# gchochla/VAuLT

Hardware: AMD Instinct MI355X
Metric: train samples/sec (img+text pairs) ViLT-B32+BERTweet, bs256, 1/2/4/8 MI355X (higher is better)
Workload: dtype bf16; 1 GPU; ViLT-B32 + bertweet fine-tune step (fwd+bwd+AdamW), per-GPU batch 256, 40 text tokens + 384x384 image (185-token fused sequence; resident as the patch-embedding operand `pixel_patches`, the input pipeline's output), all weights trained; global_batch=256, seq_len=185, parallelism=dp1

## Files before the change

include/vault_hip.h:

```cpp
#ifndef VAULT_HIP_H
#define VAULT_HIP_H
#include <stdint.h>
#ifdef __cplusplus
extern "C" {
#endif

int vault_abi_version(void);
int vault_operand_format(void);

typedef struct vault_gemm_args {
  const void* A; const void* B; void* out; void* out2;
  const float* bias; const float* res; const void* aux; const float* addtab;
  float* colsum;
  int split3;
  int M, N, K, lda, ldb, ldo, m_valid;
  int a_mode, b_mode, epi, cfg, splits, accumulate;
  int rpg, gstride, goff;
  uint32_t drop_thresh, drop_seed, drop_stream; float drop_scale;
  int gn;
  int persist;
  int batch;
  long long batch_a, batch_b, batch_o;
  int aux_u8;
  int out_hm;
  int a_hm;
  void* out_q; void* out_scale;
  void* splitk_ws; long long splitk_bytes;
} vault_gemm_args;
int vault_gemm(const vault_gemm_args* args, void* stream);
int vault_gemm_plan(const vault_gemm_args* args);

typedef struct vault_wgrad_seg {
  const void* dy; const void* x; float* dw;
  int n_out, n_in, ld_dy, ld_x, ld_dw;
  int batch;
  int first, count;
  long long batch_dy, batch_x, batch_dw;
  int dy_hm;
} vault_wgrad_seg;
typedef struct vault_wgrad_grouped_args {
  int nseg;
  vault_wgrad_seg seg[3];
  int tokens, splits, accumulate;
  int persist;
} vault_wgrad_grouped_args;
int vault_wgrad_grouped(const vault_wgrad_grouped_args* args, void* stream);

int vault_quant_mxfp8(const void* src_bf16, long long rows, int K, int ld_src, void* dst_q, void* dst_scale, void* stream);
int vault_gemm_mxfp8(const vault_gemm_args* args, const void* a_scale, const void* b_scale, void* stream);
int vault_gemm_mxfp8_plan(const vault_gemm_args* args);


typedef struct vault_ln_fwd_args {
  const float* x; const float* gamma; const float* beta; const float* post_add;
  void* y_bf16; float* y_f32; float* mean; float* rstd;
  int rows, H; float eps;
  int x_rpg, x_gstride, x_goff, y_rpg, y_gstride, y_goff;
  uint32_t drop_thresh, drop_seed, drop_stream; float drop_scale;
  void* y_split3;
  void* y_q; void* y_scale;
} vault_ln_fwd_args;
int vault_layernorm_fwd(const vault_ln_fwd_args* args, void* stream);

typedef struct vault_ln_bwd_args {
  const void* dy_bf16; const float* dy_f32; const float* x; const float* mean; const float* rstd;
  const float* gamma; const float* dres;
  float* dx_f32; void* dx_bf16; float* dgamma; float* dbeta;
  int rows, H;
  int dy_rpg, dy_gstride, dy_goff, x_rpg, x_gstride, x_goff, dx_rpg, dx_gstride, dx_goff;
  uint32_t drop_thresh, drop_seed, drop_stream; float drop_scale;
  int drop_on_dy;
  float* dbias;
  const void* dres_bf16;
} vault_ln_bwd_args;
int vault_layernorm_bwd(const vault_ln_bwd_args* args, void* stream);

int vault_colsum(const void* in_bf16, int ld, int rows, int N, float* out, void* stream);
int vault_colsum_hm(const void* in_bf16, int rows, int hm_rows, int planes, float* out, int batch, long long batch_in,
                    long long batch_out, void* stream);
int vault_colsum_batched(const void* in_bf16, int ld, int rows, int N, float* out, int batch, long long batch_in,
                         long long batch_out, void* stream);


typedef struct vault_attn_args {
  const void* qkv; const float* keymask; void* ctx; float* lse;
  const void* dctx; void* dqkv;
  int B, S, H, heads;
  uint32_t drop_thresh, drop_seed, drop_stream; float drop_scale;
  void* ctx_split3;
  int qkv_hm;
  float* bias_partials;
  int bias_thirds;
  int q_rows;
} vault_attn_args;
int vault_attention_fwd(const vault_attn_args* args, void* stream);
int vault_attention_bwd(const vault_attn_args* args, void* stream);
int vault_attention_bwd_partials(const vault_attn_args* args);
int vault_colsum_partials(const float* part, int nparts, int n, float* out, int batch, long long batch_in,
                          long long batch_out, void* stream);


int vault_position_ids(const int64_t* ids, int* pos, int B, int T, int mode, int pad, void* stream);

typedef struct vault_gather_args {
  const float* src; float* out;
  const float* tab[3]; const void* idx[3]; int is64[3]; int fixed[3];
  int period, rows, H;
  const float* rowmask;
} vault_gather_args;
int vault_gather_sum(const vault_gather_args* args, void* stream);
int vault_scatter_add(const vault_gather_args* args, void* stream);

int vault_im2col(const float* pixel_values, void* out_bf16, int B, int C, int IMG, int ps, int split3, void* stream);

int vault_image_consts(const float* conv_bias, const float* pos_emb, const float* mtype1, const float* cls,
                       float* addtab, float* x, int P, int H, int B, int S, int T, void* stream);
int vault_image_rows_bwd(const float* dx, float* dpos, float* dmtype1, float* dcls, float* dconv_bias,
                         void* dyp_bf16, int P, int H, int B, int S, int T, void* stream);

int vault_im2col_sel(const float* pixel_values, void* out_bf16, const int* sel, int B, int L, int C, int HP, int WP,
                     int ps, int split3, void* stream);
int vault_image_sel_consts(const float* conv_bias, const float* pos_emb, const float* mtype1, const float* cls,
                           float* addtab, float* x, int L, int H, int B, int S, int T, void* stream);
int vault_image_pos_sel_fwd(float* x, const float* pos_emb, const int* sel, const int* hw, int B, int L, int S, int T,
                            int H, int gw, int G, void* stream);
int vault_image_sel_bwd(const float* dx, float* dpos, float* dmtype1, float* dcls, float* dconv_bias, void* dyp_bf16,
                        const int* sel, const int* hw, int B, int L, int S, int T, int H, int gw, int G, void* stream);
int vault_axpy_f32(float* dst, const float* src, float a, long long n, void* stream);
int vault_scale_f32(float* x, float a, long long n, void* stream);
int vault_rows_add_f32(const float* src, const float* vec, float* out, int rows, int H, int rpg, int gstride, int goff,
                       void* stream);
int vault_rows_gather_bwd_f32(const float* dx, float* dsrc, float* dvec, int rows, int H, int rpg, int gstride, int goff,
                              void* stream);
int vault_rows_scatter_bf16(const void* src, void* out, int rows, int H, int rpg, int gstride, int goff, void* stream);

typedef struct vault_head_args {
  const float* pre; const float* Wc; const float* bc; const int64_t* labels; const float* dlogits;
  float* pooled; float* logits; float* loss_sum; float* dWc; float* dbc; void* dpre_bf16;
  int B, H, C; float loss_scale, grad_scale;
  uint32_t drop_thresh, drop_seed, drop_stream; float drop_scale;
  const float* targets; int loss_kind;
} vault_head_args;
int vault_head_fwd(const vault_head_args* args, void* stream);
int vault_head_bwd(const vault_head_args* args, void* stream);
int vault_tanh_bwd(const float* pooled, const float* dpooled, void* dpre_bf16, long long n, void* stream);
int vault_gelu_fwd(const float* x, void* y_bf16, long long n, void* stream);
int vault_gelu_fwd_f32(const float* x, float* y_f32, long long n, void* stream);
int vault_gelu_bwd(const float* x, const float* dy, float* dx, long long n, void* stream);

int vault_adamw_step(float* p, float* g, float* m, float* v, void* p_bf16, long long n, float lr, float beta1,
                     float beta2, float eps, float weight_decay, float bias_corr_factor, float grad_scale,
                     int zero_grad, const unsigned char* zero_mask, void* stream);
#define VAULT_GRAD_NORM_PARTIALS 2048
int vault_grad_norm(const float* g, long long n, double* partials, float* out2, float max_norm, float unscale, void* stream);
int vault_adamw_step_grouped(float* p, float* g, float* m, float* v, void* p_bf16, long long n,
                             const unsigned char* group_map, const float* group_table, int n_groups, float lr_factor,
                             float beta1, float beta2, float eps, float bias_corr_factor, float grad_scale,
                             const float* coef, int zero_grad, const unsigned char* zero_mask, void* stream);
int vault_adamw_step_ema(float* p, float* g, float* m, float* v, void* p_bf16, float* ema, long long n,
                         const unsigned char* group_map, const float* group_table, int n_groups, float lr_factor,
                         float beta1, float beta2, float eps, float bias_corr_factor, float grad_scale, const float* coef,
                         float one_minus_decay, int zero_grad, const unsigned char* zero_mask, void* stream);
int vault_ema_swap(float* p, float* ema, void* p_bf16, long long n, void* stream);
int vault_adamw_step_torch(float* p, float* g, float* m, float* v, void* p_bf16, float* ema ,
                           long long n, const unsigned char* group_map, const float* group_table, int n_groups,
                           float lr_factor, float beta1, float beta2, float eps, float inv_bias_corr1,
                           float inv_sqrt_bias_corr2, float grad_scale, const float* coef, float one_minus_decay,
                           int zero_grad, const unsigned char* zero_mask, void* stream);
int vault_cast_bf16(const float* x, void* y_bf16, long long n, void* stream);
int vault_h16_census(const void* x_h16, long long n, unsigned long long* out4, void* stream);
int vault_rows_union(const long long* keys, long long n_keys, int V, int* flags_zeroed, long long* uniq, int* count,
                     void* stream);
int vault_rows_gather_f32(const float* table, const long long* idx, int n_rows, int H, float* out, void* stream);
int vault_rows_scatter_f32(const float* src, const long long* idx, int n_rows, int H, float* table, void* stream);
int vault_sum_chunks_bf16(const void* src_bf16, int n_src, long long chunk, void* out_bf16, void* stream);
int vault_widen_bf16(const void* x_bf16, float* y, long long n, void* stream);
int vault_transpose_bf16(const void* src, void* dst, int rows, int cols, int batch, long long stride_src,
                         long long stride_dst, void* stream);
int vault_split3_bf16(const float* x, void* out_bf16, long long rows, int K, int layout, void* stream);

typedef struct vault_layer_args {
  int B, S, H, FF, heads, rows, rows_pad; float eps;
  const void *wqkv, *wo, *wi, *wf, *wo_t, *wf_t;
  const float *bqkv, *bo, *bi, *bf, *ln1w, *ln1b, *ln2w, *ln2b;
  const float* x_in; const void* x_in_bf16; float* x_out; void* x_out_bf16; const float* keymask;
  void *n1, *qkv, *ctx; float* lse; float* xm; float* y1; void* n2; void* act; void* u; float* h2;
  float *m1, *r1, *m2, *r2;
  uint32_t attn_drop_thresh, hid_drop_thresh, drop_seed, drop_stream_base; float attn_drop_scale, hid_drop_scale;
  int persist;
  void* splitk_ws; long long splitk_bytes;
} vault_layer_args;
typedef struct vault_layer_bwd_args {
  const vault_layer_args* fwd;
  const void* dy_bf16; const float* dy_f32;
  float* dx_f32; void* dx_bf16;
  void *dU, *dN, *dctx, *dqkv, *dmid_bf16, *dh1_bf16; float* dmid_f32;
  float *g_wqkv, *g_bqkv, *g_wo, *g_bo, *g_wi, *g_bi, *g_wf, *g_bf, *g_ln1w, *g_ln1b, *g_ln2w, *g_ln2b, *g_bf_below;
  int do_wgrad;
} vault_layer_bwd_args;
long long vault_layer_workspace_bytes(int B, int S, int H, int FF, int heads, int train, long long* rows_pad_out);
int vault_vilt_layer_fwd(const vault_layer_args* args, void* stream);
int vault_vilt_layer_bwd(const vault_layer_bwd_args* args, void* stream);
int vault_lm_layer_fwd(const vault_layer_args* args, void* stream);
int vault_lm_layer_bwd(const vault_layer_bwd_args* args, void* stream);

typedef struct vault_lm_embed_args {
  int B, T, H, rows_pad, pos_mode, pad_id; float eps;
  const int64_t* ids; const int64_t* token_type_ids; const float* inputs_embeds;
  const float *word, *pos, *type, *lnw, *lnb;
  int* pos_ids; float* esum; float* mean; float* rstd; float* y; void* y_bf16;
  uint32_t drop_thresh, drop_seed, drop_stream; float drop_scale;
  const void* dy_bf16; const float* dy_f32; float* desum; const float* rowmask;
  float *g_word, *g_pos, *g_type, *g_lnw, *g_lnb;
} vault_lm_embed_args;
int vault_lm_embed_fwd(const vault_lm_embed_args* args, void* stream);
int vault_lm_embed_bwd(const vault_lm_embed_args* args, void* stream);

typedef struct vault_text_embed_args {
  int B, T, S, H, rows_pad; float eps;
  const float* text_src; const int64_t* ids; const int64_t* token_type_ids;
  const float *word, *pos, *type, *lnw, *lnb, *mtype0;
  float* vsum; float* mean; float* rstd; float* x;
  const float* dx; float* dvsum; float* dbeta_scratch;
  float *g_word, *g_pos, *g_type, *g_lnw, *g_lnb, *g_mtype0;
} vault_text_embed_args;
int vault_vilt_text_embed_fwd(const vault_text_embed_args* args, void* stream);
int vault_vilt_text_embed_bwd(const vault_text_embed_args* args, void* stream);

typedef struct vault_patch_embed_args {
  int B, C, IMG, ps, T, S, H;
  const float* pixel_values; const void* w_bf16; const float *conv_bias, *pos_emb, *mtype1, *cls;
  void* apatch; float* addtab; float* x; int persist;
  const float* dx; void* dyp;
  float *g_w, *g_conv_bias, *g_pos, *g_mtype1, *g_cls;
} vault_patch_embed_args;
int vault_patch_embed_fwd(const vault_patch_embed_args* args, void* stream);
int vault_patch_embed_bwd(const vault_patch_embed_args* args, void* stream);

typedef struct vault_head_loss_args {
  int B, S, H, C, seq_rows_pad; float eps;
  const float* x; const float *lnw, *lnb; const void* wp_bf16; const float* bp; const float *Wc, *bc;
  const int64_t* labels; const float* targets; int loss_kind; float loss_scale, grad_scale;
  void* h0_bf16; float* mean; float* rstd; float* pre; float* pooled; float* logits; float* loss;
  uint32_t drop_thresh, drop_seed, drop_stream; float drop_scale; int persist;
  void* dpre; void* dh0; float* dx_f32; void* dx_bf16;
  float *g_Wc, *g_bc, *g_wp, *g_bp, *g_lnw, *g_lnb, *g_bf_last;
} vault_head_loss_args;
int vault_head_loss_fwd(const vault_head_loss_args* args, void* stream);
int vault_head_loss_bwd(const vault_head_loss_args* args, void* stream);

typedef struct vault_image_desc {
  long long src_off, tmp_off;
  int h_in, w_in, h_out, w_out, ksize_h, ksize_v;
  int hb_off, hk_off, vb_off, vk_off;
} vault_image_desc;
typedef struct vault_preprocess_args {
  const uint8_t* src; uint8_t* tmp; const int* plan; const vault_image_desc* desc; const float* lut;
  float* pixel_values; int64_t* pixel_mask; float* pixel_mask_f32;
  int B, H, W, max_h_in, max_w_out;
  int max_w_in; long long src_bytes;
  void* patch_unfold_bf16; int ps;
  int ksize_max, band_rows_max;
} vault_preprocess_args;
int vault_image_preprocess(const vault_preprocess_args* args, void* stream);
int vault_image_preprocess_is_fused(const vault_preprocess_args* args);

typedef struct vault_model_dims {
  int H, FF, heads, lm_layers, vilt_layers, IMG, ps, C, n_classes;
} vault_model_dims;
long long vault_workspace_bytes(const vault_model_dims* dims, int B, int T, int train);

#ifdef __cplusplus
}
#endif
#endif
```

vault_amd/backward.py:

```python
from __future__ import annotations

import contextlib
from typing import Dict, Optional

import torch

from . import ops
from .params import _in_format, _pad


class BackwardMixin:
    def _wgrads_aside(self, launch, after_layer, items=0):
        if not (self._wgrad_side or items > 0) or after_layer is not None:
            launch()
            return
        if self._wgrad_stream is None:
            self._wgrad_stream = torch.cuda.Stream(self.device)
        side, main, ev = self._wgrad_stream, torch.cuda.current_stream(), torch.cuda.Event()
        ops.pycall(lambda: ev.record(main))
        ops.pycall(lambda: side.wait_event(ev))
        with torch.cuda.stream(side):
            self._wgrad_items = items
            try:
                launch()
            finally:
                self._wgrad_items = 0
        self._wgrad_pending = True

    def _join_wgrads(self):
        if self._wgrad_pending:
            side, main, ev = self._wgrad_stream, torch.cuda.current_stream(), torch.cuda.Event()
            ops.pycall(lambda: ev.record(side))
            ops.pycall(lambda: main.wait_event(ev))
            self._wgrad_pending = False

    def _wgrad(self, dy_bf16, x_bf16, wname, bname, Mtok_pad, Nout, Kin, m_valid, out_rows=0, unsplit=False):
        P = self.params
        gw = P.gr(wname, n_elems=Nout * Kin, shape=(Nout, Kin))
        if gw is None:
            return
        nk = Mtok_pad // 64
        wide = Nout % 256 == 0 and Kin % 256 == 0 and (Nout // 256) * (Kin // 256) >= 24
        if Mtok_pad <= 16384 and Nout % 128 == 0 and Kin % 128 == 0 and not wide:
            tiles = (Nout // 128) * (Kin // 128)
            splits = 7 if tiles <= 36 else (4 if tiles <= 108 else 3)
            cfg = 0
        elif Nout % 256 == 0 and Kin % 256 == 0:
            tiles = (Nout // 256) * (Kin // 256)
            splits = max(1, min(nk // 2, 256 // tiles, 16))
            cfg = 3
        else:
            tiles = (Nout // 128) * (Kin // 128)
            splits = max(1, min(nk, (self.WGRAD_TARGET_WGS + tiles - 1) // tiles))
            cfg = 0
        if unsplit:
            splits = 1
        if cfg == 3:
            ops.pycall(lambda: self._prof_begin("wgrad"))
        ops.gemm(dy_bf16, x_bf16, gw, Nout, Kin, Mtok_pad, Nout, Kin, Kin, 1, 1, ops.EPI_F32_ATOMIC, cfg=cfg,
                 splits=splits, accumulate=1, m_valid=out_rows)
        if cfg == 3:
            fl = 2.0 * m_valid * Nout * Kin
            ops.pycall(lambda: self._prof_end("wgrad", fl))
        if bname is not None:
            ops.colsum(dy_bf16, Nout, m_valid, Nout, P.gr(bname, n_elems=Nout, shape=(Nout,)))

    @staticmethod
    def _wgrad_splits(items, per_round, nk, fixed, fixed_unsplit=None):
        def cost(sp):
            fx = fixed_unsplit if (sp == 1 and fixed_unsplit is not None) else fixed
            return -(-items * sp // per_round) * (1.67 * -(-nk // sp) + fx)
        return min((sp for sp in range(1, 9) if nk // sp >= 2), key=cost)

    def _wgrad_batched(self, dY_all, X_all, wnames, i0, Mtok_pad, Nout, Kin, m_valid):
        P = self.params
        G = len(wnames)
        offs = [P.offsets[w][0] for w in wnames]
        stride_o = (offs[1] - offs[0]) if G > 1 else 0
        if any(offs[k + 1] - offs[k] != stride_o for k in range(G - 1)) or Nout % 128 or Kin % 128:
            raise RuntimeError("batched weight gradients need identically laid out layers and 128-multiples")
        gw = P.gr(wnames[0], n_elems=Nout * Kin, shape=(Nout, Kin))
        nk = Mtok_pad // 64
        if Nout % 256 == 0 and Kin % 256 == 0:
            cfg, tiles = 3, (Nout // 256) * (Kin // 256) * G
            splits = self._wgrad_splits(tiles, 256, nk, 40.0)
        else:
            cfg, tiles = 0, (Nout // 128) * (Kin // 128) * G
            splits = max(1, min(8, Mtok_pad // 512, int(round(512.0 / tiles))))
        st = torch.cuda.current_stream()
        if cfg == 3:
            ops.pycall(lambda: self._prof_begin("wgrad", st))
        acc = 0 if (self._grads_zero and splits == 1) else 1
        ops.gemm(dY_all[i0], X_all[i0], gw, Nout, Kin, Mtok_pad, Nout, Kin, Kin, 1, 1, ops.EPI_F32_ATOMIC, cfg=cfg,
                 splits=splits, accumulate=acc, batch=G, batch_a=dY_all.stride(0), batch_b=X_all.stride(0),
                 batch_o=stride_o)
        if acc == 0:
            self._stored_ranges += [(o, Nout * Kin) for o in offs]
        if cfg == 3:
            fl = 2.0 * m_valid * Nout * Kin * G
            ops.pycall(lambda: self._prof_end("wgrad", fl, st))
    def _wgrad_group_size(self, n_layers, after_layer, stack="lm"):
        if after_layer is None or self.dp_world <= 1:
            return n_layers
        if stack == "vilt" and self.spec.lm is not None and not self.freeze_lm:
            return n_layers
        g = self.LM_WGRAD_GROUP
        return g if g > 0 else n_layers

    def _wgrad_group(self, kinds, layers, i0, hi, Mtok_pad, m_valid, counts=None):
        P = self.params
        Gs = [hi - i0] * len(kinds) if counts is None else list(counts)
        kinds, Gs = [k for k, n in zip(kinds, Gs) if n > 0], [n for n in Gs if n > 0]
        hms = [k[5] if len(k) > 5 else 0 for k in kinds]
        kinds = [k[:5] for k in kinds]
        ok = all(no % 256 == 0 and ki % 256 == 0 for *_, no, ki in kinds)
        strides = []
        for (dY_all, X_all, wsel, Nout, Kin), G in zip(kinds, Gs):
            offs = [P.offsets[getattr(l_, wsel)][0] for l_ in layers[i0:i0 + G]]
            so = (offs[1] - offs[0]) if G > 1 else 0
            ok = ok and all(offs[k + 1] - offs[k] == so for k in range(G - 1))
            strides.append(so)
        if not ok:
            if any(hms):
                raise RuntimeError("head-major dqkv needs the grouped ring weight-gradient launches (_plan_head_major)")
            for (dY_all, X_all, wsel, Nout, Kin), G in zip(kinds, Gs):
                self._wgrad_batched(dY_all, X_all, [getattr(l_, wsel) for l_ in layers[i0:i0 + G]], i0, Mtok_pad, Nout, Kin, m_valid)
            return
        nk = Mtok_pad // 64
        CU = self._wgrad_items or (self.WGRAD_SIDE_ITEMS if self._wgrad_side else 256)
        remaining = []
        for k, (dY_all, X_all, wsel, Nout, Kin) in enumerate(kinds):
            remaining.append([k, 0, (Nout // 256) * (Kin // 256) * Gs[k]])
        launches, cur, room = [], [], CU
        for k, first, left in remaining:
            while left > 0:
                take = min(left, room)
                cur.append((k, first, take))
                first, left, room = first + take, left - take, room - take
                if room == 0 or len(cur) == 3:
                    launches.append(cur)
                    cur, room = [], CU
        if cur:
            launches.append(cur)
        st = torch.cuda.current_stream()
        covered: Dict[tuple, int] = {}
        for segs in launches:
            count = sum(c for _, _, c in segs)
            if count == CU:
                splits = 1
            else:
                splits = self._wgrad_splits(count, CU, nk, 50.0, 10.0 if self._grads_zero else 50.0)
            acc = 0 if (self._grads_zero and splits == 1) else 1
            args = []
            for k, first, c in segs:
                dY_all, X_all, wsel, Nout, Kin = kinds[k]
                if acc == 0:
                    tpl = (Nout // 256) * (Kin // 256)
                    for it in range(first, first + c):
                        covered[(k, it // tpl)] = covered.get((k, it // tpl), 0) + 1
                gw = P.gr(getattr(layers[i0], wsel), n_elems=Nout * Kin, shape=(Nout, Kin))
                args.append(dict(dy=dY_all[i0], x=X_all[i0], dw=gw, n_out=Nout, n_in=Kin, batch=Gs[k], first=first, count=c,
                                 batch_dy=dY_all.stride(0), batch_x=X_all.stride(0), batch_dw=strides[k], dy_hm=hms[k]))
            ops.pycall(lambda: self._prof_begin("wgrad", st))
            ops.wgrad_grouped(args, Mtok_pad, splits=splits, accumulate=acc)
            fl = 2.0 * m_valid * 65536.0 * count
            ops.pycall(lambda fl=fl: self._prof_end("wgrad", fl, st))
        for (k, lay), n in covered.items():
            _, _, wsel, Nout, Kin = kinds[k]
            if n == (Nout // 256) * (Kin // 256):
                self._stored_ranges.append((P.offsets[getattr(layers[i0 + lay], wsel)][0], Nout * Kin))

    def _qkv_bias_grads_batched(self, dqkv_all, layers, i0, hi, ld, rows, N, hm=0, parts=None):
        P = self.params
        offs = [P.offsets[l_.qb][0] for l_ in layers[i0:hi]]
        stride_o = (offs[1] - offs[0]) if len(offs) > 1 else 0
        if any(offs[k + 1] - offs[k] != stride_o for k in range(len(offs) - 1)):
            raise RuntimeError("batched bias gradients need identically laid out layers")
        gqb = P.gr(layers[i0].qb, n_elems=ld, shape=(ld,))
        if parts is not None:
            part_all, nparts = parts
            ops.colsum_partials(part_all[i0], nparts, N, gqb, hi - i0, part_all.stride(0), stride_o)
            return
        if hm:
            ops.colsum_hm(dqkv_all[i0], rows, hm, N // 64, gqb, hi - i0, dqkv_all.stride(0), stride_o)
            return
        ops.colsum_batched(dqkv_all[i0], ld, rows, N, gqb, hi - i0, dqkv_all.stride(0), stride_o)
    @_in_format
    def zero_grad(self):
        if self.params.g is not None:
            self.params.g.zero_()
        self._g_dirty = False
        self._g_stale_key = None

    def backward(self, grad_scale: Optional[float] = None, dlogits: Optional[torch.Tensor] = None,
                 dpooled: Optional[torch.Tensor] = None, dhidden: Optional[torch.Tensor] = None,
                 after_layer=None, ws: Optional[dict] = None):
        self._api_backward_begins()
        with torch.cuda.device(self.device), self._grads_scaled():
            self._backward(grad_scale, dlogits, dpooled, dhidden, after_layer, ws)
            if self.grad_scale != 1.0:
                w_ = self.last if ws is None else ws
                for k in ("d_inputs_embeds", "d_image_embeds"):
                    t = w_.get(k)
                    if t is not None:
                        with ops.operand_format(self.half):
                            ops.scale(t, 1.0 / self.grad_scale, t.numel())

    def _api_backward_begins(self):
        if self._g_stale_key is not None:
            self.zero_grad()
        self._g_dirty = True

    @contextlib.contextmanager
    def _grads_scaled(self):
        def rescale(factor):
            if self.grad_scale != 1.0 and self.params.g is not None:
                with ops.operand_format(self.half):
                    ops.scale(self.params.g, factor, self.params.n_train)
        rescale(self.grad_scale)
        try:
            yield
        finally:
            rescale(1.0 / self.grad_scale)

    def _scaled_in(self, ws, name, t):
        t = t.contiguous()
        if self.grad_scale == 1.0:
            return t
        b = self._buf(ws, name, tuple(t.shape), torch.float32)
        b.copy_(t)
        ops.scale(b.view(-1), self.grad_scale, b.numel())
        return b

    @_in_format
    def _backward(self, grad_scale, dlogits, dpooled, dhidden, after_layer, ws=None, grads_zero=False):
        self._grads_zero = bool(grads_zero)
        self._stored_ranges = []
        ws = self.last if ws is None else ws
        if ws is None or not ws.get("train"):
            raise RuntimeError("backward() needs a preceding forward(train=True)")
        if ws.get("pruned_last") and dhidden is not None:
            raise ValueError("the forward pruned the last layer to the pooler's rows: a gradient of last_hidden_state needs "
                             "forward(need_hidden=True)")
        self.drop_seed = ws["drop_seed"]
        note = (lambda tag: ops.pycall(lambda: after_layer(tag))) if after_layer is not None else (lambda tag: None)
        self._wgrad_side = ws["Mp"] <= self.WGRAD_STREAM_MAX_ROWS
        vb = self._vilt_grad_buffers(ws, after_layer)
        self._backward_head(ws, vb["top"], grad_scale, dlogits, dpooled, dhidden)
        note("head")
        self._backward_vilt_stack(ws, vb, after_layer, note)
        dvs = self._backward_vilt_embeddings(ws, vb["dx"], after_layer)
        note("vilt_embed")
        if self.spec.lm is None or self.freeze_lm:
            self._join_wgrads()
        else:
            self._backward_lm_stack(ws, dvs, after_layer, note)
        self._run_census(ws, "backward")

    def _wgrad_groups(self, ws, tag, layers, after_layer, dY, X, rows_pad, rows):
        H, FF = ws["H"], ws["FF"]
        kinds = tuple((dy, ws[x], wsel, no, ki) for dy, x, (wsel, no, ki) in
                      zip(dY, X, (("fw", H, FF), ("iw", FF, H), ("ow", H, H), ("qw", 3 * H, H))))
        n, cut = len(layers), 1 if (tag == "vilt" and ws.get("pruned_last")) else 0
        return dict(layers=layers, size=self._wgrad_group_size(n, after_layer, tag), kinds=kinds, H=H,
                    rows_pad=rows_pad, rows=rows, ends=(n - cut, n - cut, n - cut, n))

    def _layer_done(self, tag, grp, i, note, after_layer, N=None, hm=0, parts=None, items=0, ahead=None):
        if grp is None:
            note(f"{tag}{i}")
        if grp is None or i % grp["size"]:
            return
        layers, kinds, H, hi = grp["layers"], grp["kinds"], grp["H"], min(len(grp["layers"]), i + grp["size"])
        if ahead is not None:
            ahead()

        def launch():
            self._qkv_bias_grads_batched(kinds[3][0], layers, i, hi, 3 * H, grp["rows"], 3 * H if N is None else N, hm=hm, parts=parts)
            self._wgrad_group(kinds[:3] + (kinds[3] + (hm,),), layers, i, hi, grp["rows_pad"], grp["rows"],
                              counts=[max(0, min(hi, e) - i) for e in grp["ends"]])
        self._wgrads_aside(launch, after_layer, items=items)
        for j in reversed(range(i, hi)):
            note(f"{tag}{j}")

    def _backward_head(self, ws, dxb_top, grad_scale, dlogits, dpooled, dhidden):
        spec, P, x, nv = self.spec, self.params, ws["x"], len(self.vl)
        B, S, M, H = (ws[k] for k in ("B", "S", "M", "H"))
        pruned = bool(ws.get("pruned_last"))
        cls_map = (0, 0, 0) if pruned else (1, S, 0)
        if not pruned:
            ops.pycall(dxb_top.zero_)
        if spec.add_pooling_layer and (spec.n_classes > 0 or dpooled is not None):
            Bp = ws["Bp"]
            dpre = self._buf(ws, "dpre", (Bp, H), self.hdt)
            if spec.n_classes > 0 and spec.head == "mlp" and dpooled is None:
                if dlogits is None:
                    raise ValueError("the MLP head has no built-in loss: pass dlogits (the autograd bridge does)")
                ops.tanh_bwd(ws["pooled"], self._mlp_backward(ws, dlogits, B, scale=self.grad_scale), dpre, B * H)
            elif spec.n_classes > 0 and dpooled is None:
                hd = self._drop(self.classifier_dropout, 9001, True)
                gs = ((1.0 / B) if grad_scale is None else grad_scale) * self.grad_scale
                if dlogits is not None:
                    dlogits = self._scaled_in(ws, "dlogits_scaled", dlogits)
                ops.head_bwd(ws["pooled"], ws["logits"], ws.get("labels"), P.w("classifier.1.weight"),
                             P.gr("classifier.1.weight"), P.gr("classifier.1.bias"), dpre, B, H, spec.n_classes, gs,
                             dlogits=dlogits, drop=hd)
            else:
                ops.tanh_bwd(ws["pooled"], self._scaled_in(ws, "dpooled_scaled", dpooled), dpre, B * H)
            self._wgrad(dpre, ws["h0b"], "pooler.dense.weight", "pooler.dense.bias", Bp, H, H, B)
            dh0 = self._buf(ws, "dh0", (Bp, H), self.hdt)
            self._dgrad(dpre, "pooler.dense.weight", dh0, Bp, H, H, ops.EPI_BF16, B)
            ops.layernorm_bwd(ws["pl_xout"] if pruned else x[nv], ws["f_mean"], ws["f_rstd"], P.w("layernorm.weight"), B, H,
                              dy_bf16=dh0, dx_bf16=dxb_top, dgamma=P.gr("layernorm.weight"),
                              dbeta=P.gr("layernorm.bias"), xmap=cls_map, dxmap=cls_map,
                              dbias=None if dhidden is not None else P.gr(self.vl[nv - 1].fb))
        if dhidden is not None:
            ops.layernorm_bwd(x[nv], ws["f_mean_all"], ws["f_rstd_all"], P.w("layernorm.weight"), M, H,
                              dy_f32=self._scaled_in(ws, "dhidden_scaled", dhidden).view(M, H),
                              dres_bf16=dxb_top,
                              dx_bf16=dxb_top,
                              dgamma=P.gr("layernorm.weight"), dbeta=P.gr("layernorm.bias"),
                              dbias=P.gr(self.vl[nv - 1].fb))

    def _layer_bwd_staged(self, ws, style, layers, i, d, deferred):
        P, ln, H = self.params, layers[i], ws["H"]
        a = ws[f"stage_{style}{i}"]
        if style == "lm":
            a.drop_seed = self.drop_seed & 0xFFFFFFFF
        gb = ops.layer_bwd_args(
            a, **d, do_wgrad=0 if deferred else 1, g_wqkv=P.gr(ln.qw, n_elems=3 * H * H, shape=(3 * H, H)),
            g_bqkv=None if deferred else P.gr(ln.qb, n_elems=3 * H, shape=(3 * H,)),
            g_wo=P.gr(ln.ow), g_bo=P.gr(ln.ob), g_wi=P.gr(ln.iw), g_bi=P.gr(ln.ib), g_wf=P.gr(ln.fw),
            g_ln1w=P.gr(ln.ln1w), g_ln1b=P.gr(ln.ln1b), g_ln2w=P.gr(ln.ln2w), g_ln2b=P.gr(ln.ln2b),
            g_bf=P.gr(ln.fb) if style == "lm" else None,
            g_bf_below=P.gr(layers[i - 1].fb) if (style == "vilt" and i > 0) else None)
        ws[f"stage_{style}_bwd{i}"] = gb
        ops.layer_call(f"vault_{style}_layer_bwd", gb, seeded=bool(a.attn_drop_thresh or a.hid_drop_thresh))

    def _vilt_grad_buffers(self, ws, after_layer):
        Mp, H, FF, nv, bf = ws["Mp"], ws["H"], ws["FF"], len(self.vl), self.hdt
        vb = dict(dx=self._buf(ws, "dx_a", (Mp, H), torch.float32), grp=None,
                  dxb=(self._buf(ws, "dxb_a", (Mp, H), bf), self._buf(ws, "dxb_b", (Mp, H), bf)))
        if self.LM_WGRAD_BATCHED and "act_all" in ws and self.params.gr(self.vl[0].fw) is not None:
            vb["dY"] = (self._stack(ws, "v_dxbA", nv, (Mp, H), bf), self._stack(ws, "v_dU", nv, (Mp, FF), bf),
                        self._stack(ws, "v_dxbB", nv, (Mp, H), bf), self._stack(ws, "v_dqkv", nv, (Mp, 3 * H), bf))
            vb["grp"] = self._wgrad_groups(ws, "vilt", self.vl, after_layer, vb["dY"],
                                           ("act_all", "n2_all", "ctx_all", "n1_all"), Mp, ws["M"])
        vb["top"] = vb["dY"][0][nv - 1] if vb["grp"] else vb["dxb"][0]
        if ws.get("pruned_last"):
            vb["top"] = self._buf(ws, "pl_dtop", (ws["Bp"], H), bf)
        return vb

    def _backward_vilt_stack(self, ws, vb, after_layer, note):
        B, S, Mp, H, FF, heads, nv, bf = ws["B"], ws["S"], ws["Mp"], ws["H"], ws["FF"], ws["heads"], len(self.vl), self.hdt
        grp, staged, (dxa, dxb) = vb["grp"], bool(ws.get("vilt_stage")), vb["dxb"]
        d = dict(dN=self._buf(ws, "dN", (Mp, H), bf), dctx=self._buf(ws, "dctx", (Mp, H), bf))
        if not grp:
            d.update(dy_bf16=dxa, dmid_bf16=dxb, dx_bf16=dxa, dU=self._buf(ws, "dU", (Mp, FF), bf), dqkv=self._buf(ws, "dqkv", (Mp, 3 * H), bf))
        short, vparts = bool(grp) and self.QKV_BIAS_SHORTCUT and not staged, None
        if short:
            npart = ops.attention_bwd_partials(B, S, H, heads, 1)
            if npart:
                vparts = (self._stack(ws, "v_qbpart", nv, (npart, H), torch.float32), npart)
        beside = self.WGRAD_BESIDE_LM_ITEMS if (grp and grp["size"] >= nv and not staged and self.spec.lm is not None
                                                and not self.freeze_lm and not self._wgrad_side) else 0
        ops.pycall(lambda: self._prof_begin("vilt_bwd"))
        for i in reversed(range(nv)):
            if grp:
                d["dy_bf16"], d["dU"], d["dmid_bf16"], d["dqkv"] = (t[i] for t in vb["dY"])
                d["dx_bf16"] = vb["dY"][0][i - 1] if i > 0 else dxa
            d["dx_f32"] = vb["dx"] if i == 0 else None
            if staged:
                self._layer_bwd_staged(ws, "vilt", self.vl, i, d, bool(grp))
            elif i == nv - 1 and ws.get("pruned_last"):
                self._vilt_last_layer_bwd_pruned(ws, i, d, bool(grp), short, vparts, vb["top"])
            else:
                self._vilt_layer_bwd(ws, i, d, bool(grp), short, vparts)
            self._layer_done("vilt", grp, i, note, after_layer, H if short else 3 * H, ws.get("qkv_hm", 0), vparts, beside)
        ops.pycall(lambda: self._prof_end("vilt_bwd"))

    def _vilt_layer_bwd(self, ws, i, d, deferred, short, vparts):
        P, ln, vhm = self.params, self.vl[i], ws.get("qkv_hm", 0)
        B, S, M, Mp, H, FF, heads = (ws[k] for k in ("B", "S", "M", "Mp", "H", "FF", "heads"))
        g = lambda k: ws[f"{k}{i}"]
        wgrad = (lambda *a: None) if deferred else self._wgrad
        dyA, dyB, dU, dqkv, dN, dctx = (d[k] for k in ("dy_bf16", "dmid_bf16", "dU", "dqkv", "dN", "dctx"))
        g8 = ws.get("gelu8_active")
        g8kw = dict(cfg=g8, aux_u8=True) if g8 is not None else {}
        self._dgrad(dyA, ln.fw, dU, Mp, FF, H, ops.EPI_BF16_DGELU, M, aux=g("u"), colsum=P.gr(ln.ib), **g8kw)
        wgrad(dyA, g("act"), ln.fw, None, Mp, H, FF, M)
        self._dgrad(dU, ln.iw, dN, Mp, H, FF, ops.EPI_BF16, M)
        wgrad(dU, g("n2"), ln.iw, None, Mp, FF, H, M)
        ops.layernorm_bwd(g("xm"), g("m2"), g("r2"), P.w(ln.ln2w), M, H, dy_bf16=dN, dres_bf16=dyA, dx_bf16=dyB,
                          dgamma=P.gr(ln.ln2w), dbeta=P.gr(ln.ln2b), dbias=P.gr(ln.ob))
        gqb = P.gr(ln.qb, n_elems=3 * H, shape=(3 * H,))
        self._dgrad(dyB, ln.ow, dctx, Mp, H, H, ops.EPI_BF16, M, **(dict(colsum=gqb[2 * H:]) if short else {}))
        wgrad(dyB, g("ctx"), ln.ow, None, Mp, H, H, M)
        ops.attention_bwd(g("qkv"), ws["keymask"], g("ctx"), g("lse"), dctx, dqkv, B, S, H, heads, qkv_hm=vhm,
                          **(dict(bias_partials=vparts[0][i], bias_thirds=1) if vparts else {}))
        self._dgrad(dqkv, ln.qw, dN, Mp, H, 3 * H, ops.EPI_BF16, M, **(dict(a_hm=vhm) if vhm else {}))
        wgrad(dqkv, g("n1"), ln.qw, ln.qb, Mp, 3 * H, H, M)
        ops.layernorm_bwd(ws["x"][i], g("m1"), g("r1"), P.w(ln.ln1w), M, H, dy_bf16=dN, dres_bf16=dyB,
                          dx_f32=d["dx_f32"], dx_bf16=d["dx_bf16"], dgamma=P.gr(ln.ln1w), dbeta=P.gr(ln.ln1b),
                          dbias=P.gr(self.vl[i - 1].fb) if i > 0 else None)

    def _vilt_last_layer_bwd_pruned(self, ws, i, d, deferred, short, vparts, dtop):
        P, ln, vhm = self.params, self.vl[i], ws.get("qkv_hm", 0)
        B, S, M, Mp, H, FF, heads, Bp = (ws[k] for k in ("B", "S", "M", "Mp", "H", "FF", "heads", "Bp"))
        bf = self.hdt
        g, c = (lambda k: ws[f"{k}{i}"]), (lambda k: ws[f"pl_{k}"])
        dU, dNc, dmid, dctx = (self._buf(ws, f"pl_{k}", (Bp, w), bf) for k, w in (("dU", FF), ("dN", H), ("dmid", H), ("dctx", H)))
        dres, dqkv, dN = self._buf(ws, "pl_dres", (Mp, H), bf), d["dqkv"], d["dN"]
        g8 = ws.get("pl_gelu8")
        g8kw = dict(cfg=g8, aux_u8=True) if g8 is not None else {}
        self._dgrad(dtop, ln.fw, dU, Bp, FF, H, ops.EPI_BF16_DGELU, B, aux=c("u"), colsum=P.gr(ln.ib), like=Mp, **g8kw)
        self._wgrad(dtop, c("act"), ln.fw, None, Bp, H, FF, B, unsplit=True)
        self._dgrad(dU, ln.iw, dNc, Bp, H, FF, ops.EPI_BF16, B, like=Mp)
        self._wgrad(dU, c("n2"), ln.iw, None, Bp, FF, H, B, unsplit=True)
        ops.layernorm_bwd(c("xm"), c("m2"), c("r2"), P.w(ln.ln2w), B, H, dy_bf16=dNc, dres_bf16=dtop, dx_bf16=dmid,
                          dgamma=P.gr(ln.ln2w), dbeta=P.gr(ln.ln2b), dbias=P.gr(ln.ob))
        ops.rows_scatter_h16(dmid, dres, B, H, 1, S, 0)
        gqb = P.gr(ln.qb, n_elems=3 * H, shape=(3 * H,))
        self._dgrad(dmid, ln.ow, dctx, Bp, H, H, ops.EPI_BF16, B, like=Mp, **(dict(colsum=gqb[2 * H:]) if short else {}))
        self._wgrad(dmid, c("ctx"), ln.ow, None, Bp, H, H, B, unsplit=True)
        ops.attention_bwd(g("qkv"), ws["keymask"], c("ctx"), g("lse"), dctx, dqkv, B, S, H, heads, qkv_hm=vhm, q_rows=1,
                          **(dict(bias_partials=vparts[0][i], bias_thirds=1) if vparts else {}))
        self._dgrad(dqkv, ln.qw, dN, Mp, H, 3 * H, ops.EPI_BF16, M, **(dict(a_hm=vhm) if vhm else {}))
        if not deferred:
            self._wgrad(dqkv, g("n1"), ln.qw, ln.qb, Mp, 3 * H, H, M)
        ops.layernorm_bwd(ws["x"][i], g("m1"), g("r1"), P.w(ln.ln1w), M, H, dy_bf16=dN, dres_bf16=dres,
                          dx_f32=d["dx_f32"], dx_bf16=d["dx_bf16"], dgamma=P.gr(ln.ln1w), dbeta=P.gr(ln.ln1b),
                          dbias=P.gr(self.vl[i - 1].fb) if i > 0 else None)

    def _backward_vilt_embeddings(self, ws, dx0, after_layer):
        spec, P, v = self.spec, self.params, self.spec.vilt
        B, T, S, H, NP, Ml, Mlp, Kp, Mpp = (ws[k] for k in ("B", "T", "S", "H", "NP", "Ml", "Mlp", "Kp", "Mpp"))
        buf = lambda name, shape, dtype=torch.float32: self._buf(ws, name, shape, dtype)
        dyp = buf("dyp", (Mpp, H), self.hdt)
        gpos = P.gr("embeddings.position_embeddings", shape=(v.num_patches + 1, H))
        gmt = P.gr("embeddings.token_type_embeddings.weight")
        if ws.get("img_embeds") is not None:
            die = buf("d_iemb", (_pad(B * NP), H))
            ops.rows_gather_bwd(dx0, die, gmt[ws.get("img_type", 1)], B * NP, H, NP, S, T)
            ws["d_image_embeds"] = die[:B * NP].view(B, NP, H)
        elif ws["ragged"]:
            ops.image_sel_bwd(dx0, gpos, gmt[ws.get("img_type", 1)], P.gr("embeddings.cls_token", shape=(H,)),
                              P.gr("embeddings.patch_embeddings.projection.bias"), dyp, ws["sel"], ws["hw"], B, NP, S, T, H,
                              ws["gw"], v.image_size // v.patch_size)
        else:
            ops.image_rows_bwd(dx0, gpos, gmt[ws.get("img_type", 1)], P.gr("embeddings.cls_token", shape=(H,)),
                               P.gr("embeddings.patch_embeddings.projection.bias"), dyp, NP, H, B, S, T)
        if ws.get("img_embeds") is None:
            self._wgrads_aside(lambda: self._wgrad(dyp, ws["apatch_in"] if ws.get("patches_in") else ws["apatch"],
                                                   "embeddings.patch_embeddings.projection.weight", None,
                                                   Mpp, H, Kp, B * NP), after_layer)
        dvs = buf("d_vt_sum", (Mlp, H))
        dbeta_now = buf("d_vt_beta", (H,))
        ops.pycall(dbeta_now.zero_)
        ops.layernorm_bwd(ws["vt_sum"], ws["vt_mean"], ws["vt_rstd"], P.w("embeddings.text_embeddings.LayerNorm.weight"),
                          Ml, H, dy_f32=dx0, dymap=(T, S, 0), dx_f32=dvs,
                          dgamma=P.gr("embeddings.text_embeddings.LayerNorm.weight"), dbeta=dbeta_now)
        ops.axpy(P.gr("embeddings.text_embeddings.LayerNorm.bias"), dbeta_now, 1.0, H)
        ops.axpy(gmt[0], dbeta_now, 1.0, H)
        tt = ws["tt"]
        gt = [(P.gr("embeddings.text_embeddings.token_type_embeddings.weight"), tt if tt is not None else 0)]
        if spec.lm is None:
            if ws.get("txt_embeds") is not None:
                ws["d_inputs_embeds"] = dvs[:Ml].view(B, T, H)
            else:
                gt.append((P.gr("embeddings.text_embeddings.word_embeddings.weight"), ws["ids"]))
        if ws["use_pos"]:
            gt.append((P.gr("embeddings.text_embeddings.position_embeddings.weight"), "mod"))
        ops.scatter_add(dvs, gt, Ml, H, period=T)
        return dvs

    def _backward_lm_stack(self, ws, dvs, after_layer, note):
        B, T, H, FF, heads, Ml, Mlp = (ws[k] for k in ("B", "T", "H", "FF", "heads", "Ml", "Mlp"))
        nl, bf, staged = len(self.ll), self.hdt, bool(ws.get("lm_stage"))
        buf = lambda name, shape, dtype=torch.float32: self._buf(ws, name, shape, dtype)
        dN, grp = buf("lm_dN", (Mlp, H), bf), None
        d = dict(dy_bf16=None, dy_f32=dvs, dmid_f32=buf("lm_dh", (Mlp, H)), dx_f32=buf("lm_dh1", (Mlp, H)), dN=dN, dx_bf16=dN,
                 dctx=buf("lm_dctx", (Mlp, H), bf))
        if self.LM_WGRAD_BATCHED and "lm_act_all" in ws and self.params.gr(self.ll[0].fw) is not None:
            dY = (self._stack(ws, "lm_dhb", nl, (Mlp, H), bf), self._stack(ws, "lm_dU", nl, (Mlp, FF), bf),
                  self._stack(ws, "lm_dh1b", nl, (Mlp, H), bf), self._stack(ws, "lm_dqkv", nl, (Mlp, 3 * H), bf))
            grp = self._wgrad_groups(ws, "lm", self.ll, after_layer, dY,
                                     ("lm_act_all", "lm_y1b_all", "lm_ctx_all", "lm_yb_all"), Mlp, Ml)
        else:
            d.update(dmid_bf16=buf("lm_dhb", (Mlp, H), bf), dh1_bf16=buf("lm_dh1b", (Mlp, H), bf),
                     dU=buf("lm_dU", (Mlp, FF), bf), dqkv=buf("lm_dqkv", (Mlp, 3 * H), bf))
        lparts = None
        if self.LM_BIAS_PARTIALS and grp and not staged:
            npart = ops.attention_bwd_partials(B, T, H, heads, 3)
            if npart:
                lparts = (self._stack(ws, "lm_qbpart", nl, (npart, 3 * H), torch.float32), npart)
        embed_done = []

        def embed_ahead():
            self._lm_embed_backward(ws, d["dy_bf16"], d["dy_f32"])
            embed_done.append(True)
            note("lm_embed")
        ops.pycall(lambda: self._prof_begin("lm_bwd"))
        for i in reversed(range(nl)):
            if grp:
                d["dmid_bf16"], d["dU"], d["dh1_bf16"], d["dqkv"] = (t[i] for t in dY)
            if staged:
                self._layer_bwd_staged(ws, "lm", self.ll, i, d, bool(grp))
            else:
                self._lm_layer_bwd(ws, i, d, bool(grp), lparts)
            d["dy_bf16"], d["dy_f32"] = d["dN"], d["dx_f32"]
            self._layer_done("lm", grp, i, note, after_layer, hm=ws.get("lm_qkv_hm", 0), parts=lparts,
                             ahead=embed_ahead if (i == 0 and after_layer is not None) else None)
        ops.pycall(lambda: self._prof_end("lm_bwd"))
        if not embed_done:
            self._lm_embed_backward(ws, d["dy_bf16"], d["dy_f32"])
        self._join_wgrads()
        if not embed_done:
            note("lm_embed")

    def _lm_embed_backward(self, ws, dyb, dyf):
        P = self.params
        B, T, H, Ml, Mlp = (ws[k] for k in ("B", "T", "H", "Ml", "Mlp"))
        desum = self._buf(ws, "lm_desum", (Mlp, H), torch.float32)
        ops.layernorm_bwd(ws["lm_esum"], ws["lm_emean"], ws["lm_erstd"], P.w("bert.embeddings.LayerNorm.weight"), Ml, H,
                          dy_bf16=dyb, dy_f32=dyf, dx_f32=desum, dgamma=P.gr("bert.embeddings.LayerNorm.weight"),
                          dbeta=P.gr("bert.embeddings.LayerNorm.bias"),
                          drop=self._drop(self.spec.lm.hidden_dropout_prob, 1, True), drop_on_dy=True)
        if ws.get("txt_embeds") is not None:
            ws["d_inputs_embeds"] = desum[:Ml].view(B, T, H)
        ops.scatter_add(desum, [None if ws.get("txt_embeds") is not None else
                                (P.gr("bert.embeddings.word_embeddings.weight"), ws["ids"]),
                                (P.gr("bert.embeddings.position_embeddings.weight"), ws["lm_pos"]),
                                (P.gr("bert.embeddings.token_type_embeddings.weight"), ws["lm_tt"])], Ml, H,
                        rowmask=ws["amf"])

    def _lm_layer_bwd(self, ws, i, d, deferred, lparts):
        P, ln, lm, lhm = self.params, self.ll[i], self.spec.lm, ws.get("lm_qkv_hm", 0)
        B, T, H, FF, heads, Ml, Mlp = (ws[k] for k in ("B", "T", "H", "FF", "heads", "Ml", "Mlp"))
        pdh, pda = lm.hidden_dropout_prob, lm.attention_probs_dropout_prob
        g = lambda k: ws[f"lm_{k}{i}"]
        wgrad = (lambda *a: None) if deferred else self._wgrad
        dh, dh1, dhb, dh1b, dU, dqkv, dN, dctx = (d[k] for k in ("dmid_f32", "dx_f32", "dmid_bf16", "dh1_bf16", "dU", "dqkv", "dN", "dctx"))
        ops.layernorm_bwd(g("h2"), g("m2"), g("r2"), P.w(ln.ln2w), Ml, H, dy_bf16=d["dy_bf16"], dy_f32=d["dy_f32"], dx_f32=dh,
                          dx_bf16=dhb, dgamma=P.gr(ln.ln2w), dbeta=P.gr(ln.ln2b),
                          drop=self._drop(pdh, 16 * i + 4, True), dbias=P.gr(ln.fb))
        self._dgrad(dhb, ln.fw, dU, Mlp, FF, H, ops.EPI_BF16_DGELU, Ml, aux=g("u"), colsum=P.gr(ln.ib))
        wgrad(dhb, g("act"), ln.fw, None, Mlp, H, FF, Ml)
        self._dgrad(dU, ln.iw, dN, Mlp, H, FF, ops.EPI_BF16, Ml)
        wgrad(dU, g("y1b"), ln.iw, None, Mlp, FF, H, Ml)
        ops.layernorm_bwd(g("h1"), g("m1"), g("r1"), P.w(ln.ln1w), Ml, H, dy_bf16=dN, dy_f32=dh, dx_f32=dh1,
                          dx_bf16=dh1b, dgamma=P.gr(ln.ln1w), dbeta=P.gr(ln.ln1b),
                          drop=self._drop(pdh, 16 * i + 3, True), dbias=P.gr(ln.ob))
        self._dgrad(dh1b, ln.ow, dctx, Mlp, H, H, ops.EPI_BF16, Ml)
        wgrad(dh1b, g("ctx"), ln.ow, None, Mlp, H, H, Ml)
        ops.attention_bwd(g("qkv"), ws["amf"], g("ctx"), g("lse"), dctx, dqkv, B, T, H, heads,
                          drop=self._drop(pda, 16 * i + 2, True), qkv_hm=lhm,
                          **(dict(bias_partials=lparts[0][i], bias_thirds=3) if lparts else {}))
        self._dgrad(dqkv, ln.qw, dN, Mlp, H, 3 * H, ops.EPI_BF16, Ml, **(dict(a_hm=lhm) if lhm else {}))
        wgrad(dqkv, ws["lm_yb"][i], ln.qw, ln.qb, Mlp, 3 * H, H, Ml)
```

vault_amd/csrc/capi_gemm.hip:

```cpp
#include "common.h"
#include "gemm.h"
#include "../../include/vault_hip.h"

int vault_gemm_mx8_launch(const GemmParams& p, const void* a_scale, const void* b_scale, int epi, int cfg, hipStream_t st);

static GemmParams params_of(const vault_gemm_args* a) {
  GemmParams p{};
  p.A = reinterpret_cast<const h16*>(a->A);
  p.B = reinterpret_cast<const h16*>(a->B);
  p.M = a->M; p.N = a->N; p.K = a->K;
  p.lda = a->lda; p.ldb = a->ldb; p.ldo = a->ldo;
  p.m_valid = a->m_valid > 0 ? a->m_valid : a->M;
  p.splits = a->splits; p.accumulate = a->accumulate;
  p.out = a->out; p.out2 = a->out2;
  p.bias = a->bias; p.res = a->res;
  p.aux = reinterpret_cast<const h16*>(a->aux);
  p.addtab = a->addtab; p.colsum = a->colsum; p.split3 = a->split3; p.rpg = a->rpg; p.gstride = a->gstride; p.goff = a->goff;
  p.drop_thresh = a->drop_thresh; p.drop_seed = a->drop_seed; p.drop_stream = a->drop_stream;
  p.drop_scale = a->drop_scale;
  p.gn = a->gn;
  p.persist = a->persist;
  p.batch = a->batch; p.batch_a = a->batch_a; p.batch_b = a->batch_b; p.batch_o = a->batch_o;
  p.aux_u8 = a->aux_u8;
  p.out_hm = a->out_hm; p.a_hm = a->a_hm;
  p.out_q = a->out_q; p.out_scale = a->out_scale;
  p.sk_ws = a->splitk_ws; p.sk_bytes = a->splitk_ws ? a->splitk_bytes : 0;
  return p;
}

extern "C" int vault_gemm(const vault_gemm_args* a, void* stream) {
  if (a == nullptr) return VAULT_EINVAL;
  return vault_gemm_launch(params_of(a), a->a_mode, a->b_mode, a->epi, a->cfg, reinterpret_cast<hipStream_t>(stream));
}

int vault_gemm_resolve(GemmParams& p, int a_mode, int b_mode, int epi, int cfg);

extern "C" int vault_gemm_plan(const vault_gemm_args* a) {
  if (a == nullptr) return -VAULT_EINVAL;
  GemmParams p = params_of(a);
  return vault_gemm_resolve(p, a->a_mode, a->b_mode, a->epi, a->cfg);
}

extern "C" int vault_gemm_mxfp8(const vault_gemm_args* a, const void* a_scale, const void* b_scale, void* stream) {
  if (a == nullptr || a->a_mode != 0 || a->b_mode != 0 || a->splits > 1) return VAULT_EINVAL;
  return vault_gemm_mx8_launch(params_of(a), a_scale, b_scale, a->epi, a->cfg, reinterpret_cast<hipStream_t>(stream));
}

int vault_gemm_mx8_resolve(const GemmParams& p, const void* a_scale, const void* b_scale, int epi, int cfg, GemmParams& q);

extern "C" int vault_gemm_mxfp8_plan(const vault_gemm_args* a) {
  if (a == nullptr || a->a_mode != 0 || a->b_mode != 0 || a->splits > 1) return -VAULT_EINVAL;
  GemmParams q;
  return vault_gemm_mx8_resolve(params_of(a), a->A, a->B, a->epi, a->cfg, q);
}

extern "C" int vault_wgrad_grouped(const vault_wgrad_grouped_args* a, void* stream) {
  if (a == nullptr || a->nseg < 1 || a->nseg > 3 || a->tokens <= 0 || (a->tokens & 63)) return VAULT_EINVAL;
  GemmParams p{};
  p.K = a->tokens;
  p.splits = a->splits > 0 ? a->splits : 1;
  p.accumulate = a->accumulate;
  p.persist = a->persist;
  p.nseg = a->nseg;
  for (int k = 0; k < a->nseg; ++k) {
    const vault_wgrad_seg& g = a->seg[k];
    if (g.n_out <= 0 || g.n_in <= 0 || (g.n_out & 255) || (g.n_in & 255) || g.batch < 1) return VAULT_EINVAL;
    GemmParams::Seg& t = p.seg[k];
    t.A = reinterpret_cast<const h16*>(g.dy); t.B = reinterpret_cast<const h16*>(g.x); t.out = g.dw;
    t.tiles_n = g.n_in / 256; t.tiles = (g.n_out / 256) * t.tiles_n;
    t.lda = g.ld_dy; t.ldb = g.ld_x; t.ldo = g.ld_dw;
    t.first = g.first; t.count = g.count;
    if (g.first < 0 || g.count < 1 || g.first + g.count > t.tiles * g.batch) return VAULT_EINVAL;
    t.batch_a = g.batch_dy; t.batch_b = g.batch_x; t.batch_o = g.batch_dw;
    t.a_hm = g.dy_hm;
    if (g.dy_hm < 0 || (g.dy_hm > 0 && g.dy_hm < a->tokens)) return VAULT_EINVAL;
    if (g.dy_hm > 0) t.lda = 64;
  }
  return vault_gemm256_grouped_launch(p, reinterpret_cast<hipStream_t>(stream));
}

extern "C" int vault_abi_version(void) { return 12; }
#ifdef VAULT_F16
extern "C" int vault_operand_format(void) { return 1; }
#else
extern "C" int vault_operand_format(void) { return 0; }
#endif
```

vault_amd/csrc/gemm.h:

```cpp
#pragma once
#include <hip/hip_runtime.h>
#include <stdint.h>
#include "common.h"

enum GemmEpi {
  EPI_BF16 = 0,
  EPI_BF16_GELU = 1,
  EPI_BF16_DGELU = 2,
  EPI_F32_RES = 3,
  EPI_F32_PATCH = 4,
  EPI_F32_ATOMIC = 5,
  EPI_BF16_GELU_INF = 6,
  EPI_BF16_GELU_U8 = 7,
  EPI_BF16_DGELU_U8 = 8,
};

struct GemmParams {
  const h16* A;
  const h16* B;
  int M, N, K;
  int lda, ldb;
  int m_valid;
  int splits;
  int accumulate;
  void* out;
  int ldo;
  void* out2;
  const float* bias;
  const float* res;
  const h16* aux;
  const float* addtab;
  int split3;
  float* colsum;
  int rpg, gstride, goff;
  uint32_t drop_thresh, drop_seed, drop_stream;
  float drop_scale;
  int persist;
  int gn;
  int batch;
  long long batch_a, batch_b, batch_o;
  int aux_u8;
  int out_hm, a_hm;
  const uint8_t* a_scale;
  const uint8_t* b_scale;
  int lds_a, lds_b;
  void* out_q;
  void* out_scale;
  void* sk_ws;
  long long sk_bytes;
  int nseg;
  struct Seg {
    const h16* A;
    const h16* B;
    float* out;
    int tiles_n, tiles;
    int lda, ldb, ldo;
    int first, count;
    long long batch_a, batch_b, batch_o;
    int a_hm;
  } seg[3];
};

constexpr int GEMM_SK_COUNTER_BYTES = 16384;
constexpr int GEMM_SK_MAX_TILES = GEMM_SK_COUNTER_BYTES / 4;

#ifdef __HIPCC__
__device__ __forceinline__ int gemm_xcd_contiguous(int n, int id) {
  const int q = n >> 3, r = n & 7, xcd = id & 7;
  return (xcd < r ? xcd * (q + 1) : r * (q + 1) + (xcd - r) * q) + (id >> 3);
}
__device__ __forceinline__ void gemm_raster(int wg, int tiles_m, int tiles_n, int gn, int& tile_m, int& tile_n) {
  const int per_group = tiles_m * gn;
  const int grp = wg / per_group;
  const int rem = wg - grp * per_group;
  const int gw = min(gn, tiles_n - grp * gn);
  tile_m = rem / gw;
  tile_n = grp * gn + (rem - tile_m * gw);
}
__device__ __forceinline__ void gemm_tile_of_block(int nwg, int id, int tiles_m, int tiles_n, int gn, int& tile_m,
                                                   int& tile_n) {
  gemm_raster(gemm_xcd_contiguous(nwg, id), tiles_m, tiles_n, gn, tile_m, tile_n);
}
#endif

int vault_gemm_launch(const GemmParams& p, int a_mode, int b_mode, int epi, int cfg, hipStream_t st);
int vault_gemm256_grouped_launch(const GemmParams& p, hipStream_t st);
```

vault_amd/csrc/gemm256.hip:

```cpp
#include <algorithm>
#include "common.h"
#include "gemm.h"
#include "gemm_epi.h"

#ifndef R256_ABLATE
#define R256_ABLATE 0
#endif
#ifndef R256_DYN
#define R256_DYN 0
#endif

#ifndef R256_STAMP
#define R256_STAMP 0
#endif
#if R256_DYN
#undef R256_STAMP
#define R256_STAMP 0
#endif
#if R256_STAMP
__device__ unsigned long long g_r256_stamp[256 * 2];
extern "C" int vault_debug_r256_stamps(unsigned long long* out512) {
  return (int)hipMemcpyFromSymbol(out512, HIP_SYMBOL(g_r256_stamp), sizeof(g_r256_stamp));
}
#endif

namespace {

__device__ unsigned int g_ring_tickets[2][8];

constexpr int HT = 16384;
constexpr int BUFB = 4 * HT;

#define WAITBAR(N) asm volatile("s_waitcnt vmcnt(%0) lgkmcnt(0)\n\ts_barrier" ::"i"(N) : "memory")
#define R256_SGPR_PAD "s_nop 4\n\t"

#define WAITBAR2(FLAG, NF, N)                                                                                  \
  asm volatile("s_cmp_eq_u32 %0, 0\n\ts_cbranch_scc1 2\n\ts_waitcnt vmcnt(%1) lgkmcnt(0)\n\ts_branch 1\n"     \
               "\ts_waitcnt vmcnt(%2) lgkmcnt(0)\n\ts_barrier" ::"s"(__builtin_amdgcn_readfirstlane((int)(FLAG))), "i"(NF), "i"(N) \
               : "memory", "scc")

template <int OFF>
__device__ __forceinline__ s16x4 tr16_asm(uint32_t lds_addr) {
  s16x4 v;
  asm volatile("ds_read_b64_tr_b16 %0, %1 offset:%2" : "=v"(v) : "v"(lds_addr), "i"(OFF));
  return v;
}

#ifndef R256_ORDER
#define R256_ORDER -1
#endif
template <int A_MODE, int B_MODE, int EPI, int NTQ, bool DYN, bool SK = false>
__global__ __launch_bounds__(256) void gemm256_kernel(const GemmParams p) {
  H16_SATURATE();
#if R256_STAMP
  const unsigned long long st_c0 = __builtin_amdgcn_s_memtime(), st_r0 = __builtin_amdgcn_s_memrealtime();
#endif
  constexpr int BNT = NTQ * 64;
  constexpr int PH_ORDER = (R256_ORDER >= 0) ? R256_ORDER : (EPI == EPI_F32_ATOMIC ? 0 : 1);
  constexpr int PB = (B_MODE == 0) ? NTQ : 4;
  constexpr int W32 = 3 * 4 + 2 * PB;
  constexpr int W23 = 2 * 4 + 3 * PB;
  extern __shared__ __attribute__((aligned(16))) char smem[];
  const int tid = threadIdx.x;
  const int lane = tid & 63;
  const int wave = __builtin_amdgcn_readfirstlane(tid >> 6);
  const int wr = wave >> 1, wc = wave & 1;
  constexpr int TN = 2 * NTQ;
  constexpr int SCRATCH_BYTES = 4 * 16 * ((NTQ == 3 ? 96 : 64) + 4) * 4;
  constexpr bool F32OUT = (EPI == EPI_F32_RES || EPI == EPI_F32_PATCH);
  constexpr int SPS = (EPI == EPI_F32_ATOMIC) ? 16 * (TN * 16 / 64) : (F32OUT ? TN : TN / 2);
#define CAPW(N, STEPS) (((N) + (STEPS) * SPS) > 63 ? 63 : ((N) + (STEPS) * SPS))

  const int tiles_m = p.M >> 8, tiles_n = p.N / BNT, ntiles = tiles_m * tiles_n;
  const int nbatch = (EPI == EPI_F32_ATOMIC && p.batch > 1) ? p.batch : 1;
  bool grouped = false;
  int seg_total = 0;
  if constexpr (EPI == EPI_F32_ATOMIC && A_MODE == 1 && B_MODE == 1) {
    grouped = p.nseg > 0;
    seg_total = p.seg[0].count + (p.nseg > 1 ? p.seg[1].count : 0) + (p.nseg > 2 ? p.seg[2].count : 0);
  }
  const int nwork = grouped ? seg_total * p.splits : ntiles * p.splits * nbatch;
  const int nk_total = p.K >> 6;
  const int per = (nk_total + p.splits - 1) / p.splits;

  int m0, n0, nk;
  int cur_z = 0, cur_tl = 0;
  float* out_cur = reinterpret_cast<float*>(p.out);
  int ldo_cur = p.ldo, mvalid_cur = p.m_valid;
  const char* a_base;
  const char* b_base;
  uint32_t a_off[4], b_off[4];
  uint32_t a_half, b_half, a_step, b_step;
  if constexpr (A_MODE == 0) { a_half = 64u * p.lda * 2u; a_step = p.a_hm ? (uint32_t)p.a_hm * 128u : 128u; }
  else { a_half = 128u; a_step = 64u * p.lda * 2u; }
  if constexpr (B_MODE == 0) { b_half = (uint32_t)(NTQ * 16) * p.ldb * 2u; b_step = 128u; }
  else { b_half = (uint32_t)(NTQ * 16) * 2u; b_step = 64u * p.ldb * 2u; }
  auto lane_offsets = [&](int lda_, int ldb_, int a_hm_ = 0) {
    const int ln_ = lane_id_volatile();
    int wv_ = wave;
    asm volatile("" : "+s"(wv_));
#pragma unroll
    for (int i = 0; i < 4; ++i) {
      const int j = wv_ * 4 + i;
      const int r8 = ln_ >> 3, r = 8 * j + r8;
      const int c = (ln_ & 7) ^ (((r8 >> 1) & 3) << 1);
      const int krow = 4 * j + (ln_ >> 4), pos16 = ln_ & 15;
      const int hk = (krow & 3) | (((krow >> 3) & 1) << 2);
      const int cb = (pos16 >> 1) ^ hk;
      if constexpr (A_MODE == 0) a_off[i] = (uint32_t)(((r >> 6) * 128 + (r & 63)) * lda_ + c * 8) * 2u;
      else if (a_hm_ == 0) a_off[i] = (uint32_t)(krow * lda_ + (cb >> 2) * 128 + (cb & 3) * 16 + (pos16 & 1) * 8) * 2u;
      else a_off[i] = ((uint32_t)krow * 64u + (uint32_t)(cb >> 2) * 2u * (uint32_t)a_hm_ * 64u + (uint32_t)((cb & 3) * 16 + (pos16 & 1) * 8)) * 2u;
      if constexpr (B_MODE == 0) {
        const int jb = wv_ * PB + (i < PB ? i : PB - 1), rb = 8 * jb + r8;
        const int wcol = rb / (NTQ * 16), within = rb - wcol * (NTQ * 16);
        b_off[i] = (uint32_t)((wcol * (NTQ * 32) + within) * ldb_ + c * 8) * 2u;
      } else {
        const int ntc = min(cb & 3, NTQ - 1);
        b_off[i] = (uint32_t)(krow * ldb_ + (cb >> 2) * (NTQ * 32) + ntc * 16 + (pos16 & 1) * 8) * 2u;
      }
    }
  };
  auto setup = [&](int w) {
    if constexpr (EPI == EPI_F32_ATOMIC && A_MODE == 1 && B_MODE == 1) {
      if (grouped) {
        const int lin = gemm_xcd_contiguous(nwork, w);
        const int z = lin / seg_total;
        int r = lin - z * seg_total;
        const int c0 = p.seg[0].count, c1 = (p.nseg > 1) ? p.seg[1].count : 0;
        const int si = (r < c0) ? 0 : ((r < c0 + c1) ? 1 : 2);
        r -= (si == 0) ? 0 : (si == 1 ? c0 : c0 + c1);
#define SEGF(F) ((si == 0) ? p.seg[0].F : ((si == 1) ? p.seg[1].F : p.seg[2].F))
        const int idx = SEGF(first) + r, tiles_k = SEGF(tiles), tn_k = SEGF(tiles_n);
        const int bz = idx / tiles_k, tl = idx - bz * tiles_k;
        const int lda_ = SEGF(lda), ldb_ = SEGF(ldb), ahm_ = SEGF(a_hm);
#if R256_ABLATE & 1
        const h16* pA = SEGF(A);
        const h16* pB = SEGF(B);
#else
        const h16* pA = SEGF(A) + (size_t)bz * SEGF(batch_a);
        const h16* pB = SEGF(B) + (size_t)bz * SEGF(batch_b);
#endif
        out_cur = SEGF(out) + (size_t)bz * SEGF(batch_o);
        ldo_cur = SEGF(ldo);
        mvalid_cur = (tiles_k / tn_k) << 8;
#undef SEGF
        const int tm_k = tiles_k / tn_k;
        int tile_m, tile_n;
        if (tn_k > tm_k) { tile_n = tl / tm_k; tile_m = tl - tile_n * tm_k; }
        else { tile_m = tl / tn_k; tile_n = tl - tile_m * tn_k; }
        m0 = tile_m << 8; n0 = tile_n << 8;
        const int kt0 = z * per;
        nk = min(nk_total, kt0 + per) - kt0;
        a_step = 64u * (uint32_t)lda_ * 2u; b_step = 64u * (uint32_t)ldb_ * 2u;
        a_half = ahm_ ? (uint32_t)ahm_ * 128u : 128u;
        lane_offsets(lda_, ldb_, ahm_);
#if R256_ABLATE & 1
        const int lm0 = 0, ln0 = 0;
#else
        const int lm0 = m0, ln0 = n0;
#endif
        a_base = ahm_ ? reinterpret_cast<const char*>(pA + ((size_t)(lm0 >> 6) * ahm_ + (size_t)kt0 * 64) * 64)
                      : reinterpret_cast<const char*>(pA + (size_t)kt0 * 64 * lda_ + lm0);
        b_base = reinterpret_cast<const char*>(pB + (size_t)kt0 * 64 * ldb_ + ln0);
        return;
      }
    }
    int lin = gemm_xcd_contiguous(nwork, w);
    const h16* pA = p.A;
    const h16* pB = p.B;
    if constexpr (EPI == EPI_F32_ATOMIC) {
      if (nbatch > 1) {
        const int per_problem = ntiles * p.splits;
        const int bz = lin / per_problem;
        lin -= bz * per_problem;
        pA += (size_t)bz * p.batch_a; pB += (size_t)bz * p.batch_b;
        out_cur = reinterpret_cast<float*>(p.out) + (size_t)bz * p.batch_o;
      }
    }
    const int z = lin / ntiles, tl = lin - z * ntiles;
    if constexpr (SK) { cur_z = z; cur_tl = tl; }
    int tile_m, tile_n;
    gemm_raster(tl, tiles_m, tiles_n, p.gn, tile_m, tile_n);
    m0 = tile_m << 8; n0 = tile_n * BNT;
    const int kt0 = z * per;
    nk = min(nk_total, kt0 + per) - kt0;
#if R256_ABLATE & 1
    const int lm0 = 0, ln0 = 0;
#else
    const int lm0 = m0, ln0 = n0;
#endif
    if constexpr (A_MODE == 0) a_base = p.a_hm ? reinterpret_cast<const char*>(pA + ((size_t)kt0 * p.a_hm + lm0) * 64)
                                               : reinterpret_cast<const char*>(pA + (size_t)lm0 * p.lda + (size_t)kt0 * 64);
    else a_base = reinterpret_cast<const char*>(pA + (size_t)kt0 * 64 * p.lda + lm0);
    if constexpr (B_MODE == 0) b_base = reinterpret_cast<const char*>(pB + (size_t)ln0 * p.ldb + (size_t)kt0 * 64);
    else b_base = reinterpret_cast<const char*>(pB + (size_t)kt0 * 64 * p.ldb + ln0);
  };
  int w = blockIdx.x;
  setup(w);
  const int xcd = blockIdx.x & 7;
  auto items_of = [&](int x) { return x < nwork ? (nwork - x + 7) >> 3 : 0; };
  auto static_of = [&](int x) { return x < (int)gridDim.x ? ((int)gridDim.x - x + 7) >> 3 : 0; };
  const int TICKET_ITEMS = (nwork <= 2 * (int)gridDim.x) ? 1 : 2;
  int pend_w = -1;
  int last_tk = 0;
  const bool dyn = DYN && (p.persist & 1) != 0;
  unsigned int* const tickets = g_ring_tickets[(p.persist >> 8) & 1];
  if (dyn && blockIdx.x == 0 && tid < 8) g_ring_tickets[((p.persist >> 8) & 1) ^ 1][tid] = 0u;
  if (!grouped) lane_offsets(p.lda, p.ldb);

  auto pieceA = [&](int h, int buf, int t, int i) {
    uint32_t o = a_off[i];
    asm volatile("" : "+v"(o));
    glds16(a_base + (size_t)h * a_half + (size_t)t * a_step + o, smem + buf * BUFB + h * HT + wave * 4096 + i * 1024);
  };
  auto pieceB = [&](int h, int buf, int t, int i) {
    if (i < PB) {
      uint32_t o = b_off[i];
      asm volatile("" : "+v"(o));
      glds16(b_base + (size_t)h * b_half + (size_t)t * b_step + o,
             smem + buf * BUFB + 2 * HT + h * HT + (wave * PB + i) * 1024);
    }
  };
  auto issueA = [&](int h, int buf, int t) {
#pragma unroll
    for (int i = 0; i < 4; ++i) pieceA(h, buf, t, i);
  };
  auto issueB = [&](int h, int buf, int t) {
#pragma unroll
    for (int i = 0; i < 4; ++i) pieceB(h, buf, t, i);
  };

#define LOAD_TR(DST, ADDR, BUF, H)                                                                       \
  {                                                                                                      \
    const uint32_t ad_ = (ADDR) + (BUF) * BUFB;                                                          \
    DST[0] = cat_tr(tr16_asm<(H) * HT>(ad_), tr16_asm<(H) * HT + 1024>(ad_));                            \
    DST[1] = cat_tr(tr16_asm<(H) * HT + 8192>(ad_), tr16_asm<(H) * HT + 8192 + 1024>(ad_));             \
  }
#define LOADA_U(RA, BUF, H, U)                                                                           \
  {                                                                                                      \
    if constexpr (A_MODE == 0) {                                                                         \
      const char* base_ = smem + (BUF) * BUFB + (H) * HT;                                                \
      RA[U][0] = *LDS_PTR(const h16x8, base_ + a_o0 + (U) * 2048);                                      \
      RA[U][1] = *LDS_PTR(const h16x8, base_ + a_o1 + (U) * 2048);                                      \
    } else {                                                                                             \
      LOAD_TR(RA[U], a_tr[U], BUF, H)                                                                    \
    }                                                                                                    \
  }
#define LOADB_U(RB, BUF, H, U)                                                                           \
  if constexpr ((U) < NTQ) {                                                                             \
    if constexpr (B_MODE == 0) {                                                                         \
      const char* base_ = smem + (BUF) * BUFB + 2 * HT + (H) * HT;                                       \
      RB[U][0] = *LDS_PTR(const h16x8, base_ + b_o0 + (U) * 2048);                                      \
      RB[U][1] = *LDS_PTR(const h16x8, base_ + b_o1 + (U) * 2048);                                      \
    } else {                                                                                             \
      LOAD_TR(RB[U], b_tr[U], BUF, H)                                                                    \
    }                                                                                                    \
  }
#define LOADA(RA, BUF, H) { LOADA_U(RA, BUF, H, 0) LOADA_U(RA, BUF, H, 1) LOADA_U(RA, BUF, H, 2) LOADA_U(RA, BUF, H, 3) }
#define LOADB(RB, BUF, H) { LOADB_U(RB, BUF, H, 0) LOADB_U(RB, BUF, H, 1) LOADB_U(RB, BUF, H, 2) LOADB_U(RB, BUF, H, 3) }

  f32x4 acc[8][2 * NTQ];

  h16x8 RA0[4][2], RA1[4][2], RB0[4][2], RB1[4][2];

  auto stage_first = [&](int h8) {
    const int t1 = nk > 1 ? 1 : 0;
    switch (h8) {
      case 0: issueA(0, 0, 0); break;
      case 1: issueB(0, 0, 0); break;
      case 2: issueB(1, 0, 0); break;
      case 3: issueA(1, 0, 0); break;
      case 4: issueA(0, 1, t1); break;
      case 5: issueB(1, 1, t1); break;
      case 6: issueB(0, 1, t1); break;
      default: issueA(1, 1, t1); break;
    }
  };
#pragma unroll
  for (int h8 = 0; h8 < 8; ++h8) stage_first(h8);

#define LOAD_TR_H(DST, ADDR, BUF, H, KS)                                                                 \
  {                                                                                                      \
    const uint32_t ad_ = (ADDR) + (BUF) * BUFB;                                                          \
    DST[KS] = cat_tr(tr16_asm<(H) * HT + (KS) * 8192>(ad_), tr16_asm<(H) * HT + (KS) * 8192 + 1024>(ad_)); \
  }
#define LOADA_UH(RA, BUF, H, U, KS)                                                                      \
  {                                                                                                      \
    if constexpr (A_MODE == 0) {                                                                         \
      const char* base_ = smem + (BUF) * BUFB + (H) * HT;                                                \
      RA[U][KS] = *LDS_PTR(const h16x8, base_ + ((KS) ? a_o1 : a_o0) + (U) * 2048);                     \
    } else {                                                                                             \
      LOAD_TR_H(RA[U], a_tr[U], BUF, H, KS)                                                              \
    }                                                                                                    \
  }
#define LOADB_UH(RB, BUF, H, U, KS)                                                                      \
  if constexpr ((U) < NTQ) {                                                                             \
    if constexpr (B_MODE == 0) {                                                                         \
      const char* base_ = smem + (BUF) * BUFB + 2 * HT + (H) * HT;                                       \
      RB[U][KS] = *LDS_PTR(const h16x8, base_ + ((KS) ? b_o1 : b_o0) + (U) * 2048);                     \
    } else {                                                                                             \
      LOAD_TR_H(RB[U], b_tr[U], BUF, H, KS)                                                              \
    }                                                                                                    \
  }
#define MMA1(KS, MT, NT, MB, NB, RA, RB)                                                   \
  if constexpr ((NT) < NTQ)                                                                \
    asm volatile(MFMA16_ASM " %0, %1, %2, %0"                                 \
                 : "+a"(acc[(MB) + (MT)][(NB) + (NT)])                                     \
                 : "v"(RA[MT][KS]), "v"(RB[NT][KS]));
#define GA(KS, MT, MB, NB, RA, RB, INS_A, INS_B)                                           \
    MMA1(KS, MT, 0, MB, NB, RA, RB) INS_A;                                                 \
    MMA1(KS, MT, 1, MB, NB, RA, RB) MMA1(KS, MT, 2, MB, NB, RA, RB) INS_B;                 \
    MMA1(KS, MT, 3, MB, NB, RA, RB)
#define PHASE_BODY_0(LOADUH, RN, LBUF, LH, PIECE, IH, IBUF, IT, MB, NB, RA, RB) \
    GA(0, 0, MB, NB, RA, RB, PIECE(IH, IBUF, IT, 0), LOADUH(RN, LBUF, LH, 0, 0)) \
    GA(0, 1, MB, NB, RA, RB, PIECE(IH, IBUF, IT, 1), LOADUH(RN, LBUF, LH, 1, 0)) \
    GA(0, 2, MB, NB, RA, RB, PIECE(IH, IBUF, IT, 2), LOADUH(RN, LBUF, LH, 2, 0)) \
    GA(0, 3, MB, NB, RA, RB, PIECE(IH, IBUF, IT, 3), LOADUH(RN, LBUF, LH, 3, 0)) \
    GA(1, 0, MB, NB, RA, RB, LOADUH(RN, LBUF, LH, 0, 1), LOADUH(RN, LBUF, LH, 1, 1)) \
    GA(1, 1, MB, NB, RA, RB, LOADUH(RN, LBUF, LH, 2, 1), LOADUH(RN, LBUF, LH, 3, 1)) \
    GA(1, 2, MB, NB, RA, RB, , )                                               \
    GA(1, 3, MB, NB, RA, RB, , )
#define PHASE_BODY_1(LOADUH, RN, LBUF, LH, PIECE, IH, IBUF, IT, MB, NB, RA, RB) \
    GA(0, 0, MB, NB, RA, RB, LOADUH(RN, LBUF, LH, 0, 0), LOADUH(RN, LBUF, LH, 1, 0)) \
    GA(0, 1, MB, NB, RA, RB, LOADUH(RN, LBUF, LH, 2, 0), LOADUH(RN, LBUF, LH, 3, 0)) \
    GA(0, 2, MB, NB, RA, RB, LOADUH(RN, LBUF, LH, 0, 1), LOADUH(RN, LBUF, LH, 1, 1)) \
    GA(0, 3, MB, NB, RA, RB, LOADUH(RN, LBUF, LH, 2, 1), LOADUH(RN, LBUF, LH, 3, 1)) \
    GA(1, 0, MB, NB, RA, RB, PIECE(IH, IBUF, IT, 0), )                         \
    GA(1, 1, MB, NB, RA, RB, PIECE(IH, IBUF, IT, 1), )                         \
    GA(1, 2, MB, NB, RA, RB, PIECE(IH, IBUF, IT, 2), )                         \
    GA(1, 3, MB, NB, RA, RB, PIECE(IH, IBUF, IT, 3), )
#define PHASE_BODY_2(LOADUH, RN, LBUF, LH, PIECE, IH, IBUF, IT, MB, NB, RA, RB) \
    GA(0, 0, MB, NB, RA, RB, PIECE(IH, IBUF, IT, 0), )                         \
    GA(0, 1, MB, NB, RA, RB, PIECE(IH, IBUF, IT, 1), )                         \
    GA(0, 2, MB, NB, RA, RB, PIECE(IH, IBUF, IT, 2), )                         \
    GA(0, 3, MB, NB, RA, RB, PIECE(IH, IBUF, IT, 3), )                         \
    GA(1, 0, MB, NB, RA, RB, LOADUH(RN, LBUF, LH, 0, 0), LOADUH(RN, LBUF, LH, 1, 0)) \
    GA(1, 1, MB, NB, RA, RB, LOADUH(RN, LBUF, LH, 2, 0), LOADUH(RN, LBUF, LH, 3, 0)) \
    GA(1, 2, MB, NB, RA, RB, LOADUH(RN, LBUF, LH, 0, 1), LOADUH(RN, LBUF, LH, 1, 1)) \
    GA(1, 3, MB, NB, RA, RB, LOADUH(RN, LBUF, LH, 2, 1), LOADUH(RN, LBUF, LH, 3, 1))
#define PHASE_BODY(...)                                                        \
    if constexpr (PH_ORDER == 0) { PHASE_BODY_0(__VA_ARGS__) }                 \
    else if constexpr (PH_ORDER == 1) { PHASE_BODY_1(__VA_ARGS__) }            \
    else { PHASE_BODY_2(__VA_ARGS__) }
#define PHASE(WAITN, WAITF, LOADUH, RN, LBUF, LH, PIECE, IH, IBUF, IT, MB, NB, RA, RB) \
  {                                                                            \
    __builtin_amdgcn_s_setprio(1);                                             \
    asm volatile("s_nop 1");                                                   \
    PHASE_BODY(LOADUH, RN, LBUF, LH, PIECE, IH, IBUF, IT, MB, NB, RA, RB)      \
    __builtin_amdgcn_s_setprio(0);                                             \
    if constexpr ((WAITF) != (WAITN)) { WAITBAR2(first, WAITF, WAITN); } else { WAITBAR(WAITN); } \
  }
#define HALF_A                                                                                       \
    PHASE(W32, CAPW(W32, 5), LOADB_UH, RB1, 0, 1, pieceA, 0, 0, t2, 0, 0, RA0, RB0)                   \
    PHASE(W23, CAPW(W23, 4), LOADA_UH, RA1, 0, 1, pieceB, 0, 0, t2, 0, NTQ, RA0, RB1)                 \
    PHASE(W23, CAPW(W23, 3), LOADA_UH, RA0, 1, 0, pieceB, 1, 0, t2, 4, NTQ, RA1, RB1)                 \
    PHASE(W32, CAPW(W32, 2), LOADB_UH, RB1, 1, 1, pieceA, 1, 0, t2, 4, 0, RA1, RB0)
#define NOLOAD_UH(R, BUF, H, U, KS)
#define HALF_A_LAST                                                                                  \
    PHASE(W32, CAPW(W32, 5), LOADB_UH, RB1, 0, 1, pieceA, 0, 0, t2, 0, 0, RA0, RB0)                   \
    PHASE(W23, CAPW(W23, 4), LOADA_UH, RA1, 0, 1, pieceB, 0, 0, t2, 0, NTQ, RA0, RB1)                 \
    PHASE(W23, CAPW(W23, 3), NOLOAD_UH, RA0, 1, 0, pieceB, 1, 0, t2, 4, NTQ, RA1, RB1)                \
    PHASE(W32, CAPW(W32, 2), NOLOAD_UH, RB1, 1, 1, pieceA, 1, 0, t2, 4, 0, RA1, RB0)
#define HALF_B                                                                                       \
    PHASE(W32, CAPW(W32, 1), LOADB_UH, RB0, 1, 0, pieceA, 0, 1, t3, 0, NTQ, RA0, RB1)                 \
    PHASE(W23, W23, LOADA_UH, RA1, 1, 1, pieceB, 1, 1, t3, 0, 0, RA0, RB0)                            \
    PHASE(W23, W23, LOADA_UH, RA0, 0, 0, pieceB, 0, 1, t3, 4, 0, RA1, RB0)                            \
    PHASE(W32, W32, LOADB_UH, RB0, 0, 0, pieceA, 1, 1, t3, 4, NTQ, RA1, RB1)
  bool behind_stores = false;
  while (true) {
    const int ln_ = lane_id_volatile();
    const int g = ln_ >> 4, l15 = ln_ & 15;
    int a_o0, a_o1, b_o0, b_o1;
    {
      const int fx = ((l15 >> 1) & 3) << 1;
      const int q = l15 >> 2, pp = l15 & 3, hk = q | ((g & 1) << 2);
      if constexpr (A_MODE == 0) {
        a_o0 = (wr * 64 + l15) * 128 + ((g ^ fx) << 4);
        a_o1 = (wr * 64 + l15) * 128 + (((4 + g) ^ fx) << 4);
      } else {
        a_o0 = (8 * g + q) * 256 + pp * 8;
        a_o1 = hk;
      }
      if constexpr (B_MODE == 0) {
        b_o0 = (wc * (NTQ * 16) + l15) * 128 + ((g ^ fx) << 4);
        b_o1 = (wc * (NTQ * 16) + l15) * 128 + (((4 + g) ^ fx) << 4);
      } else {
        b_o0 = (8 * g + q) * 256 + pp * 8;
        b_o1 = hk;
      }
    }
    uint32_t a_tr[4], b_tr[4];
    if constexpr (A_MODE == 1) {
  #pragma unroll
      for (int mt = 0; mt < 4; ++mt)
        a_tr[mt] = (uint32_t)(size_t)LDS_PTR(char, smem) + a_o0 + (((wr * 4 + mt) ^ a_o1) << 5);
    }
    if constexpr (B_MODE == 1) {
  #pragma unroll
      for (int nt = 0; nt < 4; ++nt)
        b_tr[nt] = (uint32_t)(size_t)LDS_PTR(char, smem) + 2 * HT + b_o0 + (((wc * 4 + nt) ^ b_o1) << 5);
    }
    const bool ovl = behind_stores;
    WAITBAR2(ovl, CAPW(3 * 4 + 3 * PB, 7), 3 * 4 + 3 * PB);
    LOADA(RA0, 0, 0)
    LOADB(RB0, 0, 0)
    WAITBAR2(ovl, CAPW(W32, 6), W32);
#pragma unroll
    for (int i = 0; i < 8; ++i)
#pragma unroll
      for (int j = 0; j < 2 * NTQ; ++j) acc[i][j] = f32x4{0.f, 0.f, 0.f, 0.f};

    int t = 0;
#pragma clang loop unroll(disable)
    for (; t + 1 < nk; t += 2) {
      const bool first = ovl && (t == 0);
      const int t2 = min(t + 2, nk - 1), t3 = min(t + 3, nk - 1);
      HALF_A
      HALF_B
    }
    if (t < nk) {
      const bool first = ovl && (t == 0);
      const int t2 = nk - 1;
      HALF_A_LAST
    }
    WAITBAR(0);
    asm volatile("s_nop 15\n\ts_nop 15" ::: "memory");

#if R256_ABLATE & 2
    const int em0 = 0, en0 = 0;
#else
    const int em0 = m0, en0 = n0;
#endif
    float* const eout = out_cur;
    const int eldo = ldo_cur, emvalid = mvalid_cur;
    int* sched_lds = reinterpret_cast<int*>(smem + 2 * BUFB + SCRATCH_BYTES);
    if (!dyn) {
      if (tid == 0) *sched_lds = (w + (int)gridDim.x < nwork) ? w + (int)gridDim.x : -1;
    } else if (tid == 0) {
      int wn = -1;
      const bool drew = pend_w < 0;
      if (!drew) {
        wn = pend_w;
        pend_w = -1;
      } else {
        auto tickets_of = [&](int x) { return (items_of(x) - static_of(x) + TICKET_ITEMS - 1) / TICKET_ITEMS; };
        auto take = [&](int x, unsigned int tk) {
          const int j = static_of(x) + TICKET_ITEMS * (int)tk;
          if (j < items_of(x)) {
            wn = x + 8 * j;
            if (TICKET_ITEMS == 2 && j + 1 < items_of(x)) pend_w = x + 8 * (j + 1);
          }
        };
        if (last_tk + 2 * static_of(xcd) < tickets_of(xcd)) {
          const unsigned int tk = atomicAdd(tickets + xcd, 1u);
          last_tk = (int)tk;
          take(xcd, tk);
        }
        for (int attempt = 0; attempt < 4 && wn < 0; ++attempt) {
          unsigned int cnt[8];
#pragma unroll
          for (int y = 0; y < 8; ++y) cnt[y] = __hip_atomic_load(tickets + y, __ATOMIC_RELAXED, __HIP_MEMORY_SCOPE_AGENT);
          int best = -1, best_left = 0;
#pragma unroll
          for (int y = 0; y < 8; ++y) {
            const int left = tickets_of(y) - (int)cnt[y];
            if (left > 0 && (y == xcd || (best != xcd && left > best_left))) { best = y; best_left = left; }
          }
          if (best < 0) break;
          const unsigned int tk = atomicAdd(tickets + best, 1u);
          if (best == xcd) last_tk = (int)tk;
          take(best, tk);
        }
      }
      *sched_lds = wn;
    }
    asm volatile("s_waitcnt vmcnt(0) lgkmcnt(0)\n\ts_barrier" ::: "memory");
    const int wnext = __builtin_amdgcn_readfirstlane(*reinterpret_cast<volatile int*>(sched_lds));
    const bool more = wnext >= 0;
    const int ez = cur_z, etl = cur_tl;
    if (more) setup(wnext);
    bool staged = false;
    if constexpr (SK) {
      if (p.splits > 1) {
        constexpr int SLAB = 256 * BNT * 4;
        constexpr int TNK = 2 * NTQ;
        char* const slabs = reinterpret_cast<char*>(p.sk_ws) + GEMM_SK_COUNTER_BYTES;
        const uint32_t voff = (uint32_t)lane_id_volatile() * 16u + (uint32_t)wave * 1024u;
        {
          char* const mine = slabs + ((size_t)etl * p.splits + ez) * SLAB;
#pragma unroll
          for (int i = 0; i < 8; ++i) {
            if (more) stage_first(i);
#pragma unroll
            for (int j = 0; j < TNK; ++j)
              asm volatile(R256_SGPR_PAD "global_store_dwordx4 %0, %1, %2 sc1" ::"v"(voff), "a"(acc[i][j]), "s"(mine + (i * TNK + j) * 4096) : "memory");
          }
        }
        asm volatile("s_waitcnt vmcnt(0) lgkmcnt(0)\n\ts_barrier" ::: "memory");
        if (tid == 0) {
          unsigned int* cnt = reinterpret_cast<unsigned int*>(p.sk_ws) + etl;
          const unsigned int old = __hip_atomic_fetch_add(cnt, 1u, __ATOMIC_RELAXED, __HIP_MEMORY_SCOPE_AGENT);
          if (old == (unsigned int)(p.splits - 1))
            __hip_atomic_store(cnt, 0u, __ATOMIC_RELAXED, __HIP_MEMORY_SCOPE_AGENT);
          sched_lds[1] = (int)old;
        }
        asm volatile("s_waitcnt vmcnt(0) lgkmcnt(0)\n\ts_barrier" ::: "memory");
        const int ticket = __builtin_amdgcn_readfirstlane(*reinterpret_cast<volatile int*>(sched_lds + 1));
        staged = more;
        if (ticket != p.splits - 1) {
          if (!more) break;
          behind_stores = false;
          w = wnext;
          continue;
        }
        const bool two = p.splits == 2;
        if (!two) {
#pragma unroll
          for (int i = 0; i < 8; ++i)
#pragma unroll
            for (int j = 0; j < TNK; ++j) acc[i][j] = f32x4{0.f, 0.f, 0.f, 0.f};
        }
        for (int zz = 0; zz < p.splits; ++zz) {
          if (two && zz == ez) continue;
          const char* const src = slabs + ((size_t)etl * p.splits + zz) * SLAB;
          f32x4 q[2][TNK];
#pragma unroll
          for (int j = 0; j < TNK; ++j)
            asm volatile(R256_SGPR_PAD "global_load_dwordx4 %0, %1, %2 sc1" : "=&v"(q[0][j]) : "v"(voff), "s"(src + j * 4096) : "memory");
#pragma unroll
          for (int i = 0; i < 8; ++i) {
            if (i + 1 < 8) {
#pragma unroll
              for (int j = 0; j < TNK; ++j)
                asm volatile(R256_SGPR_PAD "global_load_dwordx4 %0, %1, %2 sc1" : "=&v"(q[(i + 1) & 1][j]) : "v"(voff),
                             "s"(src + ((i + 1) * TNK + j) * 4096) : "memory");
              asm volatile("s_waitcnt vmcnt(%0)" ::"i"(TNK) : "memory");
            } else {
              asm volatile("s_waitcnt vmcnt(0)" ::: "memory");
            }
#pragma unroll
            for (int j = 0; j < TNK; ++j) {
              asm volatile("" : "+v"(q[i & 1][j]));
              acc[i][j] += q[i & 1][j];
            }
          }
        }
      }
    }
    if constexpr (EPI == EPI_F32_ATOMIC) {
      GemmParams pe = p;
      pe.out = eout;
      pe.ldo = eldo; pe.m_valid = emvalid;
      gemm_epilogue<8, TN, EPI, 2, 2, true>(acc, pe, smem + 2 * BUFB, em0, en0, wr * 128, wc * (NTQ * 32), wave, lane,
                                            [&](int step) { if (more) stage_first(step); }, more ? 4 : 0);
    } else {
      gemm_epilogue<8, TN, EPI, 2, 2, true>(acc, p, smem + 2 * BUFB, em0, en0, wr * 128, wc * (NTQ * 32), wave, lane,
                                            [&](int step) { if (more && !staged) stage_first(step); }, (more && !staged) ? 4 : 0);
    }
    if (!more) break;
    behind_stores = (em0 + 256 <= emvalid);
    w = wnext;
  }
#if R256_STAMP
  if (threadIdx.x == 0) {
    g_r256_stamp[2 * blockIdx.x] = __builtin_amdgcn_s_memtime() - st_c0;
    g_r256_stamp[2 * blockIdx.x + 1] = __builtin_amdgcn_s_memrealtime() - st_r0;
  }
#endif
#undef HALF_A
#undef HALF_A_LAST
#undef NOLOAD_UH
#undef HALF_B
#undef PHASE
#undef PHASE_BODY
#undef LOADA
#undef LOADB
#undef LOADA_U
#undef LOADB_U
#undef LOAD_TR
#undef LOAD_TR_H
#undef LOADA_UH
#undef LOADB_UH
#undef MMA1
#undef GA
#undef CAPW
}

struct RingSched {
  unsigned seq = 0;
  hipStream_t stream = nullptr;
  bool bound = false;
};
inline RingSched& ring_sched(int dev) {
  static RingSched s[64];
  return s[(dev >= 0 && dev < 64) ? dev : 0];
}

template <int A_MODE, int B_MODE, int EPI, int NTQ, bool SK>
int launch256_k(const GemmParams& p, hipStream_t st) {
  constexpr bool DYN = (R256_DYN != 0);
  constexpr int BNT = NTQ * 64;
  if ((p.M & 255) || (p.N % BNT) || (p.K & 63)) return VAULT_EINVAL;
  constexpr int LDS = 2 * BUFB + 4 * 16 * ((NTQ == 3 ? 96 : 64) + 4) * 4 + 16;
  auto kern = gemm256_kernel<A_MODE, B_MODE, EPI, NTQ, DYN, SK>;
  static bool attr_done[64] = {};
  int dev = 0;
  if (hipGetDevice(&dev) != hipSuccess || dev < 0 || dev >= 64) return VAULT_EINVAL;
  if (!attr_done[dev]) {
    hipError_t e = hipFuncSetAttribute(reinterpret_cast<const void*>(kern), hipFuncAttributeMaxDynamicSharedMemorySize, LDS);
    if (e != hipSuccess) return (int)e;
    attr_done[dev] = true;
  }
  GemmParams q = p;
  if (p.a_hm) {
    if (A_MODE != 0 || p.a_hm < p.M || p.batch > 1) return VAULT_EINVAL;
    q.lda = 64;
  }
  if (p.out_hm) return VAULT_EINVAL;
  q.gn = (p.gn > 0) ? std::min(p.gn, p.N / BNT) : p.N / BNT;
  const int nk_total = p.K >> 6;
  const int per = (nk_total + p.splits - 1) / p.splits;
  q.splits = (nk_total + per - 1) / per;
  if constexpr (SK) {
    const long long tiles = (long long)(p.M >> 8) * (p.N / BNT);
    if (q.splits > 1 && (p.sk_ws == nullptr || p.batch > 1 || tiles > GEMM_SK_MAX_TILES ||
                         p.sk_bytes < GEMM_SK_COUNTER_BYTES + tiles * q.splits * (256LL * BNT * 4)))
      return VAULT_EINVAL;
  }
  const int nwork = (p.M >> 8) * (p.N / BNT) * q.splits * ((EPI == EPI_F32_ATOMIC && p.batch > 1) ? p.batch : 1);
  dim3 grid(std::min(nwork, 256), 1, 1);
  int persist = p.persist & 0xff;
  int parity = 0;
  if (!DYN) persist &= ~1;
  if (persist & 1) {
    RingSched& rs = ring_sched(dev);
    if (!rs.bound) { rs.bound = true; rs.stream = st; }
    if (rs.stream == st) parity = (int)(rs.seq++ & 1u);
    else persist &= ~1;
  }
  q.persist = persist | (parity << 8);
  hipLaunchKernelGGL(kern, grid, dim3(256), LDS, st, q);
  return (int)hipGetLastError();
}

template <int A_MODE, int B_MODE, int EPI, int NTQ>
int launch256(const GemmParams& p, hipStream_t st) {
  constexpr bool SK_OK = A_MODE == 0 && NTQ == 3 && ((B_MODE == 1 && EPI == EPI_BF16) || (B_MODE == 0 && EPI == EPI_F32_RES));
  if (EPI != EPI_F32_ATOMIC && p.splits > 1) {
    if constexpr (SK_OK) return launch256_k<A_MODE, B_MODE, EPI, NTQ, true>(p, st);
    else return VAULT_EINVAL;
  }
  return launch256_k<A_MODE, B_MODE, EPI, NTQ, false>(p, st);
}

template <int NTQ>
int dispatch256(const GemmParams& p, int a_mode, int b_mode, int epi, hipStream_t st) {
  const int key = a_mode * 2 + b_mode;
#define VAULT_DISPATCH(AM, BMD)                                                       \
  switch (epi) {                                                                      \
    case EPI_BF16: return launch256<AM, BMD, EPI_BF16, NTQ>(p, st);                   \
    case EPI_BF16_GELU:                                                               \
      if (p.out2 != nullptr) return launch256<AM, BMD, EPI_BF16_GELU, NTQ>(p, st);    \
      else return launch256<AM, BMD, EPI_BF16_GELU_INF, NTQ>(p, st);                  \
    case EPI_BF16_DGELU: return launch256<AM, BMD, EPI_BF16_DGELU, NTQ>(p, st);       \
    case EPI_F32_RES: return launch256<AM, BMD, EPI_F32_RES, NTQ>(p, st);             \
    case EPI_F32_PATCH:             \
      if constexpr (BMD == 0) return launch256<AM, BMD, EPI_F32_PATCH, NTQ>(p, st);   \
      else return VAULT_EINVAL;                                                       \
    case EPI_F32_ATOMIC:                                                              \
      if constexpr (NTQ == 4) return launch256<AM, BMD, EPI_F32_ATOMIC, NTQ>(p, st);  \
      else return VAULT_EINVAL;                                                       \
    default: return VAULT_EINVAL;                                                     \
  }
  switch (key) {
    case 0: VAULT_DISPATCH(0, 0)
    case 1: VAULT_DISPATCH(0, 1)
    case 3:
      if constexpr (NTQ == 4) {
        if (epi == EPI_F32_ATOMIC) return launch256<1, 1, EPI_F32_ATOMIC, NTQ>(p, st);
      }
      return VAULT_EINVAL;
    default: return VAULT_EINVAL;
  }
#undef VAULT_DISPATCH
}

}

#if R256_DYN
#define R256_PUBLIC(NAME) NAME##_dyn
#else
#define R256_PUBLIC(NAME) NAME
int vault_gemm256_grouped_launch_dyn(const GemmParams& p, hipStream_t st);
int vault_gemm256_launch_dyn(const GemmParams& p, int a_mode, int b_mode, int epi, int ntq, hipStream_t st);
#endif

int R256_PUBLIC(vault_gemm256_grouped_launch)(const GemmParams& p, hipStream_t st) {
#if !R256_DYN
  if (p.persist & 1) return vault_gemm256_grouped_launch_dyn(p, st);
#endif
  if (p.nseg < 1 || p.nseg > 3 || (p.K & 63) || p.splits < 1) return VAULT_EINVAL;
  GemmParams q = p;
  int total = 0;
  for (int k = 0; k < p.nseg; ++k) {
    const GemmParams::Seg& g = p.seg[k];
    if (!g.A || !g.B || !g.out || g.tiles_n < 1 || g.tiles < g.tiles_n || g.tiles % g.tiles_n || g.count < 1 || g.first < 0 ||
        (g.lda & 7) || (g.ldb & 7) || (g.ldo & 3) || (g.batch_a & 7) || (g.batch_b & 7) || (g.batch_o & 3) ||
        (g.a_hm == 0 && g.lda < (g.tiles / g.tiles_n) * 256) || (g.a_hm != 0 && g.lda != 64) || g.ldb < g.tiles_n * 256 ||
        g.ldo < g.tiles_n * 256)
      return VAULT_EINVAL;
    total += g.count;
  }
  for (int k = p.nseg; k < 3; ++k) q.seg[k] = GemmParams::Seg{};
  q.A = p.seg[0].A; q.B = p.seg[0].B; q.out = p.seg[0].out;
  q.M = 256; q.N = 256; q.lda = p.seg[0].lda; q.ldb = p.seg[0].ldb; q.ldo = p.seg[0].ldo; q.m_valid = 256;
  q.batch = 0; q.gn = 1;
  constexpr int LDS = 2 * BUFB + 4 * 16 * (64 + 4) * 4 + 16;
  auto kern = gemm256_kernel<1, 1, EPI_F32_ATOMIC, 4, (R256_DYN != 0)>;
  static bool attr_done[64] = {};
  int dev = 0;
  if (hipGetDevice(&dev) != hipSuccess || dev < 0 || dev >= 64) return VAULT_EINVAL;
  if (!attr_done[dev]) {
    hipError_t e = hipFuncSetAttribute(reinterpret_cast<const void*>(kern), hipFuncAttributeMaxDynamicSharedMemorySize, LDS);
    if (e != hipSuccess) return (int)e;
    attr_done[dev] = true;
  }
  const int nk_total = p.K >> 6;
  const int per = (nk_total + p.splits - 1) / p.splits;
  q.splits = (nk_total + per - 1) / per;
  const int nwork = total * q.splits;
  int persist = p.persist & 0xff, parity = 0;
  if (!R256_DYN) persist &= ~1;
  if (persist & 1) {
    RingSched& rs = ring_sched(dev);
    if (!rs.bound) { rs.bound = true; rs.stream = st; }
    if (rs.stream == st) parity = (int)(rs.seq++ & 1u);
    else persist &= ~1;
  }
  q.persist = persist | (parity << 8);
  hipLaunchKernelGGL(kern, dim3(std::min(nwork, 256)), dim3(256), LDS, st, q);
  return (int)hipGetLastError();
}

int R256_PUBLIC(vault_gemm256_launch)(const GemmParams& p, int a_mode, int b_mode, int epi, int ntq, hipStream_t st) {
#if !R256_DYN
  if (p.persist & 1) return vault_gemm256_launch_dyn(p, a_mode, b_mode, epi, ntq, st);
#endif
  if (ntq == 2) {
    if (a_mode == 0 && b_mode == 0 && epi == EPI_F32_RES) return launch256<0, 0, EPI_F32_RES, 2>(p, st);
    if (a_mode == 0 && b_mode == 1 && epi == EPI_BF16) return launch256<0, 1, EPI_BF16, 2>(p, st);
    return VAULT_EINVAL;
  }
  return ntq == 3 ? dispatch256<3>(p, a_mode, b_mode, epi, st) : dispatch256<4>(p, a_mode, b_mode, epi, st);
}
```

vault_amd/engine.py:

```python
from __future__ import annotations

import math
import os
from typing import Dict, List, Optional, Tuple

import torch

from . import ops
from .backward import BackwardMixin
from .heads import HeadsMixin
from .ops import Drop, NO_DROP
from .params import ParamStore, _LayerNames, _in_format, _pad
from .spec import VaultSpec
from .staging import StagingMixin


class VaultEngine(StagingMixin, HeadsMixin, BackwardMixin):

    DEFAULT_HALF = "fp16"
    WGRAD_TARGET_WGS = 768
    LM_WGRAD_BATCHED = True
    LM_WGRAD_GROUP = 6
    STAGE_MAX_ROWS = 8192
    LM_BIAS_PARTIALS = False
    QKV_BIAS_SHORTCUT = True
    GELU8 = True
    GRAD_STREAM_BF16 = True
    WGRAD_STREAM_MAX_ROWS = 16384
    WGRAD_BATCH_MAX_ROWS = 131072
    PRUNE_LAST_LAYER = True
    PRUNE_MIN_ROWS = 16384

    def __init__(self, spec: VaultSpec, device="cuda:0", state=None, seed: int = 0, freeze_lm: bool = False,
                 with_grads: bool = True, classifier_dropout: float = 0.1, fp8_forward: bool = False,
                 half: Optional[str] = None, grad_scale_pow2: Optional[float] = None):
        self.spec, self.device = spec, torch.device(device)
        if half is None:
            half = "bf16" if fp8_forward else self.DEFAULT_HALF
        if half not in ops.HALF_DTYPE:
            raise ValueError("half must be 'bf16' or 'fp16'")
        self.half, self.hdt = half, ops.HALF_DTYPE[half]
        if fp8_forward and half != "bf16":
            raise ValueError("the fp8-forward mode quantises bf16 operands: half must be 'bf16'")
        self.grad_scale = float(grad_scale_pow2) if grad_scale_pow2 is not None else (4096.0 if half == "fp16" else 1.0)
        if self.grad_scale <= 0 or math.frexp(self.grad_scale)[0] != 0.5:
            raise ValueError("grad_scale_pow2 must be a power of two")
        self.fp8_forward = fp8_forward
        self._w8: Dict[str, tuple] = {}
        self.freeze_lm = freeze_lm and spec.lm is not None
        self.classifier_dropout = classifier_dropout
        if spec.vilt.hidden_size % 256 or (spec.lm and spec.lm.hidden_size != spec.vilt.hidden_size):
            raise ValueError("hidden size must be a multiple of 256 and equal for LM and ViLT")
        if spec.vilt.hidden_size // spec.vilt.num_attention_heads != 64:
            raise ValueError("head dimension must be 64")
        with torch.cuda.device(self.device):
            self.params = ParamStore(spec, self.device, state, seed, self.freeze_lm, with_grads, half=half)
        self.vl = [_LayerNames(f"encoder.layer.{i}", "vilt") for i in range(spec.vilt.num_hidden_layers)]
        self.ll = ([_LayerNames(f"bert.encoder.layer.{i}", "bert") for i in range(spec.lm.num_hidden_layers)]
                   if spec.lm else [])
        if with_grads:
            stacks = [self.vl] + ([self.ll] if (self.ll and not self.freeze_lm) else [])
            with torch.cuda.device(self.device):
                self.params.enable_transposed([[getattr(ln, k) for ln in st] for st in stacks for k in ("ow", "fw")])
        self._ws: Dict[tuple, dict] = {}
        self.keep_layer_outputs = False
        self._sel_cache: Dict[tuple, dict] = {}
        self.drop_seed = 0
        self.last: Optional[dict] = None
        self._wgrad_stream, self._wgrad_pending = None, False
        self._wgrad_side = False
        self._wgrad_items = 0
        self.adopt_pixel_patches = False
        self.dp_world = 1
        self._grads_zero = False
        self._g_dirty = False
        self._g_stale_key = None
        self._stored_ranges: List[Tuple[int, int]] = []
        self.profile_events: Optional[Dict[str, list]] = None
        self._e0: Dict[str, torch.cuda.Event] = {}
        self.census_on = os.environ.get("VAULT_H16_CENSUS") == "1"
        if os.environ.get("VAULT_PRUNE_LAST_LAYER") == "0":
            self.PRUNE_LAST_LAYER = False
        self.census: Dict[str, Dict[str, dict]] = {}

    def _prof_begin(self, site: str, stream=None):
        if self.profile_events is not None and site in self.profile_events:
            e0 = torch.cuda.Event(enable_timing=True)
            e0.record(stream)
            self._e0[site] = e0

    def _prof_end(self, site: str, flops: float = 0.0, stream=None):
        if self.profile_events is not None and site in self.profile_events:
            e1 = torch.cuda.Event(enable_timing=True)
            e1.record(stream)
            self.profile_events[site].append((self._e0[site], e1, flops))

    def _run_census(self, ws: dict, phase: str):
        if not self.census_on or ops.taping():
            return
        import re
        skip_u = ws.get("gelu8_active") is not None
        names = [k for k, t in ws.items() if isinstance(k, str) and isinstance(t, torch.Tensor) and t.dtype == self.hdt
                 and not k.endswith("_all") and not (skip_u and re.fullmatch(r"(pl_)?u\d*", k))]
        seen, todo = set(), []
        for k in sorted(names):
            key = (ws[k].data_ptr(), ws[k].numel())
            if key not in seen and ws[k].is_contiguous():
                seen.add(key)
                todo.append(k)
        cnt = torch.zeros((max(1, len(todo)), 4), dtype=torch.int64, device=self.device)
        for j, k in enumerate(todo):
            ops.h16_census(ws[k], cnt[j])
        host = cnt.cpu().tolist()
        self.census[phase] = {k: dict(saturated=host[j][0], nonfinite=host[j][1], subnormal=host[j][2], zero=host[j][3],
                                      n=ws[k].numel()) for j, k in enumerate(todo)}

    def _buf(self, ws, name, shape, dtype):
        t = ws.get(name)
        if t is None:
            t = torch.zeros(shape, dtype=dtype, device=self.device)
            ws[name] = t
        return t

    def _stack(self, ws, base, n, shape, dtype):
        key = base + "_all"
        t = ws.get(key)
        if t is None:
            t = torch.zeros((n,) + tuple(shape), dtype=dtype, device=self.device)
            ws[key] = t
            for i in range(n):
                ws[f"{base}{i}"] = t[i]
        return t

    MAX_RAGGED_WORKSPACES = 2

    def workspace(self, B: int, T: int, train: bool, geom: Tuple[int, int, int] = (0, 0, 0), tag: int = 0) -> dict:
        key = (B, T, train) + tuple(geom) + (tag,)
        if key not in self._ws:
            if geom != (0, 0, 0):
                old = [k for k in self._ws if len(k) == 7 and k[3:6] != (0, 0, 0)]
                while len(old) >= self.MAX_RAGGED_WORKSPACES:
                    self._ws.pop(old.pop(0))
            self._ws[key] = {"B": B, "T": T, "key": key}
        return self._ws[key]

    def _sk_ws(self):
        if not self.SPLITK:
            return None
        t = self._ws.get("splitk_ws")
        if t is None:
            t = torch.zeros(self.SPLITK_WS_BYTES, dtype=torch.uint8, device=self.device)
            self._ws["splitk_ws"] = t
        return t

    def _fp8_scratch(self, M, K):
        key = ("fp8_a", M, K)
        if key not in self._ws:
            self._ws[key] = (torch.empty(M * K, dtype=torch.uint8, device=self.device),
                             torch.empty(M * (K // 32), dtype=torch.uint8, device=self.device))
        return self._ws[key]

    def _fp8_refresh_weights(self):
        P = self.params
        if "fp8_flat" not in self._ws:
            self._ws["fp8_flat"] = (torch.empty(P.n_total, dtype=torch.uint8, device=self.device),
                                    torch.empty(P.n_total // 32, dtype=torch.uint8, device=self.device))
        pq, psc = self._ws["fp8_flat"]
        for stack in (self.ll, self.vl):
            spans = []
            for ln in stack:
                for wname in ((ln.qw, ln.iw, ln.fw) if self.FFN_OUT_FP8 else (ln.qw, ln.iw)):
                    o, shp = P.offsets[wname]
                    N = 3 * shp[0] if wname == ln.qw else shp[0]
                    K = shp[1]
                    if N % 256 or K % 128:
                        continue
                    spans.append((o, o + N * K))
                    if wname not in self._w8:
                        self._w8[wname] = (pq[o:o + N * K], psc[o // 32:(o + N * K) // 32])
            if spans:
                lo, hi = min(a for a, _ in spans), max(b for _, b in spans)
                ops.quant_mxfp8(P.pb[lo:], (hi - lo) // 64, 64, 64, pq[lo:], psc[lo // 32:])

    @staticmethod
    def _keep_hi(split3: torch.Tensor, plain: torch.Tensor, K: int):
        ops.pycall(lambda: plain.copy_(split3[:, :K]))

    def _cfg_like(self, key, plan, M, like):
        key = ("cfg_like",) + key + (M, like, ops.GEMM_SCHED)
        if key not in self._ws:
            c = plan(like, -1)
            self._ws[key] = c if (c >= 0 and plan(M, c) == c) else -1
        return self._ws[key]

    def _linear(self, a_bf16, wname, out, M, N, K, epi, m_valid, bias=None, precise=False, ldo=None, prequant=False,
                emit_q=False, like=None, **kw):
        P = self.params
        if precise:
            ops.gemm(a_bf16, P.wb3(wname, N, K), out, M, N, 3 * K, 3 * K, 3 * K, N if ldo is None else ldo, 0, 0, epi,
                     m_valid=m_valid, bias=bias, **kw)
        elif (self.fp8_forward and wname in self._w8 and M % 256 == 0 and prequant is not False
              and self._fp8_kernel_ok(M, N, K, epi, out, bias, kw)):
            wq, wsc = self._w8[wname]
            aq, asc = self._fp8_scratch(M, K)
            if prequant is None:
                ops.quant_mxfp8(a_bf16, M, K, K, aq, asc)
            kw.pop("split3", None)
            if emit_q:
                oq, osc = self._fp8_scratch(M, N)
                key = ("emit_q", M, N, K, epi, kw.get("cfg", -1), bool(kw.get("aux_u8")))
                if key not in self._ws:
                    self._ws[key] = ops.gemm_mxfp8(aq, asc, wq, wsc, out, M, N, K, N, epi, m_valid=m_valid, bias=bias, out_q=oq,
                                                   out_scale=osc, plan_only=True, **{k: v for k, v in kw.items() if k != "drop"}) == 5
                emit_q = self._ws[key]
                if emit_q:
                    kw.update(out_q=oq, out_scale=osc)
            ops.gemm_mxfp8(aq, asc, wq, wsc, out, M, N, K, N, epi, m_valid=m_valid, bias=bias, **kw)
            return emit_q
        else:
            w = P.wb(wname, n_elems=N * K, shape=(N, K))
            if like is not None and "cfg" not in kw:
                kwl = dict(kw, splitk_ws=self._sk_ws()) if (epi == ops.EPI_F32_RES and K >= 1536) else kw
                kw["cfg"] = self._cfg_like(("lin", wname, epi), lambda m, c: ops.gemm(
                    a_bf16, w, out, m, N, K, K, K, N if ldo is None else ldo, 0, 0, epi, m_valid=m, bias=bias, cfg=c,
                    plan_only=True, **(kwl if c < 0 else kw)), M, like)
            elif epi == ops.EPI_F32_RES and K >= 1536:
                kw.setdefault("splitk_ws", self._sk_ws())
            ops.gemm(a_bf16, w, out, M, N, K, K, K, N if ldo is None else ldo,
                     0, 0, epi, m_valid=m_valid, bias=bias, **kw)

    def _fp8_kernel_ok(self, M, N, K, epi, out, bias, kw) -> bool:
        if epi != ops.EPI_F32_RES:
            return True
        drop = kw.get("drop", NO_DROP)
        key = ("fp8_ok", M, N, K, epi, bool(drop.thresh))
        if key not in self._ws:
            self._ws[key] = ops.gemm_mxfp8(out, out, out, out, out, M, N, K, N, epi, bias=bias, res=kw.get("res"), drop=drop,
                                           plan_only=True) in (5, 6)
        return self._ws[key]

    def _dgrad(self, dy_bf16, wname, out, M, Kin, Nout, epi, m_valid, like=None, **kw):
        P = self.params
        wt = P.pbT.get(wname)
        if wt is not None and M % 256 == 0:
            if like is not None and "cfg" not in kw:
                kw["cfg"] = self._cfg_like(("dgrad", wname, epi), lambda m, c: ops.gemm(
                    dy_bf16, wt, out, m, Kin, Nout, Nout, Nout, Kin, 0, 0, epi, m_valid=m, cfg=c, plan_only=True, **kw), M, like)
            ops.gemm(dy_bf16, wt, out, M, Kin, Nout, Nout, Nout, Kin, 0, 0, epi, m_valid=m_valid, **kw)
            return
        w = P.wb(wname, n_elems=Nout * Kin, shape=(Nout, Kin))
        if like is not None and "cfg" not in kw and M % 256 == 0:
            kwl = dict(kw, splitk_ws=self._sk_ws()) if (epi == ops.EPI_BF16 and Nout >= 1536) else kw
            kw["cfg"] = self._cfg_like(("dgrad", wname, epi), lambda m, c: ops.gemm(
                dy_bf16, w, out, m, Kin, Nout, Nout, Kin, Kin, 0, 1, epi, m_valid=m, cfg=c, plan_only=True,
                **(kwl if c < 0 else kw)), M, like)
        elif epi == ops.EPI_BF16 and Nout >= 1536:
            kw.setdefault("splitk_ws", self._sk_ws())
        ops.gemm(dy_bf16, w, out, M, Kin, Nout, Nout, Kin, Kin, 0, 1, epi, m_valid=m_valid, **kw)


    FFN_OUT_FP8 = False
    HEAD_MAJOR = True
    HEAD_MAJOR_MIN_ROWS = 16384
    SPLITK = True
    SPLITK_WS_BYTES = 16384 + (64 << 20)
    WGRAD_BESIDE_LM_ITEMS = 0
    WGRAD_SIDE_ITEMS = 224

    def _plan_gelu8(self, ws, n2, act, u, ln, Mp, M):
        mode = (bool(self.fp8_forward), ops.GEMM_SCHED, self.GELU8)
        if ws.get("gelu8_mode") == mode:
            return ws["gelu8_cfg"]
        ws["gelu8_mode"] = mode
        P, H, FF = self.params, ws["H"], ws["FF"]
        cfg, wt = None, P.pbT.get(ln.fw)
        if self.GELU8 and u is not None and wt is not None and Mp % 256 == 0:
            if self.fp8_forward:
                c1 = (ops.gemm_mxfp8(n2, n2, n2, n2, act, Mp, FF, H, FF, ops.EPI_BF16_GELU, m_valid=M, bias=P.w(ln.ib), out2=u,
                                     aux_u8=True, plan_only=True) if ln.iw in self._w8 else -1)
            else:
                c1 = ops.gemm(n2, P.wb(ln.iw, n_elems=FF * H, shape=(FF, H)), act, Mp, FF, H, H, H, FF, 0, 0,
                              ops.EPI_BF16_GELU, m_valid=M, bias=P.w(ln.ib), out2=u, aux_u8=True, plan_only=True)
            c2 = ops.gemm(n2, wt, act, Mp, FF, H, H, H, FF, 0, 0, ops.EPI_BF16_DGELU, m_valid=M, aux=u,
                          colsum=P.gr(ln.ib), aux_u8=True, plan_only=True)
            if c1 in (5, 6) and c1 == c2:
                cfg = c1
        ws["gelu8_cfg"] = cfg
        return cfg

    def _plan_head_major(self, ws, key, a16, wname, rows_pad, rows, S, pr, train):
        mode = (bool(self.fp8_forward), ops.GEMM_SCHED, bool(pr), bool(train), self.HEAD_MAJOR)
        if ws.get(key + "_mode") == mode:
            return ws[key]
        ws[key + "_mode"] = mode
        P, H, FF = self.params, ws["H"], ws["FF"]
        hm = 0
        if (self.HEAD_MAJOR and not pr and S <= 192 and rows_pad % 256 == 0 and H % 256 == 0 and FF % 256 == 0
                and self.HEAD_MAJOR_MIN_ROWS <= rows_pad <= self.WGRAD_BATCH_MAX_ROWS):
            w = P.wb(wname, n_elems=3 * H * H, shape=(3 * H, H))
            qb = P.w(wname.replace("weight", "bias"), n_elems=3 * H, shape=(3 * H,))
            if self.fp8_forward:
                c1 = (ops.gemm_mxfp8(a16, a16, a16, a16, a16, rows_pad, 3 * H, H, 3 * H, ops.EPI_BF16, m_valid=rows, bias=qb,
                                     out_hm=rows_pad, plan_only=True) if wname in self._w8 else -1)
            else:
                c1 = ops.gemm(a16, w, a16, rows_pad, 3 * H, H, H, H, 3 * H, 0, 0, ops.EPI_BF16, m_valid=rows, bias=qb,
                              out_hm=rows_pad, plan_only=True)
            ok = c1 in (5, 6)
            if ok and train:
                c2 = ops.gemm(a16, w, a16, rows_pad, H, 3 * H, 3 * H, H, H, 0, 1, ops.EPI_BF16, m_valid=rows, a_hm=rows_pad,
                              plan_only=True)
                ok = c2 in (3, 4, 8) and self.LM_WGRAD_BATCHED and P.gr(wname) is not None
            if ok:
                hm = rows_pad
        ws[key] = hm
        return hm

    def _use_stage(self, rows_pad: int, pr: bool) -> bool:
        if pr or self.fp8_forward:
            return False
        return rows_pad <= self.STAGE_MAX_ROWS

    def _stage_layer_args(self, ws, ln, style, i, rows, rows_pad, S, keymask, x_in, x_out, bufs, drops=None,
                          x_in_bf16=None, x_out_bf16=None):
        P = self.params
        H, FF, heads, B = ws["H"], ws["FF"], ws["heads"], ws["B"]
        eps = self.spec.vilt.layer_norm_eps if style == "vilt" else self.spec.lm.layer_norm_eps
        kw = dict(B=B, S=S, H=H, FF=FF, heads=heads, rows=rows, rows_pad=rows_pad, eps=eps,
                  wqkv=P.wb(ln.qw, n_elems=3 * H * H, shape=(3 * H, H)), wo=P.wb(ln.ow), wi=P.wb(ln.iw), wf=P.wb(ln.fw),
                  wo_t=P.pbT.get(ln.ow), wf_t=P.pbT.get(ln.fw),
                  bqkv=P.w(ln.qb, n_elems=3 * H, shape=(3 * H,)), bo=P.w(ln.ob), bi=P.w(ln.ib), bf=P.w(ln.fb),
                  ln1w=P.w(ln.ln1w), ln1b=P.w(ln.ln1b), ln2w=P.w(ln.ln2w), ln2b=P.w(ln.ln2b),
                  x_in=x_in, x_out=x_out, x_in_bf16=x_in_bf16, x_out_bf16=x_out_bf16, keymask=keymask, **bufs)
        sk = self._sk_ws()
        if sk is not None:
            kw.update(splitk_ws=sk, splitk_bytes=sk.numel())
        if drops is not None:
            da, dh = drops
            kw.update(attn_drop_thresh=da.thresh, attn_drop_scale=da.scale, hid_drop_thresh=dh.thresh, hid_drop_scale=dh.scale,
                      drop_seed=self.drop_seed & 0xFFFFFFFF, drop_stream_base=16 * i)
        a = ops.layer_args(**{k: v for k, v in kw.items() if v is not None})
        ws[f"stage_{style}{i}"] = a
        return a

    def _drop(self, p: float, stream: int, train: bool) -> Drop:
        return Drop(p, self.drop_seed, stream) if (train and p > 0.0) else NO_DROP

    def forward(self, batch: Dict[str, torch.Tensor], train: bool = False, labels: Optional[torch.Tensor] = None,
                need_hidden: bool = True, loss_scale: Optional[float] = None,
                precise: bool = False, ws_tag: int = 0, image_token_type_idx: int = 1,
                advance_seed: bool = True) -> Dict[str, torch.Tensor]:
        with torch.cuda.device(self.device):
            return self._forward(batch, train, labels, need_hidden, loss_scale, precise, ws_tag, image_token_type_idx,
                                 advance_seed)

    def _forward(self, batch, train, labels, need_hidden, loss_scale, precise=False, ws_tag=0, image_type_idx=1,
                 advance_seed=True):
        if not 0 < image_type_idx < self.spec.vilt.modality_type_vocab_size:
            raise ValueError("image_token_type_idx outside the modality type table")
        ws = self.stage_inputs(batch, train, labels, ws_tag=ws_tag)
        ws["img_type"] = image_type_idx
        if train and advance_seed:
            self.drop_seed = (self.drop_seed + 1) & 0xFFFFFFFF
        if precise:
            self.params.ensure_split3()
        return self.forward_staged(ws, need_hidden, loss_scale, precise)

    @_in_format
    def forward_staged(self, ws: dict, need_hidden: bool = True, loss_scale: Optional[float] = None,
                       precise: bool = False):
        spec, P = self.spec, self.params
        v = spec.vilt
        train = ws["train"]
        B, T, S, Mp, H, NP = (ws[k] for k in ("B", "T", "S", "Mp", "H", "NP"))
        ids, tt, pix, labels, km = ws["ids"], ws["tt"], ws["pix"], ws["labels"], ws["keymask"]
        buf = lambda name, shape, dtype=torch.float32: self._buf(ws, name, shape, dtype)
        bf = self.hdt
        ws["drop_seed"] = self.drop_seed
        pr = precise
        W3 = 3 if pr else 1
        if pr:
            if train:
                self.params._pb3_fresh = False
            self.params.ensure_split3()
        if self.fp8_forward and not pr:
            self._fp8_refresh_weights()

        Ml, Mlp = B * T, _pad(B * T)
        ws.update(Ml=Ml, Mlp=Mlp)
        if spec.lm is not None:
            ws["lm_y"], ws["lm_yb"] = self._lm_forward(ws, pr, buf, bf)
            text_src = ws["lm_y"][-1]
            use_pos = spec.use_vilt_position_embeddings
            tables = [(P.w("embeddings.text_embeddings.token_type_embeddings.weight"), tt if tt is not None else 0)]
        else:
            ws["lm_y"] = ws["lm_yb"] = None
            text_src = ws.get("txt_embeds")
            use_pos = True
            tables = [(P.w("embeddings.text_embeddings.token_type_embeddings.weight"), tt if tt is not None else 0),
                      None if text_src is not None else (P.w("embeddings.text_embeddings.word_embeddings.weight"), ids)]
        if use_pos:
            tables.append((P.w("embeddings.text_embeddings.position_embeddings.weight"), "mod"))
        ws["use_pos"] = use_pos

        nv = v.num_hidden_layers
        x = [buf(f"x{i}" if (train or self.keep_layer_outputs) else f"x{i % 2}", (Mp, H)) for i in range(nv + 1)]
        vsum = buf("vt_sum", (Mlp, H))
        ops.gather_sum(text_src, vsum, tables, Ml, H, period=T)
        mt = P.w("embeddings.token_type_embeddings.weight")
        ops.layernorm_fwd(vsum, P.w("embeddings.text_embeddings.LayerNorm.weight"),
                          P.w("embeddings.text_embeddings.LayerNorm.bias"), v.layer_norm_eps, Ml, H, y_f32=x[0],
                          ymap=(T, S, 0), post_add=mt[0], mean=buf("vt_mean", (Mlp,)), rstd=buf("vt_rstd", (Mlp,)))
        Kp = v.num_channels * v.patch_size * v.patch_size
        Mpp = _pad(B * NP)
        ws.update(Kp=Kp, Mpp=Mpp)
        if ws.get("img_embeds") is not None:
            ops.rows_add(ws["img_embeds"], mt[ws.get("img_type", 1)], x[0], B * NP, H, NP, S, T)
        else:
            self._patch_embed_forward(ws, x, mt, pix, pr, W3, Kp, Mpp, buf, bf)
        return self._forward_encoder(ws, x, need_hidden, loss_scale, pr, W3, labels, km, train, buf, bf)

    def _ln_y16(self, ws, pr, y16, name, shape):
        return y16 if not pr else (self._buf(ws, name, shape, self.hdt) if ws["train"] else None)

    def _ffn_forward(self, ws, a16, ln, pre, sfx, rows, rows_pad, res, out, u, act, pr, prequant, drop=NO_DROP, g8=None,
                     like=None):
        P, H, FF, bf, W3, pt = self.params, ws["H"], ws["FF"], self.hdt, (3 if pr else 1), pr and ws["train"]
        ops.pycall(lambda: self._prof_begin("ffn1"))
        u_out = self._buf(ws, f"{pre}u{sfx}_3", (rows_pad, W3 * FF), bf) if (pt and u is not None) else u
        actq = self._linear(a16, ln.iw, act, rows_pad, FF, H, ops.EPI_BF16_GELU, rows, bias=P.w(ln.ib), out2=u_out, precise=pr,
                            split3=pr, ldo=W3 * FF, prequant=prequant, emit_q=self.FFN_OUT_FP8, like=like,
                            **(dict(cfg=g8, aux_u8=True) if g8 is not None else {}))
        if pt:
            self._keep_hi(act, self._buf(ws, f"{pre}act{sfx}", (rows_pad, FF), bf), FF)
            if u is not None:
                self._keep_hi(u_out, u, FF)
        ops.pycall(lambda: self._prof_end("ffn1", 2.0 * rows * FF * H * W3))
        self._linear(act, ln.fw, out, rows_pad, H, FF, ops.EPI_F32_RES, rows, bias=P.w(ln.fb), res=res, drop=drop, precise=pr,
                     prequant=bool(actq), like=like)
        return bool(actq)

    def _lm_forward(self, ws, pr, buf, bf):
        P, lm, train, ids, tt, amf = self.params, self.spec.lm, ws["train"], ws["ids"], ws["tt"], ws["amf"]
        B, T, H, FF, heads, Ml, Mlp = (ws[k] for k in ("B", "T", "H", "FF", "heads", "Ml", "Mlp"))
        W3, pt = (3 if pr else 1), pr and train
        lm_tt = ws["lm_tt"] = tt if (tt is not None and lm.type_vocab_size >= 2) else 0
        pos = buf("lm_pos", (B, T), torch.int32)
        ops.position_ids(ids, pos, B, T, 1 if lm.kind == "roberta" else 0, lm.pad_token_id)
        esum = buf("lm_esum", (Mlp, H))
        te = ws.get("txt_embeds")
        ops.gather_sum(te, esum, [None if te is not None else (P.w("bert.embeddings.word_embeddings.weight"), ids),
                                  (P.w("bert.embeddings.position_embeddings.weight"), pos),
                                  (P.w("bert.embeddings.token_type_embeddings.weight"), lm_tt)], Ml, H)
        keep = train and not self.freeze_lm
        nl = lm.num_hidden_layers
        if keep and self.LM_WGRAD_BATCHED and H % 128 == 0 and FF % 128 == 0:
            self._stack(ws, "lm_yb", nl + 1, (Mlp, H), bf)
            for base, width in (("lm_ctx", H), ("lm_y1b", H), ("lm_act", FF)):
                self._stack(ws, base, nl, (Mlp, width), bf)
        ybn = [f"lm_yb{i}" if keep else f"lm_yb{i % 2}" for i in range(nl + 1)]
        y = [buf(f"lm_y{i}" if keep else f"lm_y{i % 2}", (Mlp, H)) for i in range(nl + 1)]
        yb = [buf(n + ("_3" if pr else ""), (Mlp, W3 * H), bf) for n in ybn]
        lm_train = train
        pdh, pda = lm.hidden_dropout_prob, lm.attention_probs_dropout_prob
        q8l = self._fp8_scratch(Mlp, H) if (self.fp8_forward and not pr and Mlp % 256 == 0) else (None, None)
        ops.layernorm_fwd(esum, P.w("bert.embeddings.LayerNorm.weight"), P.w("bert.embeddings.LayerNorm.bias"),
                          lm.layer_norm_eps, Ml, H, y_f32=y[0], y_bf16=self._ln_y16(ws, pr, yb[0], ybn[0], (Mlp, H)),
                          y_split3=yb[0] if pr else None, mean=buf("lm_emean", (Mlp,)),
                          rstd=buf("lm_erstd", (Mlp,)), drop=self._drop(pdh, 1, lm_train),
                          y_q=q8l[0], y_scale=q8l[1])
        lm_stage = ws["lm_stage"] = self._use_stage(Mlp, pr)
        ops.pycall(lambda: self._prof_begin("lm_fwd"))
        for i, ln in enumerate(self.ll):
            sfx = f"{i}" if keep else ""
            qkv = buf(f"lm_qkv{sfx}", (Mlp, 3 * H), bf)
            p3 = "_3" if pr else ""
            ctx = buf(f"lm_ctx{sfx}{p3}", (Mlp, W3 * H), bf)
            lse = buf(f"lm_lse{sfx}", (B, heads, T))
            h1 = buf(f"lm_h1{sfx}", (Mlp, H)); y1 = buf(f"lm_y1{sfx}", (Mlp, H))
            y1b = buf(f"lm_y1b{sfx}{p3}", (Mlp, W3 * H), bf)
            u = buf(f"lm_u{sfx}", (Mlp, FF), bf) if keep else None
            act = buf(f"lm_act{sfx}{p3}", (Mlp, W3 * FF), bf)
            h2 = buf(f"lm_h2{sfx}", (Mlp, H))
            if lm_stage:
                ws["lm_qkv_hm"], ws["lm_qkv_hm_mode"] = 0, None
                da, dh = self._drop(pda, 16 * i + 2, lm_train), self._drop(pdh, 16 * i + 3, lm_train)
                a = self._stage_layer_args(
                    ws, ln, "lm", i, Ml, Mlp, T, amf, y[i], y[i + 1],
                    dict(qkv=qkv, ctx=ctx, lse=lse, xm=h1, y1=y1, n2=y1b, act=act, u=u, h2=h2,
                         m1=buf(f"lm_m1{sfx}", (Mlp,)), r1=buf(f"lm_r1{sfx}", (Mlp,)),
                         m2=buf(f"lm_m2{sfx}", (Mlp,)), r2=buf(f"lm_r2{sfx}", (Mlp,))),
                    drops=(da, dh), x_in_bf16=yb[i], x_out_bf16=yb[i + 1])
                ops.layer_call("vault_lm_layer_fwd", a, seeded=bool(da.thresh or dh.thresh))
                continue
            lhm = self._plan_head_major(ws, "lm_qkv_hm", yb[i], ln.qw, Mlp, Ml, T, pr, keep)
            self._linear(yb[i], ln.qw, qkv, Mlp, 3 * H, H, ops.EPI_BF16, Ml,
                         bias=P.w(ln.qb, n_elems=3 * H, shape=(3 * H,)), precise=pr, prequant=q8l[0] is not None,
                         **(dict(out_hm=lhm) if lhm else {}))
            ops.attention_fwd(qkv, amf, None if pr else ctx, lse, B, T, H, heads,
                              drop=self._drop(pda, 16 * i + 2, lm_train), ctx_split3=ctx if pr else None, qkv_hm=lhm)
            if pt:
                self._keep_hi(ctx, buf(f"lm_ctx{sfx}", (Mlp, H), bf), H)
            self._linear(ctx, ln.ow, h1, Mlp, H, H, ops.EPI_F32_RES, Ml, bias=P.w(ln.ob), res=y[i],
                         drop=self._drop(pdh, 16 * i + 3, lm_train), precise=pr)
            ops.layernorm_fwd(h1, P.w(ln.ln1w), P.w(ln.ln1b), lm.layer_norm_eps, Ml, H, y_f32=y1,
                              y_bf16=self._ln_y16(ws, pr, y1b, f"lm_y1b{sfx}", (Mlp, H)), y_split3=y1b if pr else None,
                              mean=buf(f"lm_m1{sfx}", (Mlp,)), rstd=buf(f"lm_r1{sfx}", (Mlp,)),
                              y_q=q8l[0], y_scale=q8l[1])
            self._ffn_forward(ws, y1b, ln, "lm_", sfx, Ml, Mlp, y1, h2, u, act, pr, q8l[0] is not None or None,
                              drop=self._drop(pdh, 16 * i + 4, lm_train))
            ops.layernorm_fwd(h2, P.w(ln.ln2w), P.w(ln.ln2b), lm.layer_norm_eps, Ml, H, y_f32=y[i + 1],
                              y_bf16=self._ln_y16(ws, pr, yb[i + 1], ybn[i + 1], (Mlp, H)), y_split3=yb[i + 1] if pr else None,
                              mean=buf(f"lm_m2{sfx}", (Mlp,)), rstd=buf(f"lm_r2{sfx}", (Mlp,)),
                              y_q=q8l[0], y_scale=q8l[1])
        ops.pycall(lambda: self._prof_end("lm_fwd"))
        return y, ([buf(n, (Mlp, H), bf) for n in ybn] if pt else yb)

    def _patch_embed_forward(self, ws, x, mt, pix, pr, W3, Kp, Mpp, buf, bf):
        spec, P = self.spec, self.params
        v = spec.vilt
        B, T, S, H, NP = (ws[k] for k in ("B", "T", "S", "H", "NP"))
        apatch = buf("apatch_3" if pr else "apatch", (Mpp, W3 * Kp), bf)
        if ws.get("patches_in"):
            apatch = ws["apatch_in"]
        addtab = buf("addtab", (NP, H))
        wpn = "embeddings.patch_embeddings.projection.weight"
        if ws["ragged"]:
            ops.im2col_sel(pix, apatch, ws["sel"], B, NP, v.num_channels, ws["HP"], ws["WP"], v.patch_size, split3=pr)
            if pr and ws["train"]:
                ops.im2col_sel(pix, buf("apatch", (Mpp, Kp), bf), ws["sel"], B, NP, v.num_channels, ws["HP"], ws["WP"], v.patch_size)
            ops.image_sel_consts(P.w("embeddings.patch_embeddings.projection.bias"), P.w("embeddings.position_embeddings"),
                                 mt[ws.get("img_type", 1)], P.w("embeddings.cls_token"), addtab, x[0], NP, H, B, S, T)
        else:
            if ws.get("patches_in"):
                if pr:
                    raise ValueError("pixel_patches carry bf16 pixels: the precise (split-bf16) mode needs pixel_values")
            else:
                ops.im2col(pix, apatch, B, v.num_channels, v.image_size, v.patch_size, split3=pr)
                if pr and ws["train"]:
                    ops.im2col(pix, buf("apatch", (Mpp, Kp), bf), B, v.num_channels, v.image_size, v.patch_size)
                ev = ws.get("pixels_consumed")
                if ev is None:
                    ev = ws["pixels_consumed"] = torch.cuda.Event()
                ops.pycall(lambda ev=ev: ev.record(torch.cuda.current_stream()))
            ops.image_consts(P.w("embeddings.patch_embeddings.projection.bias"), P.w("embeddings.position_embeddings"),
                             mt[ws.get("img_type", 1)], P.w("embeddings.cls_token"), addtab, x[0], NP, H, B, S, T)
        ops.gemm(apatch, P.wb3(wpn, H, Kp) if pr else P.wb(wpn, shape=(H, Kp)), x[0], Mpp, H, W3 * Kp, W3 * Kp, W3 * Kp,
                 H, 0, 0, ops.EPI_F32_PATCH, m_valid=B * NP, addtab=addtab, rpg=NP, gstride=S, goff=T + 1)
        if ws["ragged"]:
            ops.image_pos_sel_fwd(x[0], P.w("embeddings.position_embeddings"), ws["sel"], ws["hw"], B, NP, S, T, H,
                                  ws["gw"], v.image_size // v.patch_size)

    def _plan_prune(self, ws, need_hidden, pr) -> bool:
        return bool(self.PRUNE_LAST_LAYER and self.spec.add_pooling_layer and not need_hidden and not self.keep_layer_outputs
                    and not pr and not self.fp8_forward and not self._use_stage(ws["Mp"], pr)
                    and ws["Mp"] >= self.PRUNE_MIN_ROWS and ws["S"] <= 192 and len(self.vl) > 0)

    def _vilt_last_layer_pruned(self, ws, x, i, km, train, buf, bf):
        P, v, ln = self.params, self.spec.vilt, self.vl[i]
        B, S, M, Mp, H, FF, heads = (ws[k] for k in ("B", "S", "M", "Mp", "H", "FF", "heads"))
        Bp = ws["Bp"] = _pad(B)
        sfx, like = (f"{i}" if train else ""), Mp
        n1, qkv, lse = buf(f"n1{sfx}", (Mp, H), bf), buf(f"qkv{sfx}", (Mp, 3 * H), bf), buf(f"lse{sfx}", (B, heads, S))
        ws["vilt_stage"] = False
        ops.layernorm_fwd(x[i], P.w(ln.ln1w), P.w(ln.ln1b), v.layer_norm_eps, M, H, y_bf16=n1,
                          mean=buf(f"m1{sfx}", (Mp,)), rstd=buf(f"r1{sfx}", (Mp,)))
        vhm = self._plan_head_major(ws, "qkv_hm", n1, ln.qw, Mp, M, S, False, train)
        self._linear(n1, ln.qw, qkv, Mp, 3 * H, H, ops.EPI_BF16, M, bias=P.w(ln.qb, n_elems=3 * H, shape=(3 * H,)),
                     **(dict(out_hm=vhm) if vhm else {}))
        ctx, xres, xm = buf("pl_ctx", (Bp, H), bf), buf("pl_xres", (Bp, H)), buf("pl_xm", (Bp, H))
        ops.attention_fwd(qkv, km, ctx, lse, B, S, H, heads, qkv_hm=vhm, q_rows=1)
        ops.rows_gather_bwd(x[i], xres, None, B, H, 1, S, 0)
        self._linear(ctx, ln.ow, xm, Bp, H, H, ops.EPI_F32_RES, B, bias=P.w(ln.ob), res=xres, like=like)
        n2 = buf("pl_n2", (Bp, H), bf)
        ops.layernorm_fwd(xm, P.w(ln.ln2w), P.w(ln.ln2b), v.layer_norm_eps, B, H, y_bf16=n2,
                          mean=buf("pl_m2", (Bp,)), rstd=buf("pl_r2", (Bp,)))
        u, act = (buf("pl_u", (Bp, FF), bf) if train else None), buf("pl_act", (Bp, FF), bf)
        g8 = self._plan_gelu8(ws, n2, act, u, ln, Mp, M)
        if g8 is not None and ws.get("pl_gelu8_of") != (g8, ops.GEMM_SCHED):
            wt = P.pbT.get(ln.fw)
            c1 = ops.gemm(n2, P.wb(ln.iw, n_elems=FF * H, shape=(FF, H)), act, Bp, FF, H, H, H, FF, 0, 0, ops.EPI_BF16_GELU,
                          m_valid=B, bias=P.w(ln.ib), out2=u, aux_u8=True, cfg=g8, plan_only=True)
            c2 = ops.gemm(n2, wt, act, Bp, FF, H, H, H, FF, 0, 0, ops.EPI_BF16_DGELU, m_valid=B, aux=u, colsum=P.gr(ln.ib),
                          aux_u8=True, cfg=g8, plan_only=True)
            ws["pl_gelu8_of"], ws["pl_gelu8_ok"] = (g8, ops.GEMM_SCHED), (c1 == g8 and c2 == g8)
        g8 = g8 if (g8 is not None and ws["pl_gelu8_ok"]) else None
        ws["pl_gelu8"] = g8
        self._ffn_forward(ws, n2, ln, "pl_", "", B, Bp, xm, buf("pl_xout", (Bp, H)), u, act, False, None, g8=g8, like=like)

    def _forward_encoder(self, ws, x, need_hidden, loss_scale, pr, W3, labels, km, train, buf, bf):
        spec, P = self.spec, self.params
        v = spec.vilt
        B, S, M, Mp, H, FF, heads = (ws[k] for k in ("B", "S", "M", "Mp", "H", "FF", "heads"))
        nv = v.num_hidden_layers
        pt = pr and train
        if (train and self.LM_WGRAD_BATCHED and Mp <= self.WGRAD_BATCH_MAX_ROWS and H % 128 == 0
                and FF % 128 == 0):
            for base, width in (("n1", H), ("ctx", H), ("n2", H), ("act", FF)):
                self._stack(ws, base, nv, (Mp, width), bf)
        prune = ws["pruned_last"] = self._plan_prune(ws, need_hidden, pr)
        ops.pycall(lambda: self._prof_begin("vilt_fwd"))
        for i, ln in enumerate(self.vl):
            if prune and i == nv - 1:
                self._vilt_last_layer_pruned(ws, x, i, km, train, buf, bf)
                continue
            sfx = f"{i}" if train else ""
            p3 = "_3" if pr else ""
            n1 = buf(f"n1{sfx}{p3}", (Mp, W3 * H), bf); qkv = buf(f"qkv{sfx}", (Mp, 3 * H), bf)
            ctx = buf(f"ctx{sfx}{p3}", (Mp, W3 * H), bf); lse = buf(f"lse{sfx}", (B, heads, S))
            xm = buf(f"xm{sfx}", (Mp, H)); n2 = buf(f"n2{sfx}{p3}", (Mp, W3 * H), bf)
            u = buf(f"u{sfx}", (Mp, FF), bf) if train else None
            act = buf(f"act{sfx}{p3}", (Mp, W3 * FF), bf)
            if self._use_stage(Mp, pr):
                ws["vilt_stage"] = True
                ws["qkv_hm"], ws["qkv_hm_mode"] = 0, None
                a = self._stage_layer_args(
                    ws, ln, "vilt", i, M, Mp, S, km, x[i], x[i + 1],
                    dict(n1=n1, qkv=qkv, ctx=ctx, lse=lse, xm=xm, n2=n2, act=act, u=u, m1=buf(f"m1{sfx}", (Mp,)),
                         r1=buf(f"r1{sfx}", (Mp,)), m2=buf(f"m2{sfx}", (Mp,)), r2=buf(f"r2{sfx}", (Mp,))))
                ops.layer_call("vault_vilt_layer_fwd", a)
                continue
            ws["vilt_stage"] = False
            q8 = self._fp8_scratch(Mp, H) if (self.fp8_forward and not pr and Mp % 256 == 0) else (None, None)
            ops.layernorm_fwd(x[i], P.w(ln.ln1w), P.w(ln.ln1b), v.layer_norm_eps, M, H,
                              y_bf16=self._ln_y16(ws, pr, n1, f"n1{sfx}", (Mp, H)), y_split3=n1 if pr else None,
                              mean=buf(f"m1{sfx}", (Mp,)), rstd=buf(f"r1{sfx}", (Mp,)),
                              y_q=q8[0], y_scale=q8[1])
            vhm = self._plan_head_major(ws, "qkv_hm", n1, ln.qw, Mp, M, S, pr, train)
            self._linear(n1, ln.qw, qkv, Mp, 3 * H, H, ops.EPI_BF16, M, bias=P.w(ln.qb, n_elems=3 * H, shape=(3 * H,)),
                         precise=pr, prequant=q8[0] is not None, **(dict(out_hm=vhm) if vhm else {}))
            ops.attention_fwd(qkv, km, None if pr else ctx, lse, B, S, H, heads, ctx_split3=ctx if pr else None, qkv_hm=vhm)
            if pt:
                self._keep_hi(ctx, buf(f"ctx{sfx}", (Mp, H), bf), H)
            self._linear(ctx, ln.ow, xm, Mp, H, H, ops.EPI_F32_RES, M, bias=P.w(ln.ob), res=x[i], precise=pr)
            ops.layernorm_fwd(xm, P.w(ln.ln2w), P.w(ln.ln2b), v.layer_norm_eps, M, H,
                              y_bf16=self._ln_y16(ws, pr, n2, f"n2{sfx}", (Mp, H)), y_split3=n2 if pr else None,
                              mean=buf(f"m2{sfx}", (Mp,)), rstd=buf(f"r2{sfx}", (Mp,)),
                              y_q=q8[0], y_scale=q8[1])
            g8 = None if pr else self._plan_gelu8(ws, n2, act, u, ln, Mp, M)
            ws["gelu8_active"] = g8
            self._ffn_forward(ws, n2, ln, "", sfx, M, Mp, xm, x[i + 1], u, act, pr, q8[0] is not None or None, g8=g8)
        ops.pycall(lambda: self._prof_end("vilt_fwd"))
        out: Dict[str, torch.Tensor] = {}
        xl = x[nv]
        lw, lb = P.w("layernorm.weight"), P.w("layernorm.bias")
        if need_hidden:
            hid = buf("last_hidden", (Mp, H))
            ops.layernorm_fwd(xl, lw, lb, v.layer_norm_eps, M, H, y_f32=hid, mean=buf("f_mean_all", (Mp,)),
                              rstd=buf("f_rstd_all", (Mp,)))
            out["last_hidden_state"] = hid[:M].view(B, S, H)
        if spec.add_pooling_layer:
            Bp = _pad(B)
            ws["Bp"] = Bp
            h0b = buf("h0b_3" if pr else "h0b", (Bp, W3 * H), bf)
            ops.layernorm_fwd(ws["pl_xout"] if prune else xl, lw, lb, v.layer_norm_eps, B, H,
                              y_bf16=self._ln_y16(ws, pr, h0b, "h0b", (Bp, H)), y_split3=h0b if pr else None,
                              xmap=(0, 0, 0) if prune else (1, S, 0), mean=buf("f_mean", (Bp,)), rstd=buf("f_rstd", (Bp,)))
            pre = buf("pool_pre", (Bp, H))
            self._linear(h0b, "pooler.dense.weight", pre, Bp, H, H, ops.EPI_F32_RES, B, bias=P.w("pooler.dense.bias"),
                         precise=pr)
            pooled = buf("pooled", (Bp, H))
            if spec.n_classes > 0 and spec.head == "mlp":
                ops.head_fwd(pre, None, None, None, pooled, None, None, B, H, 0, 0.0)
                if spec.num_images == 1:
                    out["logits"] = self._mlp_forward(ws, pooled, B)
            elif spec.n_classes > 0:
                C = spec.n_classes
                logits = buf("logits", (B, C))
                loss = buf("loss", (1,))
                ops.pycall(loss.zero_)
                hd = self._drop(self.classifier_dropout, 9001, train)
                ops.head_fwd(pre, P.w("classifier.1.weight"), P.w("classifier.1.bias"), labels, pooled, logits,
                             loss if labels is not None else None, B, H, C,
                             (1.0 / B) if loss_scale is None else loss_scale, drop=hd)
                out["logits"] = logits if C > 1 else logits.view(B)
                if labels is not None:
                    out["loss"] = loss
            else:
                ops.head_fwd(pre, None, None, None, pooled, None, None, B, H, 0, 0.0)
            out["pooler_output"] = pooled[:B]
        ws["x"] = x
        self.last = ws
        self._run_census(ws, "forward")
        return out
```

vault_amd/ops.py:

```python
from __future__ import annotations

import contextvars
import ctypes as C
from typing import Optional

import torch

from . import lib as L

EPI_BF16, EPI_BF16_GELU, EPI_BF16_DGELU, EPI_F32_RES, EPI_F32_PATCH, EPI_F32_ATOMIC = range(6)


class LnFwdArgs(C.Structure):
    _fields_ = [("x", C.c_void_p), ("gamma", C.c_void_p), ("beta", C.c_void_p), ("post_add", C.c_void_p),
                ("y_bf16", C.c_void_p), ("y_f32", C.c_void_p), ("mean", C.c_void_p), ("rstd", C.c_void_p),
                ("rows", C.c_int), ("H", C.c_int), ("eps", C.c_float),
                ("x_rpg", C.c_int), ("x_gstride", C.c_int), ("x_goff", C.c_int),
                ("y_rpg", C.c_int), ("y_gstride", C.c_int), ("y_goff", C.c_int),
                ("drop_thresh", C.c_uint32), ("drop_seed", C.c_uint32), ("drop_stream", C.c_uint32),
                ("drop_scale", C.c_float), ("y_split3", C.c_void_p), ("y_q", C.c_void_p), ("y_scale", C.c_void_p)]


class LnBwdArgs(C.Structure):
    _fields_ = [("dy_bf16", C.c_void_p), ("dy_f32", C.c_void_p), ("x", C.c_void_p), ("mean", C.c_void_p),
                ("rstd", C.c_void_p), ("gamma", C.c_void_p), ("dres", C.c_void_p),
                ("dx_f32", C.c_void_p), ("dx_bf16", C.c_void_p), ("dgamma", C.c_void_p), ("dbeta", C.c_void_p),
                ("rows", C.c_int), ("H", C.c_int),
                ("dy_rpg", C.c_int), ("dy_gstride", C.c_int), ("dy_goff", C.c_int),
                ("x_rpg", C.c_int), ("x_gstride", C.c_int), ("x_goff", C.c_int),
                ("dx_rpg", C.c_int), ("dx_gstride", C.c_int), ("dx_goff", C.c_int),
                ("drop_thresh", C.c_uint32), ("drop_seed", C.c_uint32), ("drop_stream", C.c_uint32),
                ("drop_scale", C.c_float), ("drop_on_dy", C.c_int), ("dbias", C.c_void_p), ("dres_bf16", C.c_void_p)]


class AttnArgs(C.Structure):
    _fields_ = [("qkv", C.c_void_p), ("keymask", C.c_void_p), ("ctx", C.c_void_p), ("lse", C.c_void_p),
                ("dctx", C.c_void_p), ("dqkv", C.c_void_p),
                ("B", C.c_int), ("S", C.c_int), ("H", C.c_int), ("heads", C.c_int),
                ("drop_thresh", C.c_uint32), ("drop_seed", C.c_uint32), ("drop_stream", C.c_uint32),
                ("drop_scale", C.c_float), ("ctx_split3", C.c_void_p), ("qkv_hm", C.c_int),
                ("bias_partials", C.c_void_p), ("bias_thirds", C.c_int), ("q_rows", C.c_int)]


def _p(t: Optional[torch.Tensor]):
    return None if t is None else t.data_ptr()


_FMT: contextvars.ContextVar = contextvars.ContextVar("vault_operand_format", default="bf16")
HALF_DTYPE = {"bf16": torch.bfloat16, "fp16": torch.float16}


class operand_format:

    def __init__(self, fmt: str):
        if fmt not in HALF_DTYPE:
            raise ValueError("operand format must be 'bf16' or 'fp16'")
        self.fmt = fmt

    def __enter__(self):
        self._token = _FMT.set(self.fmt)
        return self

    def __exit__(self, *exc):
        _FMT.reset(self._token)
        return False


def current_format() -> str:
    return _FMT.get()


def _h(t: Optional[torch.Tensor]):
    if t is None:
        return None
    fmt = _FMT.get()
    if t.dtype != HALF_DTYPE[fmt] and t.dtype in (torch.bfloat16, torch.float16):
        raise TypeError(f"{t.dtype} operand in a launch on the {fmt} library")
    return t.data_ptr()


class Tape:

    def __init__(self):
        self.calls = []
        self.seeded = []
        self.rebind_range = None
        self.rebinds = []

    def rebind(self, base: int):
        for s, f, off in self.rebinds:
            setattr(s, f, base + off)

    def replay(self, seed: Optional[int] = None):
        if seed is not None:
            sd = seed & 0xFFFFFFFF
            for a in self.seeded:
                a.drop_seed = sd
        for fn, args in self.calls:
            rc = fn(*args)
            if isinstance(rc, int) and rc != 0:
                raise RuntimeError(f"{getattr(fn, '__name__', fn)} failed with code {rc} during replay")


_TAPE: Optional[Tape] = None


def start_tape() -> Tape:
    global _TAPE
    _TAPE = Tape()
    return _TAPE


def stop_tape() -> Optional[Tape]:
    global _TAPE
    t, _TAPE = _TAPE, None
    return t


def taping() -> bool:
    return _TAPE is not None


def pycall(fn):
    global _TAPE
    t = _TAPE
    if t is not None:
        t.calls.append((fn, ()))
    _TAPE = None
    try:
        fn()
    finally:
        _TAPE = t


def _invoke(name: str, *args, struct=None, drop=None):
    fn = getattr(L.load(_FMT.get()), name)
    if _TAPE is not None:
        _TAPE.calls.append((fn, args))
        if struct is not None and drop is not None and drop.thresh:
            _TAPE.seeded.append(struct)
    L.check(fn(*args), name)


def _stream():
    return C.c_void_p(torch.cuda.current_stream().cuda_stream)


class Drop:

    __slots__ = ("thresh", "seed", "stream", "scale")

    def __init__(self, p: float = 0.0, seed: int = 0, stream: int = 0):
        self.thresh = 0 if p <= 0.0 else min(int(p * 4294967296.0), 4294967295)
        self.seed = seed & 0xFFFFFFFF
        self.stream = stream & 0xFFFFFFFF
        self.scale = 1.0 if p <= 0.0 else 1.0 / (1.0 - p)


NO_DROP = Drop()


def _set_drop(a, drop: Drop):
    a.drop_thresh, a.drop_seed, a.drop_stream, a.drop_scale = drop.thresh, drop.seed, drop.stream, drop.scale


GEMM_SCHED = 0


def gemm(A, B, out, M, N, K, lda, ldb, ldo, a_mode, b_mode, epi, *, cfg=-1, m_valid=0, splits=1, accumulate=0,
         bias=None, res=None, aux=None, out2=None, addtab=None, rpg=0, gstride=0, goff=0, drop: Drop = NO_DROP,
         colsum=None, split3=False, batch=0, batch_a=0, batch_b=0, batch_o=0, aux_u8=False, plan_only=False, out_hm=0, a_hm=0,
         splitk_ws=None):
    a = L.GemmArgs()
    if splitk_ws is not None:
        a.splitk_ws, a.splitk_bytes = _p(splitk_ws), splitk_ws.numel() * splitk_ws.element_size()
    a.aux_u8 = 1 if aux_u8 else 0
    a.out_hm, a.a_hm = int(out_hm), int(a_hm)
    a.A, a.B, a.out, a.out2 = _h(A), _h(B), _h(out), _h(out2)
    a.bias, a.res, a.aux, a.addtab = _p(bias), _p(res), _h(aux), _p(addtab)
    a.colsum = _p(colsum)
    a.split3 = 1 if split3 else 0
    a.M, a.N, a.K, a.lda, a.ldb, a.ldo, a.m_valid = M, N, K, lda, ldb, ldo, m_valid
    a.a_mode, a.b_mode, a.epi, a.cfg, a.splits, a.accumulate = a_mode, b_mode, epi, cfg, splits, accumulate
    a.rpg, a.gstride, a.goff = rpg, gstride, goff
    a.persist = GEMM_SCHED
    a.batch, a.batch_a, a.batch_b, a.batch_o = batch, batch_a, batch_b, batch_o
    _set_drop(a, drop)
    if plan_only:
        return int(L.load(_FMT.get()).vault_gemm_plan(C.byref(a)))
    if _TAPE is not None and _TAPE.rebind_range is not None:
        lo, hi = _TAPE.rebind_range
        for f in ("A", "B"):
            p = getattr(a, f) or 0
            if lo <= p < hi:
                _TAPE.rebinds.append((a, f, p - lo))
    _invoke("vault_gemm", C.byref(a), _stream(), struct=a, drop=drop)


class WgradSeg(C.Structure):
    _fields_ = [("dy", C.c_void_p), ("x", C.c_void_p), ("dw", C.c_void_p),
                ("n_out", C.c_int), ("n_in", C.c_int), ("ld_dy", C.c_int), ("ld_x", C.c_int), ("ld_dw", C.c_int),
                ("batch", C.c_int), ("first", C.c_int), ("count", C.c_int),
                ("batch_dy", C.c_longlong), ("batch_x", C.c_longlong), ("batch_dw", C.c_longlong), ("dy_hm", C.c_int)]


class WgradGroupedArgs(C.Structure):
    _fields_ = [("nseg", C.c_int), ("seg", WgradSeg * 3), ("tokens", C.c_int), ("splits", C.c_int), ("accumulate", C.c_int),
                ("persist", C.c_int)]


def wgrad_grouped(segs, tokens, splits=1, accumulate=1):
    a = WgradGroupedArgs()
    a.nseg, a.tokens, a.splits, a.accumulate, a.persist = len(segs), tokens, splits, accumulate, GEMM_SCHED
    for k, g in enumerate(segs):
        t = a.seg[k]
        t.dy, t.x, t.dw = _h(g["dy"]), _h(g["x"]), _p(g["dw"])
        t.n_out, t.n_in, t.ld_dy, t.ld_x, t.ld_dw = g["n_out"], g["n_in"], g["n_out"], g["n_in"], g["n_in"]
        t.batch, t.first, t.count = g["batch"], g["first"], g["count"]
        t.batch_dy, t.batch_x, t.batch_dw = g["batch_dy"], g["batch_x"], g["batch_dw"]
        t.dy_hm = int(g.get("dy_hm", 0))
    _invoke("vault_wgrad_grouped", C.byref(a), _stream(), struct=a)


def quant_mxfp8(src_bf16, rows, K, ld, dst_q, dst_scale):
    _invoke("vault_quant_mxfp8", C.c_void_p(_p(src_bf16)), C.c_longlong(rows), C.c_int(K), C.c_int(ld),
            C.c_void_p(_p(dst_q)), C.c_void_p(_p(dst_scale)), _stream())


def gemm_mxfp8(Aq, As, Bq, Bs, out, M, N, K, ldo, epi, *, m_valid=0, bias=None, res=None, out2=None,
               drop: Drop = NO_DROP, cfg=-1, aux_u8=False, out_hm=0, out_q=None, out_scale=None, plan_only=False):
    a = L.GemmArgs()
    a.out_q, a.out_scale = _p(out_q), _p(out_scale)
    a.A, a.B, a.out, a.out2 = _p(Aq), _p(Bq), _p(out), _p(out2)
    a.bias, a.res = _p(bias), _p(res)
    a.M, a.N, a.K, a.lda, a.ldb, a.ldo, a.m_valid = M, N, K, K, K, ldo, m_valid
    a.a_mode, a.b_mode, a.epi, a.cfg, a.splits, a.accumulate = 0, 0, epi, cfg, 1, 0
    a.aux_u8, a.out_hm = int(bool(aux_u8)), int(out_hm)
    a.persist = GEMM_SCHED
    _set_drop(a, drop)
    if plan_only:
        return int(L.load(_FMT.get()).vault_gemm_mxfp8_plan(C.byref(a)))
    _invoke("vault_gemm_mxfp8", C.byref(a), C.c_void_p(_p(As)), C.c_void_p(_p(Bs)), _stream(), struct=a, drop=drop)


def layernorm_fwd(x, gamma, beta, eps, rows, H, *, y_bf16=None, y_f32=None, mean=None, rstd=None, post_add=None,
                  xmap=(0, 0, 0), ymap=(0, 0, 0), drop: Drop = NO_DROP, y_split3=None, y_q=None, y_scale=None):
    a = LnFwdArgs()
    a.x, a.gamma, a.beta, a.post_add = _p(x), _p(gamma), _p(beta), _p(post_add)
    a.y_bf16, a.y_f32, a.mean, a.rstd = _h(y_bf16), _p(y_f32), _p(mean), _p(rstd)
    a.rows, a.H, a.eps = rows, H, eps
    a.x_rpg, a.x_gstride, a.x_goff = xmap
    a.y_rpg, a.y_gstride, a.y_goff = ymap
    _set_drop(a, drop)
    a.y_split3 = _h(y_split3)
    a.y_q, a.y_scale = _p(y_q), _p(y_scale)
    _invoke("vault_layernorm_fwd", C.byref(a), _stream(), struct=a, drop=drop)


def layernorm_bwd(x, mean, rstd, gamma, rows, H, *, dy_bf16=None, dy_f32=None, dres=None, dx_f32=None, dx_bf16=None,
                  dgamma=None, dbeta=None, dymap=(0, 0, 0), xmap=(0, 0, 0), dxmap=(0, 0, 0), drop: Drop = NO_DROP,
                  drop_on_dy: bool = False, dbias=None, dres_bf16=None):
    a = LnBwdArgs()
    a.dres_bf16 = _h(dres_bf16)
    a.dy_bf16, a.dy_f32, a.x, a.mean, a.rstd, a.gamma, a.dres = (_h(dy_bf16), _p(dy_f32), _p(x), _p(mean),
                                                                  _p(rstd), _p(gamma), _p(dres))
    a.dx_f32, a.dx_bf16, a.dgamma, a.dbeta = _p(dx_f32), _h(dx_bf16), _p(dgamma), _p(dbeta)
    a.rows, a.H = rows, H
    a.dy_rpg, a.dy_gstride, a.dy_goff = dymap
    a.x_rpg, a.x_gstride, a.x_goff = xmap
    a.dx_rpg, a.dx_gstride, a.dx_goff = dxmap
    _set_drop(a, drop)
    a.drop_on_dy = 1 if drop_on_dy else 0
    a.dbias = _p(dbias)
    _invoke("vault_layernorm_bwd", C.byref(a), _stream(), struct=a, drop=drop)


def colsum_batched(x_bf16, ld, rows, N, out, batch, batch_in, batch_out):
    _invoke("vault_colsum_batched", C.c_void_p(_p(x_bf16)), C.c_int(ld), C.c_int(rows), C.c_int(N), C.c_void_p(_p(out)),
            C.c_int(batch), C.c_longlong(batch_in), C.c_longlong(batch_out), _stream())


def colsum_hm(x_bf16, rows, hm_rows, planes, out, batch=1, batch_in=0, batch_out=0):
    _invoke("vault_colsum_hm", C.c_void_p(_h(x_bf16)), C.c_int(rows), C.c_int(hm_rows), C.c_int(planes), C.c_void_p(_p(out)),
            C.c_int(batch), C.c_longlong(batch_in), C.c_longlong(batch_out), _stream())


def colsum(x_bf16, ld, rows, N, out):
    _invoke("vault_colsum", C.c_void_p(_p(x_bf16)), C.c_int(ld), C.c_int(rows), C.c_int(N), C.c_void_p(_p(out)), _stream())


def _attn_args(qkv, keymask, ctx, lse, B, S, H, heads, dctx=None, dqkv=None, drop: Drop = NO_DROP, ctx_split3=None, qkv_hm=0,
               q_rows=0):
    a = AttnArgs()
    a.q_rows = int(q_rows)
    a.qkv_hm = int(qkv_hm)
    a.ctx_split3 = _h(ctx_split3)
    a.qkv, a.keymask, a.ctx, a.lse, a.dctx, a.dqkv = _h(qkv), _p(keymask), _h(ctx), _p(lse), _h(dctx), _h(dqkv)
    a.B, a.S, a.H, a.heads = B, S, H, heads
    _set_drop(a, drop)
    return a


def attention_fwd(qkv, keymask, ctx, lse, B, S, H, heads, drop: Drop = NO_DROP, ctx_split3=None, qkv_hm=0, q_rows=0):
    a = _attn_args(qkv, keymask, ctx, lse, B, S, H, heads, drop=drop, ctx_split3=ctx_split3, qkv_hm=qkv_hm, q_rows=q_rows)
    _invoke("vault_attention_fwd", C.byref(a), _stream(), struct=a, drop=drop)


def attention_bwd(qkv, keymask, ctx, lse, dctx, dqkv, B, S, H, heads, drop: Drop = NO_DROP, qkv_hm=0, bias_partials=None,
                  bias_thirds=1, q_rows=0):
    a = _attn_args(qkv, keymask, ctx, lse, B, S, H, heads, dctx, dqkv, drop, qkv_hm=qkv_hm, q_rows=q_rows)
    a.bias_partials, a.bias_thirds = _p(bias_partials), (int(bias_thirds) if bias_partials is not None else 0)
    _invoke("vault_attention_bwd", C.byref(a), _stream(), struct=a, drop=drop)


def attention_bwd_partials(B, S, H, heads, thirds) -> int:
    a = AttnArgs()
    a.B, a.S, a.H, a.heads, a.bias_thirds = B, S, H, heads, thirds
    return int(L.load(_FMT.get()).vault_attention_bwd_partials(C.byref(a)))


def colsum_partials(part_f32, nparts, n, out, batch=1, batch_in=0, batch_out=0):
    _invoke("vault_colsum_partials", C.c_void_p(_p(part_f32)), C.c_int(nparts), C.c_int(n), C.c_void_p(_p(out)), C.c_int(batch),
            C.c_longlong(batch_in), C.c_longlong(batch_out), _stream())


class GatherArgs(C.Structure):
    _fields_ = [("src", C.c_void_p), ("out", C.c_void_p),
                ("tab", C.c_void_p * 3), ("idx", C.c_void_p * 3), ("is64", C.c_int * 3), ("fixed", C.c_int * 3),
                ("period", C.c_int), ("rows", C.c_int), ("H", C.c_int), ("rowmask", C.c_void_p)]


class HeadArgs(C.Structure):
    _fields_ = [("pre", C.c_void_p), ("Wc", C.c_void_p), ("bc", C.c_void_p), ("labels", C.c_void_p),
                ("dlogits", C.c_void_p),
                ("pooled", C.c_void_p), ("logits", C.c_void_p), ("loss_sum", C.c_void_p), ("dWc", C.c_void_p),
                ("dbc", C.c_void_p), ("dpre_bf16", C.c_void_p),
                ("B", C.c_int), ("H", C.c_int), ("C", C.c_int), ("loss_scale", C.c_float), ("grad_scale", C.c_float),
                ("drop_thresh", C.c_uint32), ("drop_seed", C.c_uint32), ("drop_stream", C.c_uint32),
                ("drop_scale", C.c_float), ("targets", C.c_void_p), ("loss_kind", C.c_int)]


def position_ids(ids_i64, pos_i32, B, T, mode, pad):
    _invoke("vault_position_ids", C.c_void_p(_p(ids_i64)), C.c_void_p(_p(pos_i32)), C.c_int(B), C.c_int(T),
            C.c_int(mode), C.c_int(pad), _stream())


def _gather_args(src, out, tables, rows, H, period=1):
    a = GatherArgs()
    a.src, a.out, a.rows, a.H, a.period = _p(src), _p(out), rows, H, period
    for k in range(3):
        if k < len(tables) and tables[k] is not None:
            tab, idx = tables[k]
            a.tab[k] = _p(tab)
            if isinstance(idx, torch.Tensor):
                a.idx[k] = _p(idx)
                a.is64[k] = 1 if idx.dtype == torch.int64 else 0
                a.fixed[k] = 0
            elif idx == "mod":
                a.idx[k], a.is64[k], a.fixed[k] = None, 0, -2
            else:
                a.idx[k], a.is64[k], a.fixed[k] = None, 0, int(idx)
        else:
            a.tab[k], a.idx[k], a.is64[k], a.fixed[k] = None, None, 0, -1
    return a


def gather_sum(src, out, tables, rows, H, period=1):
    a = _gather_args(src, out, tables, rows, H, period)
    _invoke("vault_gather_sum", C.byref(a), _stream())


def scatter_add(src, grad_tables, rows, H, period=1, rowmask=None):
    a = _gather_args(src, None, grad_tables, rows, H, period)
    a.rowmask = _p(rowmask)
    _invoke("vault_scatter_add", C.byref(a), _stream())


def im2col(pix, out_bf16, B, Cn, IMG, ps, split3=False):
    _invoke("vault_im2col", C.c_void_p(_p(pix)), C.c_void_p(_p(out_bf16)), C.c_int(B), C.c_int(Cn), C.c_int(IMG),
            C.c_int(ps), C.c_int(1 if split3 else 0), _stream())


def image_consts(bias, pos, mtype1, cls, addtab, x, P, H, B, S, T):
    _invoke("vault_image_consts", C.c_void_p(_p(bias)), C.c_void_p(_p(pos)), C.c_void_p(_p(mtype1)),
            C.c_void_p(_p(cls)), C.c_void_p(_p(addtab)), C.c_void_p(_p(x)), C.c_int(P), C.c_int(H), C.c_int(B),
            C.c_int(S), C.c_int(T), _stream())


def image_rows_bwd(dx, dpos, dmtype1, dcls, dbias, dyp_bf16, P, H, B, S, T):
    _invoke("vault_image_rows_bwd", C.c_void_p(_p(dx)), C.c_void_p(_p(dpos)), C.c_void_p(_p(dmtype1)),
            C.c_void_p(_p(dcls)), C.c_void_p(_p(dbias)), C.c_void_p(_p(dyp_bf16)), C.c_int(P), C.c_int(H), C.c_int(B),
            C.c_int(S), C.c_int(T), _stream())


def im2col_sel(pix, out_bf16, sel, B, L, Cn, HP, WP, ps, split3=False):
    _invoke("vault_im2col_sel", C.c_void_p(_p(pix)), C.c_void_p(_p(out_bf16)), C.c_void_p(_p(sel)), C.c_int(B), C.c_int(L),
            C.c_int(Cn), C.c_int(HP), C.c_int(WP), C.c_int(ps), C.c_int(1 if split3 else 0), _stream())


def image_sel_consts(bias, pos, mtype1, cls, addtab, x, L, H, B, S, T):
    _invoke("vault_image_sel_consts", C.c_void_p(_p(bias)), C.c_void_p(_p(pos)), C.c_void_p(_p(mtype1)),
            C.c_void_p(_p(cls)), C.c_void_p(_p(addtab)), C.c_void_p(_p(x)), C.c_int(L), C.c_int(H), C.c_int(B),
            C.c_int(S), C.c_int(T), _stream())


def image_pos_sel_fwd(x, pos, sel, hw, B, L, S, T, H, gw, G):
    _invoke("vault_image_pos_sel_fwd", C.c_void_p(_p(x)), C.c_void_p(_p(pos)), C.c_void_p(_p(sel)), C.c_void_p(_p(hw)),
            C.c_int(B), C.c_int(L), C.c_int(S), C.c_int(T), C.c_int(H), C.c_int(gw), C.c_int(G), _stream())


def image_sel_bwd(dx, dpos, dmtype1, dcls, dbias, dyp_bf16, sel, hw, B, L, S, T, H, gw, G):
    _invoke("vault_image_sel_bwd", C.c_void_p(_p(dx)), C.c_void_p(_p(dpos)), C.c_void_p(_p(dmtype1)), C.c_void_p(_p(dcls)),
            C.c_void_p(_p(dbias)), C.c_void_p(_p(dyp_bf16)), C.c_void_p(_p(sel)), C.c_void_p(_p(hw)), C.c_int(B),
            C.c_int(L), C.c_int(S), C.c_int(T), C.c_int(H), C.c_int(gw), C.c_int(G), _stream())


def axpy(dst, src, a, n):
    _invoke("vault_axpy_f32", C.c_void_p(_p(dst)), C.c_void_p(_p(src)), C.c_float(a), C.c_longlong(n), _stream())


def scale(x, a, n):
    _invoke("vault_scale_f32", C.c_void_p(_p(x)), C.c_float(a), C.c_longlong(n), _stream())


def _head_args(pre, Wc, bc, labels, pooled, logits, loss_sum, B, H, Cc, loss_scale=1.0, grad_scale=1.0, dlogits=None,
               dWc=None, dbc=None, dpre=None, drop: Drop = NO_DROP):
    a = HeadArgs()
    a.pre, a.Wc, a.bc, a.labels, a.dlogits = _p(pre), _p(Wc), _p(bc), _p(labels), _p(dlogits)
    if labels is not None and labels.dtype.is_floating_point:
        if labels.dtype != torch.float32:
            raise TypeError("BCE targets must be float32")
        a.labels, a.targets, a.loss_kind = None, _p(labels), 1
    a.pooled, a.logits, a.loss_sum, a.dWc, a.dbc, a.dpre_bf16 = (_p(pooled), _p(logits), _p(loss_sum), _p(dWc),
                                                                 _p(dbc), _p(dpre))
    a.B, a.H, a.C, a.loss_scale, a.grad_scale = B, H, Cc, loss_scale, grad_scale
    _set_drop(a, drop)
    return a


def head_fwd(pre, Wc, bc, labels, pooled, logits, loss_sum, B, H, Cc, loss_scale, drop: Drop = NO_DROP):
    a = _head_args(pre, Wc, bc, labels, pooled, logits, loss_sum, B, H, Cc, loss_scale=loss_scale, drop=drop)
    _invoke("vault_head_fwd", C.byref(a), _stream(), struct=a, drop=drop)


def head_bwd(pooled, logits, labels, Wc, dWc, dbc, dpre, B, H, Cc, grad_scale, dlogits=None, drop: Drop = NO_DROP):
    a = _head_args(None, Wc, None, labels, pooled, logits, None, B, H, Cc, grad_scale=grad_scale, dlogits=dlogits,
                   dWc=dWc, dbc=dbc, dpre=dpre, drop=drop)
    _invoke("vault_head_bwd", C.byref(a), _stream(), struct=a, drop=drop)


def tanh_bwd(pooled, dpooled, dpre_bf16, n):
    _invoke("vault_tanh_bwd", C.c_void_p(_p(pooled)), C.c_void_p(_p(dpooled)), C.c_void_p(_p(dpre_bf16)),
            C.c_longlong(n), _stream())


def gelu_fwd(x, y_bf16, n):
    _invoke("vault_gelu_fwd", C.c_void_p(_p(x)), C.c_void_p(_p(y_bf16)), C.c_longlong(n), _stream())


def gelu_fwd_f32(x, y, n):
    _invoke("vault_gelu_fwd_f32", C.c_void_p(_p(x)), C.c_void_p(_p(y)), C.c_longlong(n), _stream())


def gelu_bwd(x, dy, dx, n):
    _invoke("vault_gelu_bwd", C.c_void_p(_p(x)), C.c_void_p(_p(dy)), C.c_void_p(_p(dx)), C.c_longlong(n), _stream())


def adamw_step(p, g, m, v, p_bf16, n, lr, beta1, beta2, eps, weight_decay, bias_corr_factor=1.0, grad_scale=1.0,
               zero_grad=True, zero_mask=None):
    _invoke("vault_adamw_step", C.c_void_p(_p(p)), C.c_void_p(_p(g)), C.c_void_p(_p(m)), C.c_void_p(_p(v)),
            C.c_void_p(_h(p_bf16)), C.c_longlong(n), C.c_float(lr), C.c_float(beta1), C.c_float(beta2), C.c_float(eps),
            C.c_float(weight_decay), C.c_float(bias_corr_factor), C.c_float(grad_scale),
            C.c_int(1 if zero_grad else 0), C.c_void_p(_p(zero_mask)), _stream())


GRAD_NORM_PARTIALS = 2048


def grad_norm(g, n, partials_f64, out2_f32, max_norm=float("inf"), unscale=1.0):
    if partials_f64.dtype != torch.float64 or partials_f64.numel() < GRAD_NORM_PARTIALS or out2_f32.dtype != torch.float32 \
            or out2_f32.numel() < 2:
        raise ValueError(f"grad_norm needs {GRAD_NORM_PARTIALS} float64 partials and two float32 outputs")
    _invoke("vault_grad_norm", C.c_void_p(_p(g)), C.c_longlong(n), C.c_void_p(_p(partials_f64)), C.c_void_p(_p(out2_f32)),
            C.c_float(max_norm), C.c_float(unscale), _stream())


def _check_groups(group_map, group_table, n):
    if group_map.dtype != torch.uint8 or group_table.dtype != torch.float32 or group_table.dim() != 2 \
            or group_table.shape[1] != 2 or group_map.numel() < (n + 63) // 64:
        raise ValueError("group_map: uint8, one byte per 64 elements; group_table: float32 [n_groups, 2]")


def _check_ema(ema, n):
    if ema is not None and (ema.dtype != torch.float32 or ema.numel() < n):
        raise ValueError("ema: float32, one element per parameter of the range")


def adamw_step_grouped(p, g, m, v, p_bf16, n, group_map, group_table, lr_factor, beta1, beta2, eps, bias_corr_factor=1.0,
                       grad_scale=1.0, coef=None, zero_grad=True, zero_mask=None):
    _check_groups(group_map, group_table, n)
    _invoke("vault_adamw_step_grouped", C.c_void_p(_p(p)), C.c_void_p(_p(g)), C.c_void_p(_p(m)), C.c_void_p(_p(v)),
            C.c_void_p(_h(p_bf16)), C.c_longlong(n), C.c_void_p(_p(group_map)), C.c_void_p(_p(group_table)),
            C.c_int(group_table.shape[0]), C.c_float(lr_factor), C.c_float(beta1), C.c_float(beta2), C.c_float(eps),
            C.c_float(bias_corr_factor), C.c_float(grad_scale), C.c_void_p(_p(coef)), C.c_int(1 if zero_grad else 0),
            C.c_void_p(_p(zero_mask)), _stream())


def adamw_step_ema(p, g, m, v, p_bf16, ema, n, group_map, group_table, lr_factor, beta1, beta2, eps, one_minus_decay,
                   bias_corr_factor=1.0, grad_scale=1.0, coef=None, zero_grad=True, zero_mask=None):
    _check_groups(group_map, group_table, n)
    _check_ema(ema, n)
    _invoke("vault_adamw_step_ema", C.c_void_p(_p(p)), C.c_void_p(_p(g)), C.c_void_p(_p(m)), C.c_void_p(_p(v)),
            C.c_void_p(_h(p_bf16)), C.c_void_p(_p(ema)), C.c_longlong(n), C.c_void_p(_p(group_map)),
            C.c_void_p(_p(group_table)), C.c_int(group_table.shape[0]), C.c_float(lr_factor), C.c_float(beta1),
            C.c_float(beta2), C.c_float(eps), C.c_float(bias_corr_factor), C.c_float(grad_scale), C.c_void_p(_p(coef)),
            C.c_float(one_minus_decay), C.c_int(1 if zero_grad else 0), C.c_void_p(_p(zero_mask)), _stream())


def adamw_step_torch(p, g, m, v, p_bf16, n, group_map, group_table, lr_factor, beta1, beta2, eps, inv_bias_corr1,
                     inv_sqrt_bias_corr2, ema=None, one_minus_decay=1.0, grad_scale=1.0, coef=None, zero_grad=True,
                     zero_mask=None):
    _check_groups(group_map, group_table, n)
    _check_ema(ema, n)
    _invoke("vault_adamw_step_torch", C.c_void_p(_p(p)), C.c_void_p(_p(g)), C.c_void_p(_p(m)), C.c_void_p(_p(v)),
            C.c_void_p(_h(p_bf16)), C.c_void_p(_p(ema)), C.c_longlong(n), C.c_void_p(_p(group_map)),
            C.c_void_p(_p(group_table)), C.c_int(group_table.shape[0]), C.c_float(lr_factor), C.c_float(beta1),
            C.c_float(beta2), C.c_float(eps), C.c_float(inv_bias_corr1), C.c_float(inv_sqrt_bias_corr2),
            C.c_float(grad_scale), C.c_void_p(_p(coef)), C.c_float(one_minus_decay), C.c_int(1 if zero_grad else 0),
            C.c_void_p(_p(zero_mask)), _stream())


def ema_swap(p, ema, p_bf16, n):
    if p.dtype != torch.float32 or ema.dtype != torch.float32 or p.numel() < n or ema.numel() < n \
            or (p_bf16 is not None and p_bf16.numel() < n):
        raise ValueError("ema_swap: float32 p and ema (and a 16-bit shadow) of at least n elements")
    _invoke("vault_ema_swap", C.c_void_p(_p(p)), C.c_void_p(_p(ema)), C.c_void_p(_h(p_bf16)), C.c_longlong(n), _stream())


def cast_bf16(x, y_bf16, n):
    _invoke("vault_cast_bf16", C.c_void_p(_p(x)), C.c_void_p(_h(y_bf16)), C.c_longlong(n), _stream())


def h16_census(x_h16, out4_u64):
    _invoke("vault_h16_census", C.c_void_p(_h(x_h16)), C.c_longlong(x_h16.numel()), C.c_void_p(_p(out4_u64)), _stream())


def rows_union(keys_i64, n_keys, V, flags_i32, uniq_i64, count_i32):
    _invoke("vault_rows_union", C.c_void_p(_p(keys_i64)), C.c_longlong(n_keys), C.c_int(V), C.c_void_p(_p(flags_i32)),
            C.c_void_p(_p(uniq_i64)), C.c_void_p(_p(count_i32)), _stream())


def rows_gather(table_f32, idx_i64, n_rows, H, out_f32):
    _invoke("vault_rows_gather_f32", C.c_void_p(_p(table_f32)), C.c_void_p(_p(idx_i64)), C.c_int(n_rows), C.c_int(H),
            C.c_void_p(_p(out_f32)), _stream())


def rows_scatter(src_f32, idx_i64, n_rows, H, table_f32):
    _invoke("vault_rows_scatter_f32", C.c_void_p(_p(src_f32)), C.c_void_p(_p(idx_i64)), C.c_int(n_rows), C.c_int(H),
            C.c_void_p(_p(table_f32)), _stream())


def sum_chunks_bf16(src_bf16, n_src, chunk, out_bf16):
    _invoke("vault_sum_chunks_bf16", C.c_void_p(_p(src_bf16)), C.c_int(n_src), C.c_longlong(chunk), C.c_void_p(_p(out_bf16)),
            _stream())


def widen_bf16(x_bf16, y_f32, n):
    _invoke("vault_widen_bf16", C.c_void_p(_p(x_bf16)), C.c_void_p(_p(y_f32)), C.c_longlong(n), _stream())


def split3_bf16(x_f32, out_bf16, rows, K, layout):
    _invoke("vault_split3_bf16", C.c_void_p(_p(x_f32)), C.c_void_p(_p(out_bf16)), C.c_longlong(rows), C.c_int(K),
            C.c_int(layout), _stream())


def transpose_bf16(src, dst, rows, cols, batch=1, stride_src=0, stride_dst=0):
    _invoke("vault_transpose_bf16", C.c_void_p(_h(src)), C.c_void_p(_h(dst)), C.c_int(rows), C.c_int(cols), C.c_int(batch),
            C.c_longlong(stride_src), C.c_longlong(stride_dst), _stream())


def rows_add(src, vec, out, rows, H, rpg, gstride, goff):
    _invoke("vault_rows_add_f32", C.c_void_p(_p(src)), C.c_void_p(_p(vec)), C.c_void_p(_p(out)), C.c_int(rows), C.c_int(H),
            C.c_int(rpg), C.c_int(gstride), C.c_int(goff), _stream())


def rows_scatter_h16(src, out, rows, H, rpg, gstride, goff):
    _invoke("vault_rows_scatter_bf16", C.c_void_p(_h(src)), C.c_void_p(_h(out)), C.c_int(rows), C.c_int(H), C.c_int(rpg),
            C.c_int(gstride), C.c_int(goff), _stream())


def rows_gather_bwd(dx, dsrc, dvec, rows, H, rpg, gstride, goff):
    _invoke("vault_rows_gather_bwd_f32", C.c_void_p(_p(dx)), C.c_void_p(_p(dsrc)), C.c_void_p(_p(dvec)), C.c_int(rows),
            C.c_int(H), C.c_int(rpg), C.c_int(gstride), C.c_int(goff), _stream())


class LayerArgs(C.Structure):
    _fields_ = ([(n, C.c_int) for n in ("B", "S", "H", "FF", "heads", "rows", "rows_pad")] + [("eps", C.c_float)] +
                [(n, C.c_void_p) for n in ("wqkv", "wo", "wi", "wf", "wo_t", "wf_t", "bqkv", "bo", "bi", "bf", "ln1w", "ln1b",
                                           "ln2w", "ln2b", "x_in", "x_in_bf16", "x_out", "x_out_bf16", "keymask", "n1", "qkv",
                                           "ctx", "lse", "xm", "y1", "n2", "act", "u", "h2", "m1", "r1", "m2", "r2")] +
                [(n, C.c_uint32) for n in ("attn_drop_thresh", "hid_drop_thresh", "drop_seed", "drop_stream_base")] +
                [("attn_drop_scale", C.c_float), ("hid_drop_scale", C.c_float), ("persist", C.c_int),
                 ("splitk_ws", C.c_void_p), ("splitk_bytes", C.c_longlong)])


class LayerBwdArgs(C.Structure):
    _fields_ = ([("fwd", C.POINTER(LayerArgs))] +
                [(n, C.c_void_p) for n in ("dy_bf16", "dy_f32", "dx_f32", "dx_bf16", "dU", "dN", "dctx", "dqkv", "dmid_bf16",
                                           "dh1_bf16", "dmid_f32", "g_wqkv", "g_bqkv", "g_wo", "g_bo", "g_wi", "g_bi", "g_wf",
                                           "g_bf", "g_ln1w", "g_ln1b", "g_ln2w", "g_ln2b", "g_bf_below")] +
                [("do_wgrad", C.c_int)])


def _struct(name, doc, spec):
    kinds = {"i": C.c_int, "f": C.c_float, "p": C.c_void_p, "u": C.c_uint32}
    fields = []
    for part in spec:
        k, names = part.split(":")
        fields += [(n, kinds[k]) for n in names.split()]
    return type(name, (C.Structure,), {"_fields_": fields, "__doc__": doc})


LmEmbedArgs = _struct("LmEmbedArgs", "vault_lm_embed_args", [
    "i:B T H rows_pad pos_mode pad_id", "f:eps", "p:ids token_type_ids inputs_embeds word pos type lnw lnb pos_ids esum mean rstd y y_bf16",
    "u:drop_thresh drop_seed drop_stream", "f:drop_scale", "p:dy_bf16 dy_f32 desum rowmask g_word g_pos g_type g_lnw g_lnb"])
TextEmbedArgs = _struct("TextEmbedArgs", "vault_text_embed_args", [
    "i:B T S H rows_pad", "f:eps", "p:text_src ids token_type_ids word pos type lnw lnb mtype0 vsum mean rstd x",
    "p:dx dvsum dbeta_scratch g_word g_pos g_type g_lnw g_lnb g_mtype0"])
PatchEmbedArgs = _struct("PatchEmbedArgs", "vault_patch_embed_args", [
    "i:B C IMG ps T S H", "p:pixel_values w_bf16 conv_bias pos_emb mtype1 cls apatch addtab x", "i:persist",
    "p:dx dyp g_w g_conv_bias g_pos g_mtype1 g_cls"])
HeadLossArgs = _struct("HeadLossArgs", "vault_head_loss_args", [
    "i:B S H C seq_rows_pad", "f:eps", "p:x lnw lnb wp_bf16 bp Wc bc labels targets", "i:loss_kind", "f:loss_scale grad_scale",
    "p:h0_bf16 mean rstd pre pooled logits loss", "u:drop_thresh drop_seed drop_stream", "f:drop_scale", "i:persist",
    "p:dpre dh0 dx_f32 dx_bf16 g_Wc g_bc g_wp g_bp g_lnw g_lnb g_bf_last"])
ModelDims = _struct("ModelDims", "vault_model_dims", ["i:H FF heads lm_layers vilt_layers IMG ps C n_classes"])


def stage_args(struct_type, /, **kw):
    a = struct_type()
    keep = []
    for k, v in kw.items():
        if isinstance(v, torch.Tensor):
            keep.append(v)
            v = _p(v)
        setattr(a, k, v)
    if hasattr(a, "persist"):
        a.persist = GEMM_SCHED
    a._keep = keep
    return a


def workspace_bytes(H, FF, heads, lm_layers, vilt_layers, IMG, ps, Cn, n_classes, B, T, train) -> int:
    fn = L.load(_FMT.get()).vault_workspace_bytes
    fn.restype = C.c_longlong
    d = ModelDims(H, FF, heads, lm_layers, vilt_layers, IMG, ps, Cn, n_classes)
    return int(fn(C.byref(d), C.c_int(B), C.c_int(T), C.c_int(1 if train else 0)))


def layer_args(**kw) -> LayerArgs:
    a = LayerArgs()
    for k, v in kw.items():
        setattr(a, k, _p(v) if isinstance(v, torch.Tensor) else v)
    a.persist = GEMM_SCHED
    return a


def layer_bwd_args(fwd: LayerArgs, **kw) -> LayerBwdArgs:
    g = LayerBwdArgs()
    g.fwd = C.pointer(fwd)
    for k, v in kw.items():
        setattr(g, k, _p(v) if isinstance(v, torch.Tensor) else v)
    g._fwd_keep = fwd
    return g


def layer_call(name: str, args, seeded: bool = False):
    fn = getattr(L.load(_FMT.get()), name)
    call = (C.byref(args), _stream())
    if _TAPE is not None:
        _TAPE.calls.append((fn, call))
        if seeded:
            _TAPE.seeded.append(args if isinstance(args, LayerArgs) else args._fwd_keep)
    L.check(fn(*call), name)
```

Measured before the change: 7011 samples/s.

## Pack leftover weight-gradient tiles into one mixed, load-balanced persistent launch

Adds a mixed weight-gradient kernel that takes per-block item tables covering tiles from many differently sized GEMMs, such as the pooler/last-layer wgrads, the patch embedding, partial ViLT groups and an LM tail. A host-side LPT scheduler assigns tiles to 256 blocks, using a cost model in K-steps plus a fixed per-item cost, and the plan is cached per signature. The aim is to replace several under-filled launches with one balanced launch so the GPU tail is not left idle. The cost is extra plan complexity and device-side segment and table buffers, and the cost model constants may not match real tile costs.

```diff
diff --git a/include/vault_hip.h b/include/vault_hip.h
--- a/include/vault_hip.h
+++ b/include/vault_hip.h
@@ -45,6 +45,29 @@
   int persist;
 } vault_wgrad_grouped_args;
 int vault_wgrad_grouped(const vault_wgrad_grouped_args* args, void* stream);
+
+typedef struct vault_wgrad_mixed_seg {
+  const void* dy; const void* x; float* dw;
+  int n_out, n_in, ld_dy, ld_x, ld_dw;
+  int batch;
+  int first, count;
+  long long batch_dy, batch_x, batch_dw;
+  int dy_hm;
+  int tokens;
+} vault_wgrad_mixed_seg;
+typedef struct vault_wgrad_mixed_args {
+  int nseg;
+  const vault_wgrad_mixed_seg* seg;
+  const void* seg_dev;
+  const int* table;
+  const int* table_dev;
+  int slots, blocks;
+  int x_arg_seg;
+  const void* x_arg;
+} vault_wgrad_mixed_args;
+int vault_wgrad_mixed(const vault_wgrad_mixed_args* args, void* stream);
+int vault_wgrad_mixed_plan(const vault_wgrad_mixed_seg* seg, int nseg, double cost_kstep, double cost_item, int blocks,
+                           int* table, int max_slots, double* makespan);
 
 int vault_quant_mxfp8(const void* src_bf16, long long rows, int K, int ld_src, void* dst_q, void* dst_scale, void* stream);
 int vault_gemm_mxfp8(const vault_gemm_args* args, const void* a_scale, const void* b_scale, void* stream);
diff --git a/vault_amd/backward.py b/vault_amd/backward.py
--- a/vault_amd/backward.py
+++ b/vault_amd/backward.py
@@ -10,6 +10,7 @@
 
 
 class BackwardMixin:
+    _tail, _tail_ws = None, None
     def _wgrads_aside(self, launch, after_layer, items=0):
         if not (self._wgrad_side or items > 0) or after_layer is not None:
             launch()
@@ -34,10 +35,16 @@
             ops.pycall(lambda: main.wait_event(ev))
             self._wgrad_pending = False
 
-    def _wgrad(self, dy_bf16, x_bf16, wname, bname, Mtok_pad, Nout, Kin, m_valid, out_rows=0, unsplit=False):
+    def _wgrad(self, dy_bf16, x_bf16, wname, bname, Mtok_pad, Nout, Kin, m_valid, out_rows=0, unsplit=False, tail=False):
         P = self.params
         gw = P.gr(wname, n_elems=Nout * Kin, shape=(Nout, Kin))
         if gw is None:
+            return
+        if tail and self._tail is not None and bname is None and not out_rows and Nout % 256 == 0 and Kin % 256 == 0 \
+                and Mtok_pad % 64 == 0:
+            self._tail.append(dict(dy=dy_bf16, x=x_bf16, dw=gw, n_out=Nout, n_in=Kin, batch=1, first=0,
+                                   count=(Nout // 256) * (Kin // 256), tokens=Mtok_pad, m_valid=m_valid, x_arg=(tail == "x_arg")))
+            self._stored_ranges.append((P.offsets[wname][0], Nout * Kin))
             return
         nk = Mtok_pad // 64
         wide = Nout % 256 == 0 and Kin % 256 == 0 and (Nout // 256) * (Kin // 256) >= 24
@@ -107,7 +114,7 @@
         g = self.LM_WGRAD_GROUP
         return g if g > 0 else n_layers
 
-    def _wgrad_group(self, kinds, layers, i0, hi, Mtok_pad, m_valid, counts=None):
+    def _wgrad_group(self, kinds, layers, i0, hi, Mtok_pad, m_valid, counts=None, tag=None):
         P = self.params
         Gs = [hi - i0] * len(kinds) if counts is None else list(counts)
         kinds, Gs = [k for k, n in zip(kinds, Gs) if n > 0], [n for n in Gs if n > 0]
@@ -131,21 +138,37 @@
         remaining = []
         for k, (dY_all, X_all, wsel, Nout, Kin) in enumerate(kinds):
             remaining.append([k, 0, (Nout // 256) * (Kin // 256) * Gs[k]])
-        launches, cur, room = [], [], CU
+        mixed = self._tail is not None and tag in ("vilt", "lm") and CU == 256
+        tail_items = self._lm_tail_items(sum(r[2] for r in remaining), nk) if (mixed and tag == "lm") else 0
+        launches, cur, room = [], [], (tail_items or CU)
         for k, first, left in remaining:
             while left > 0:
                 take = min(left, room)
                 cur.append((k, first, take))
                 first, left, room = first + take, left - take, room - take
-                if room == 0 or len(cur) == 3:
+                if room == 0 or (len(cur) == 3 and not (tail_items and not launches)):
                     launches.append(cur)
                     cur, room = [], CU
         if cur:
             launches.append(cur)
         st = torch.cuda.current_stream()
         covered: Dict[tuple, int] = {}
-        for segs in launches:
+        for li, segs in enumerate(launches):
             count = sum(c for _, _, c in segs)
+            defer = mixed and ((tag == "lm" and tail_items and li == 0) or (tag == "vilt" and count < CU))
+            if defer:
+                for k, first, c in segs:
+                    dY_all, X_all, wsel, Nout, Kin = kinds[k]
+                    tpl = (Nout // 256) * (Kin // 256)
+                    for it in range(first, first + c):
+                        covered[(k, it // tpl)] = covered.get((k, it // tpl), 0) + 1
+                    gw = P.gr(getattr(layers[i0], wsel), n_elems=Nout * Kin, shape=(Nout, Kin))
+                    self._tail.append(dict(dy=dY_all[i0], x=X_all[i0], dw=gw, n_out=Nout, n_in=Kin, batch=Gs[k], first=first, count=c,
+                                           batch_dy=dY_all.stride(0), batch_x=X_all.stride(0), batch_dw=strides[k], dy_hm=hms[k],
+                                           tokens=Mtok_pad, m_valid=m_valid))
+                if tag == "lm":
+                    self._wgrad_tail_launch()
+                continue
             if count == CU:
                 splits = 1
             else:
@@ -165,10 +188,58 @@
             ops.wgrad_grouped(args, Mtok_pad, splits=splits, accumulate=acc)
             fl = 2.0 * m_valid * 65536.0 * count
             ops.pycall(lambda fl=fl: self._prof_end("wgrad", fl, st))
+        if mixed and tag == "lm" and not tail_items:
+            self._wgrad_tail_launch()
         for (k, lay), n in covered.items():
             _, _, wsel, Nout, Kin = kinds[k]
             if n == (Nout // 256) * (Kin // 256):
                 self._stored_ranges.append((P.offsets[getattr(layers[i0 + lay], wsel)][0], Nout * Kin))
+
+    def _mixed_tail_applies(self, ws, after_layer):
+        H, FF = ws["H"], ws["FF"]
+        return bool(self.WGRAD_MIXED_TAIL and after_layer is None and self.dp_world <= 1 and self.spec.lm is not None
+                    and not self.freeze_lm and self._grads_zero and not self._wgrad_side and ops.GEMM_SCHED == 0
+                    and not ws.get("vilt_stage") and not ws.get("lm_stage") and self.LM_WGRAD_BATCHED
+                    and "act_all" in ws and "lm_act_all" in ws and H % 256 == 0 and FF % 256 == 0
+                    and ws["Mp"] % 64 == 0 and ws["Mlp"] % 64 == 0 and self.WGRAD_BESIDE_LM_ITEMS == 0
+                    and self.params.gr(self.vl[0].fw) is not None and self.params.gr(self.ll[0].fw) is not None)
+
+    def _lm_tail_items(self, items, nk):
+        ck, ci = ops.WGRAD_MIXED_COST_KSTEP, ops.WGRAD_MIXED_COST_ITEM
+        best = None
+        for j in range(3):
+            n = items % 256 + 256 * j
+            if n > items:
+                break
+            kinds = [(g["tokens"], g["count"]) for g in self._tail] + ([(64 * nk, n)] if n else [])
+            if not kinds:
+                continue
+            span = ops.wgrad_mixed_makespan(kinds, 256)
+            cost = span + ((items - n) // 256) * (ci + ck * nk)
+            if best is None or cost < best[0] - 1e-9:
+                best = (cost, n)
+        return best[1] if best else 0
+
+    def _wgrad_tail_launch(self):
+        segs, self._tail = self._tail, None
+        if not segs:
+            return
+        ws = self._tail_ws
+        xs = [k for k, g in enumerate(segs) if g.get("x_arg")]
+        sig = tuple((g["dy"].data_ptr(), 0 if g.get("x_arg") else g["x"].data_ptr(), g["dw"].data_ptr(), g["n_out"], g["n_in"],
+                     g["batch"], g["first"], g["count"], g["tokens"], g.get("dy_hm", 0)) for g in segs)
+        cached = ws.get("wgrad_mixed_plan")
+        if cached is None or cached[0] != sig:
+            cached = (sig, ops.WgradMixedPlan(segs, blocks=256, x_arg_seg=xs[0] if xs else -1))
+            ws["wgrad_mixed_plan"] = cached
+        plan = cached[1]
+        if xs:
+            plan.set_x_arg(segs[xs[0]]["x"])
+        st = torch.cuda.current_stream()
+        fl = sum(2.0 * g["m_valid"] * 65536.0 * g["count"] for g in segs)
+        ops.pycall(lambda: self._prof_begin("wgrad", st))
+        plan.launch()
+        ops.pycall(lambda: self._prof_end("wgrad", fl, st))
 
     def _qkv_bias_grads_batched(self, dqkv_all, layers, i0, hi, ld, rows, N, hm=0, parts=None):
         P = self.params
@@ -245,6 +316,7 @@
         self.drop_seed = ws["drop_seed"]
         note = (lambda tag: ops.pycall(lambda: after_layer(tag))) if after_layer is not None else (lambda tag: None)
         self._wgrad_side = ws["Mp"] <= self.WGRAD_STREAM_MAX_ROWS
+        self._tail, self._tail_ws = ([] if self._mixed_tail_applies(ws, after_layer) else None), ws
         vb = self._vilt_grad_buffers(ws, after_layer)
         self._backward_head(ws, vb["top"], grad_scale, dlogits, dpooled, dhidden)
         note("head")
@@ -255,6 +327,9 @@
             self._join_wgrads()
         else:
             self._backward_lm_stack(ws, dvs, after_layer, note)
+        if self._tail:
+            self._wgrad_tail_launch()
+        self._tail = None
         self._run_census(ws, "backward")
 
     def _wgrad_groups(self, ws, tag, layers, after_layer, dY, X, rows_pad, rows):
@@ -277,7 +352,7 @@
         def launch():
             self._qkv_bias_grads_batched(kinds[3][0], layers, i, hi, 3 * H, grp["rows"], 3 * H if N is None else N, hm=hm, parts=parts)
             self._wgrad_group(kinds[:3] + (kinds[3] + (hm,),), layers, i, hi, grp["rows_pad"], grp["rows"],
-                              counts=[max(0, min(hi, e) - i) for e in grp["ends"]])
+                              counts=[max(0, min(hi, e) - i) for e in grp["ends"]], tag=tag)
         self._wgrads_aside(launch, after_layer, items=items)
         for j in reversed(range(i, hi)):
             note(f"{tag}{j}")
@@ -413,15 +488,15 @@
         g8 = ws.get("pl_gelu8")
         g8kw = dict(cfg=g8, aux_u8=True) if g8 is not None else {}
         self._dgrad(dtop, ln.fw, dU, Bp, FF, H, ops.EPI_BF16_DGELU, B, aux=c("u"), colsum=P.gr(ln.ib), like=Mp, **g8kw)
-        self._wgrad(dtop, c("act"), ln.fw, None, Bp, H, FF, B, unsplit=True)
+        self._wgrad(dtop, c("act"), ln.fw, None, Bp, H, FF, B, unsplit=True, tail=True)
         self._dgrad(dU, ln.iw, dNc, Bp, H, FF, ops.EPI_BF16, B, like=Mp)
-        self._wgrad(dU, c("n2"), ln.iw, None, Bp, FF, H, B, unsplit=True)
+        self._wgrad(dU, c("n2"), ln.iw, None, Bp, FF, H, B, unsplit=True, tail=True)
         ops.layernorm_bwd(c("xm"), c("m2"), c("r2"), P.w(ln.ln2w), B, H, dy_bf16=dNc, dres_bf16=dtop, dx_bf16=dmid,
                           dgamma=P.gr(ln.ln2w), dbeta=P.gr(ln.ln2b), dbias=P.gr(ln.ob))
         ops.rows_scatter_h16(dmid, dres, B, H, 1, S, 0)
         gqb = P.gr(ln.qb, n_elems=3 * H, shape=(3 * H,))
         self._dgrad(dmid, ln.ow, dctx, Bp, H, H, ops.EPI_BF16, B, like=Mp, **(dict(colsum=gqb[2 * H:]) if short else {}))
-        self._wgrad(dmid, c("ctx"), ln.ow, None, Bp, H, H, B, unsplit=True)
+        self._wgrad(dmid, c("ctx"), ln.ow, None, Bp, H, H, B, unsplit=True, tail=True)
         ops.attention_bwd(g("qkv"), ws["keymask"], c("ctx"), g("lse"), dctx, dqkv, B, S, H, heads, qkv_hm=vhm, q_rows=1,
                           **(dict(bias_partials=vparts[0][i], bias_thirds=1) if vparts else {}))
         self._dgrad(dqkv, ln.qw, dN, Mp, H, 3 * H, ops.EPI_BF16, M, **(dict(a_hm=vhm) if vhm else {}))
@@ -452,7 +527,7 @@
         if ws.get("img_embeds") is None:
             self._wgrads_aside(lambda: self._wgrad(dyp, ws["apatch_in"] if ws.get("patches_in") else ws["apatch"],
                                                    "embeddings.patch_embeddings.projection.weight", None,
-                                                   Mpp, H, Kp, B * NP), after_layer)
+                                                   Mpp, H, Kp, B * NP, tail="x_arg"), after_layer)
         dvs = buf("d_vt_sum", (Mlp, H))
         dbeta_now = buf("d_vt_beta", (H,))
         ops.pycall(dbeta_now.zero_)
diff --git a/vault_amd/csrc/capi_gemm.hip b/vault_amd/csrc/capi_gemm.hip
--- a/vault_amd/csrc/capi_gemm.hip
+++ b/vault_amd/csrc/capi_gemm.hip
@@ -79,6 +79,23 @@
   return vault_gemm256_grouped_launch(p, reinterpret_cast<hipStream_t>(stream));
 }
 
+static_assert(sizeof(vault_wgrad_mixed_seg) == sizeof(GemmMixSeg) && offsetof(vault_wgrad_mixed_seg, dw) == offsetof(GemmMixSeg, dw) &&
+              offsetof(vault_wgrad_mixed_seg, count) == offsetof(GemmMixSeg, count) &&
+              offsetof(vault_wgrad_mixed_seg, batch_dw) == offsetof(GemmMixSeg, batch_dw) &&
+              offsetof(vault_wgrad_mixed_seg, dy_hm) == offsetof(GemmMixSeg, dy_hm) &&
+              offsetof(vault_wgrad_mixed_seg, tokens) == offsetof(GemmMixSeg, tokens), "vault_wgrad_mixed_seg layout");
+
+extern "C" int vault_wgrad_mixed_plan(const vault_wgrad_mixed_seg* seg, int nseg, double cost_kstep, double cost_item, int blocks,
+                                      int* table, int max_slots, double* makespan) {
+  return vault_wgrad_plan_items(reinterpret_cast<const GemmMixSeg*>(seg), nseg, cost_kstep, cost_item, blocks, table, max_slots, makespan);
+}
+
+extern "C" int vault_wgrad_mixed(const vault_wgrad_mixed_args* a, void* stream) {
+  if (a == nullptr) return VAULT_EINVAL;
+  return vault_gemm256_mixed_launch(reinterpret_cast<const GemmMixSeg*>(a->seg), a->nseg, a->seg_dev, a->table, a->table_dev,
+                                    a->slots, a->blocks, a->x_arg, a->x_arg_seg, reinterpret_cast<hipStream_t>(stream));
+}
+
 extern "C" int vault_abi_version(void) { return 12; }
 #ifdef VAULT_F16
 extern "C" int vault_operand_format(void) { return 1; }
diff --git a/vault_amd/csrc/gemm.h b/vault_amd/csrc/gemm.h
--- a/vault_amd/csrc/gemm.h
+++ b/vault_amd/csrc/gemm.h
@@ -59,7 +59,27 @@
     long long batch_a, batch_b, batch_o;
     int a_hm;
   } seg[3];
+  const void* mix_seg;
+  const int* mix_table;
+  int mix_slots;
+  int mix_xseg;
 };
+
+struct GemmMixSeg {
+  const void* dy; const void* x; float* dw;
+  int n_out, n_in, ld_dy, ld_x, ld_dw;
+  int batch;
+  int first, count;
+  long long batch_dy, batch_x, batch_dw;
+  int dy_hm;
+  int tokens;
+};
+constexpr int GEMM_MIX_MAX_SEGS = 32;
+
+int vault_wgrad_plan_items(const GemmMixSeg* seg, int nseg, double cost_kstep, double cost_item, int blocks, int* table,
+                           int max_slots, double* makespan);
+int vault_gemm256_mixed_launch(const GemmMixSeg* seg, int nseg, const void* seg_dev, const int* table, const int* table_dev,
+                               int slots, int blocks, const void* x_arg, int x_arg_seg, hipStream_t st);
 
 constexpr int GEMM_SK_COUNTER_BYTES = 16384;
 constexpr int GEMM_SK_MAX_TILES = GEMM_SK_COUNTER_BYTES / 4;
diff --git a/vault_amd/csrc/gemm256.hip b/vault_amd/csrc/gemm256.hip
--- a/vault_amd/csrc/gemm256.hip
+++ b/vault_amd/csrc/gemm256.hip
@@ -1,4 +1,6 @@
 #include <algorithm>
+#include <queue>
+#include <vector>
 #include "common.h"
 #include "gemm.h"
 #include "gemm_epi.h"
@@ -49,8 +51,9 @@
 #ifndef R256_ORDER
 #define R256_ORDER -1
 #endif
-template <int A_MODE, int B_MODE, int EPI, int NTQ, bool DYN, bool SK = false>
+template <int A_MODE, int B_MODE, int EPI, int NTQ, bool DYN, bool SK = false, bool MIXED = false>
 __global__ __launch_bounds__(256) void gemm256_kernel(const GemmParams p) {
+  static_assert(!MIXED || (EPI == EPI_F32_ATOMIC && A_MODE == 1 && B_MODE == 1 && NTQ == 4 && !DYN && !SK), "mixed launch: weight gradients");
   H16_SATURATE();
 #if R256_STAMP
   const unsigned long long st_c0 = __builtin_amdgcn_s_memtime(), st_r0 = __builtin_amdgcn_s_memrealtime();
@@ -76,7 +79,7 @@
   bool grouped = false;
   int seg_total = 0;
   if constexpr (EPI == EPI_F32_ATOMIC && A_MODE == 1 && B_MODE == 1) {
-    grouped = p.nseg > 0;
+    grouped = MIXED || p.nseg > 0;
     seg_total = p.seg[0].count + (p.nseg > 1 ? p.seg[1].count : 0) + (p.nseg > 2 ? p.seg[2].count : 0);
   }
   const int nwork = grouped ? seg_total * p.splits : ntiles * p.splits * nbatch;
@@ -121,7 +124,33 @@
     }
   };
   auto setup = [&](int w) {
-    if constexpr (EPI == EPI_F32_ATOMIC && A_MODE == 1 && B_MODE == 1) {
+    if constexpr (MIXED) {
+      typedef const __attribute__((address_space(4))) GemmMixSeg CSeg;
+      CSeg* sg = (CSeg*)(p.mix_seg);
+      int r = w, si = 0, cnt = sg->count;
+      while (r >= cnt) { r -= cnt; ++sg; ++si; cnt = sg->count; }
+      const int tn_k = sg->n_in >> 8, tm_k = sg->n_out >> 8, tiles_k = tn_k * tm_k;
+      const int idx = sg->first + r;
+      const int bz = idx / tiles_k, tl = idx - bz * tiles_k;
+      const int lda_ = sg->dy_hm ? 64 : sg->ld_dy, ldb_ = sg->ld_x, ahm_ = sg->dy_hm;
+      const h16* pA = reinterpret_cast<const h16*>(sg->dy) + (size_t)bz * sg->batch_dy;
+      const h16* pB = (si == p.mix_xseg ? p.B : reinterpret_cast<const h16*>(sg->x)) + (size_t)bz * sg->batch_x;
+      out_cur = sg->dw + (size_t)bz * sg->batch_dw;
+      ldo_cur = sg->ld_dw;
+      mvalid_cur = tm_k << 8;
+      int tile_m, tile_n;
+      if (tn_k > tm_k) { tile_n = tl / tm_k; tile_m = tl - tile_n * tm_k; }
+      else { tile_m = tl / tn_k; tile_n = tl - tile_m * tn_k; }
+      m0 = tile_m << 8; n0 = tile_n << 8;
+      nk = sg->tokens >> 6;
+      a_step = 64u * (uint32_t)lda_ * 2u; b_step = 64u * (uint32_t)ldb_ * 2u;
+      a_half = ahm_ ? (uint32_t)ahm_ * 128u : 128u;
+      lane_offsets(lda_, ldb_, ahm_);
+      a_base = ahm_ ? reinterpret_cast<const char*>(pA + (size_t)(m0 >> 6) * ahm_ * 64) : reinterpret_cast<const char*>(pA + m0);
+      b_base = reinterpret_cast<const char*>(pB + n0);
+      return;
+    }
+    if constexpr (EPI == EPI_F32_ATOMIC && A_MODE == 1 && B_MODE == 1 && !MIXED) {
       if (grouped) {
         const int lin = gemm_xcd_contiguous(nwork, w);
         const int z = lin / seg_total;
@@ -196,7 +225,14 @@
     else b_base = reinterpret_cast<const char*>(pB + (size_t)kt0 * 64 * p.ldb + ln0);
   };
   int w = blockIdx.x;
-  setup(w);
+  if constexpr (MIXED) {
+    const int item0 = ((const __attribute__((address_space(4))) int*)(p.mix_table))[blockIdx.x];
+    if (item0 < 0) return;
+    w = 0;
+    setup(item0);
+  } else {
+    setup(w);
+  }
   const int xcd = blockIdx.x & 7;
   auto items_of = [&](int x) { return x < nwork ? (nwork - x + 7) >> 3 : 0; };
   auto static_of = [&](int x) { return x < (int)gridDim.x ? ((int)gridDim.x - x + 7) >> 3 : 0; };
@@ -434,7 +470,10 @@
     float* const eout = out_cur;
     const int eldo = ldo_cur, emvalid = mvalid_cur;
     int* sched_lds = reinterpret_cast<int*>(smem + 2 * BUFB + SCRATCH_BYTES);
-    if (!dyn) {
+    if constexpr (MIXED) {
+      if (tid == 0)
+        *sched_lds = (w + 1 < p.mix_slots) ? ((const __attribute__((address_space(4))) int*)(p.mix_table))[(w + 1) * (int)gridDim.x + (int)blockIdx.x] : -1;
+    } else if (!dyn) {
       if (tid == 0) *sched_lds = (w + (int)gridDim.x < nwork) ? w + (int)gridDim.x : -1;
     } else if (tid == 0) {
       int wn = -1;
@@ -559,7 +598,7 @@
     }
     if (!more) break;
     behind_stores = (em0 + 256 <= emvalid);
-    w = wnext;
+    w = MIXED ? w + 1 : wnext;
   }
 #if R256_STAMP
   if (threadIdx.x == 0) {
@@ -742,6 +781,102 @@
   return (int)hipGetLastError();
 }
 
+#if !R256_DYN
+static bool mix_seg_ok(const GemmMixSeg& g) {
+  if (!g.dy || !g.x || !g.dw || g.n_out <= 0 || g.n_in <= 0 || (g.n_out & 255) || (g.n_in & 255) || g.batch < 1 ||
+      g.tokens <= 0 || (g.tokens & 63) || g.first < 0 || g.count < 1)
+    return false;
+  const long long tiles = (long long)(g.n_out / 256) * (g.n_in / 256);
+  if ((long long)g.first + g.count > tiles * g.batch) return false;
+  if ((g.ld_x & 7) || (g.ld_dw & 3) || (g.batch_dy & 7) || (g.batch_x & 7) || (g.batch_dw & 3) || g.ld_x < g.n_in || g.ld_dw < g.n_in)
+    return false;
+  if (g.dy_hm < 0 || (g.dy_hm > 0 && g.dy_hm < g.tokens)) return false;
+  if (g.dy_hm == 0 && ((g.ld_dy & 7) || g.ld_dy < g.n_out)) return false;
+  return true;
+}
+
+int vault_wgrad_plan_items(const GemmMixSeg* seg, int nseg, double cost_kstep, double cost_item, int blocks, int* table,
+                           int max_slots, double* makespan) {
+  if (seg == nullptr || nseg < 1 || nseg > GEMM_MIX_MAX_SEGS || blocks < 1 || blocks > 256 || cost_kstep < 0.0 || cost_item < 0.0)
+    return -VAULT_EINVAL;
+  struct Item { double cost; int id; };
+  std::vector<Item> items;
+  int total = 0;
+  for (int k = 0; k < nseg; ++k) {
+    if (seg[k].count < 1 || seg[k].tokens <= 0 || (seg[k].tokens & 63)) return -VAULT_EINVAL;
+    const double c = cost_item + cost_kstep * (seg[k].tokens / 64);
+    for (int j = 0; j < seg[k].count; ++j) items.push_back(Item{c, total + j});
+    total += seg[k].count;
+  }
+  std::stable_sort(items.begin(), items.end(), [](const Item& a, const Item& b) { return a.cost > b.cost; });
+  struct Blk { double load; int xcd, pos, id; };
+  auto later = [](const Blk& a, const Blk& b) {
+    if (a.load != b.load) return a.load > b.load;
+    if (a.xcd != b.xcd) return a.xcd > b.xcd;
+    return a.pos > b.pos;
+  };
+  std::priority_queue<Blk, std::vector<Blk>, decltype(later)> heap(later);
+  for (int b = 0; b < blocks; ++b) heap.push(Blk{0.0, b & 7, b >> 3, b});
+  std::vector<std::vector<int>> lists(blocks);
+  double span = 0.0;
+  for (const Item& it : items) {
+    Blk b = heap.top();
+    heap.pop();
+    lists[b.id].push_back(it.id);
+    b.load += it.cost;
+    span = std::max(span, b.load);
+    heap.push(b);
+  }
+  int slots = 1;
+  for (const auto& l : lists) slots = std::max(slots, (int)l.size());
+  if (makespan) *makespan = span;
+  if (table != nullptr && max_slots >= slots) {
+    for (int s = 0; s < slots; ++s)
+      for (int b = 0; b < blocks; ++b) table[s * blocks + b] = s < (int)lists[b].size() ? lists[b][s] : -1;
+  }
+  return slots;
+}
+
+int vault_gemm256_mixed_launch(const GemmMixSeg* seg, int nseg, const void* seg_dev, const int* table, const int* table_dev,
+                               int slots, int blocks, const void* x_arg, int x_arg_seg, hipStream_t st) {
+  if (x_arg_seg < -1 || x_arg_seg >= nseg || (x_arg_seg >= 0 && (x_arg == nullptr || ((size_t)x_arg & 15)))) return VAULT_EINVAL;
+  if (seg == nullptr || seg_dev == nullptr || table == nullptr || table_dev == nullptr || nseg < 1 || nseg > GEMM_MIX_MAX_SEGS ||
+      slots < 1 || blocks < 1 || blocks > 256 || ((size_t)seg_dev & 7) || ((size_t)table_dev & 3))
+    return VAULT_EINVAL;
+  long long total = 0;
+  for (int k = 0; k < nseg; ++k) {
+    if (!mix_seg_ok(seg[k])) return VAULT_EINVAL;
+    total += seg[k].count;
+  }
+  for (int b = 0; b < blocks; ++b) {
+    bool ended = false;
+    for (int s = 0; s < slots; ++s) {
+      const int id = table[s * blocks + b];
+      if (id < -1 || id >= total || (ended && id >= 0)) return VAULT_EINVAL;
+      ended = ended || id < 0;
+    }
+  }
+  GemmParams q{};
+  q.A = reinterpret_cast<const h16*>(seg[0].dy); q.B = reinterpret_cast<const h16*>(seg[0].x); q.out = seg[0].dw;
+  q.M = 256; q.N = 256; q.K = 64; q.lda = 256; q.ldb = 256; q.ldo = 256; q.m_valid = 256;
+  q.splits = 1; q.accumulate = 0; q.gn = 1;
+  q.mix_seg = seg_dev; q.mix_table = table_dev; q.mix_slots = slots; q.mix_xseg = x_arg_seg;
+  if (x_arg_seg >= 0) q.B = reinterpret_cast<const h16*>(x_arg);
+  constexpr int LDS = 2 * BUFB + 4 * 16 * (64 + 4) * 4 + 16;
+  auto kern = gemm256_kernel<1, 1, EPI_F32_ATOMIC, 4, false, false, true>;
+  static bool attr_done[64] = {};
+  int dev = 0;
+  if (hipGetDevice(&dev) != hipSuccess || dev < 0 || dev >= 64) return VAULT_EINVAL;
+  if (!attr_done[dev]) {
+    hipError_t e = hipFuncSetAttribute(reinterpret_cast<const void*>(kern), hipFuncAttributeMaxDynamicSharedMemorySize, LDS);
+    if (e != hipSuccess) return (int)e;
+    attr_done[dev] = true;
+  }
+  hipLaunchKernelGGL(kern, dim3(blocks), dim3(256), LDS, st, q);
+  return (int)hipGetLastError();
+}
+#endif
+
 int R256_PUBLIC(vault_gemm256_launch)(const GemmParams& p, int a_mode, int b_mode, int epi, int ntq, hipStream_t st) {
 #if !R256_DYN
   if (p.persist & 1) return vault_gemm256_launch_dyn(p, a_mode, b_mode, epi, ntq, st);
diff --git a/vault_amd/engine.py b/vault_amd/engine.py
--- a/vault_amd/engine.py
+++ b/vault_amd/engine.py
@@ -265,6 +265,7 @@
     SPLITK = True
     SPLITK_WS_BYTES = 16384 + (64 << 20)
     WGRAD_BESIDE_LM_ITEMS = 0
+    WGRAD_MIXED_TAIL = True
     WGRAD_SIDE_ITEMS = 224
 
     def _plan_gelu8(self, ws, n2, act, u, ln, Mp, M):
diff --git a/vault_amd/ops.py b/vault_amd/ops.py
--- a/vault_amd/ops.py
+++ b/vault_amd/ops.py
@@ -222,6 +222,88 @@
     _invoke("vault_wgrad_grouped", C.byref(a), _stream(), struct=a)
 
 
+class WgradMixedSeg(C.Structure):
+    _fields_ = WgradSeg._fields_ + [("tokens", C.c_int)]
+
+
+class WgradMixedArgs(C.Structure):
+    _fields_ = [("nseg", C.c_int), ("seg", C.POINTER(WgradMixedSeg)), ("seg_dev", C.c_void_p), ("table", C.POINTER(C.c_int)),
+                ("table_dev", C.c_void_p), ("slots", C.c_int), ("blocks", C.c_int), ("x_arg_seg", C.c_int), ("x_arg", C.c_void_p)]
+
+
+WGRAD_MIXED_COST_KSTEP, WGRAD_MIXED_COST_ITEM = 1.54, 8.0
+
+
+def wgrad_mixed_segs(segs):
+    arr = (WgradMixedSeg * len(segs))()
+    for t, g in zip(arr, segs):
+        t.dy, t.x, t.dw = _h(g["dy"]), _h(g["x"]), _p(g["dw"])
+        t.n_out, t.n_in = g["n_out"], g["n_in"]
+        t.ld_dy, t.ld_x, t.ld_dw = g.get("ld_dy", g["n_out"]), g.get("ld_x", g["n_in"]), g.get("ld_dw", g["n_in"])
+        t.batch, t.first, t.count = g["batch"], g["first"], g["count"]
+        t.batch_dy, t.batch_x, t.batch_dw = g.get("batch_dy", 0), g.get("batch_x", 0), g.get("batch_dw", 0)
+        t.dy_hm, t.tokens = int(g.get("dy_hm", 0)), g["tokens"]
+    return arr
+
+
+def wgrad_mixed_table(seg_arr, blocks, cost_kstep=None, cost_item=None):
+    ck = WGRAD_MIXED_COST_KSTEP if cost_kstep is None else cost_kstep
+    ci = WGRAD_MIXED_COST_ITEM if cost_item is None else cost_item
+    fn = L.load(_FMT.get()).vault_wgrad_mixed_plan
+    fn.restype = C.c_int
+    fn.argtypes = [C.POINTER(WgradMixedSeg), C.c_int, C.c_double, C.c_double, C.c_int, C.POINTER(C.c_int), C.c_int,
+                   C.POINTER(C.c_double)]
+    span = C.c_double(0.0)
+    slots = fn(seg_arr, len(seg_arr), ck, ci, blocks, None, 0, C.byref(span))
+    if slots < 1:
+        raise ValueError(f"vault_wgrad_mixed_plan refused the segments (code {slots})")
+    tab = (C.c_int * (slots * blocks))()
+    fn(seg_arr, len(seg_arr), ck, ci, blocks, tab, slots, C.byref(span))
+    return list(tab), slots, span.value
+
+
+def wgrad_mixed_makespan(kinds, blocks, cost_kstep=None, cost_item=None):
+    arr = (WgradMixedSeg * len(kinds))()
+    for t, (tokens, n) in zip(arr, kinds):
+        t.tokens, t.count = tokens, n
+    return wgrad_mixed_table(arr, blocks, cost_kstep, cost_item)[2]
+
+
+class WgradMixedPlan:
+
+    def __init__(self, segs, blocks=256, table=None, slots=None, device=None, x_arg_seg=-1):
+        self.seg = wgrad_mixed_segs(segs)
+        self.blocks = blocks
+        if table is None:
+            table, slots, self.makespan = wgrad_mixed_table(self.seg, blocks)
+        else:
+            self.makespan = None
+        self.slots = slots
+        if not slots or len(table) != slots * blocks:
+            raise ValueError("the item table must be [slots][blocks]")
+        self.table = (C.c_int * len(table))(*table)
+        dev = device if device is not None else segs[0]["dw"].device
+        raw = torch.frombuffer(bytearray(bytes(self.seg)), dtype=torch.uint8)
+        self.seg_dev = raw.to(dev)
+        self.table_dev = torch.tensor(list(table), dtype=torch.int32).to(dev)
+        a = self.args = WgradMixedArgs()
+        a.nseg, a.seg, a.seg_dev = len(segs), self.seg, self.seg_dev.data_ptr()
+        a.table, a.table_dev, a.slots, a.blocks = self.table, self.table_dev.data_ptr(), slots, blocks
+        a.x_arg_seg, a.x_arg = x_arg_seg, (self.seg[x_arg_seg].x if x_arg_seg >= 0 else None)
+        self.items = sum(g["count"] for g in segs)
+        self.tile_tokens = sum(g["count"] * g["tokens"] for g in segs)
+
+    def set_x_arg(self, x):
+        self.args.x_arg = _h(x)
+
+    def launch(self):
+        if _TAPE is not None and _TAPE.rebind_range is not None and self.args.x_arg_seg >= 0:
+            lo, hi = _TAPE.rebind_range
+            if lo <= (self.args.x_arg or 0) < hi:
+                _TAPE.rebinds.append((self.args, "x_arg", self.args.x_arg - lo))
+        _invoke("vault_wgrad_mixed", C.byref(self.args), _stream(), struct=self.args)
+
+
 def quant_mxfp8(src_bf16, rows, K, ld, dst_q, dst_scale):
     _invoke("vault_quant_mxfp8", C.c_void_p(_p(src_bf16)), C.c_longlong(rows), C.c_int(K), C.c_int(ld),
             C.c_void_p(_p(dst_q)), C.c_void_p(_p(dst_scale)), _stream())
```

Result: no change. 7055 samples/s, median of 6 (+0.6%).
